# lightest/cellularautomatons3d

Measured on AMD Instinct MI355X. Metric: Gcells/s CA step at 512^3, higher is better.
Workload: dtype u32

## Files before the change

cellularautomatons3d_amd/_capi.py:

```python
from __future__ import annotations

import ctypes as C
import os

_HERE = os.path.dirname(os.path.abspath(__file__))
LIB_PATH = os.path.join(_HERE, "libca3d.so")

CA3D_OK = 0
LAYOUT_PACKED32 = 0
LAYOUT_UNPACKED = 1
LUT_LEN = 81
COMM_ID_BYTES = 128

SLAB_SEND_LOW, SLAB_SEND_HIGH, SLAB_RECV_LOW, SLAB_RECV_HIGH, SLAB_OWNED = range(5)
SLAB_PHASE_ALL, SLAB_PHASE_EDGES, SLAB_PHASE_INTERIOR = range(3)


class Ca3dError(RuntimeError):
    def __init__(self, code: int, message: str):
        super().__init__(f"ca3d error {code}: {message}")
        self.code = code
        self.message = message


class Info(C.Structure):
    _fields_ = [
        ("grid_size", C.c_uint32), ("layout", C.c_int32), ("z0", C.c_uint32), ("nz", C.c_uint32),
        ("ghost", C.c_uint32), ("step", C.c_uint64), ("state_words", C.c_uint64),
        ("current_buffer", C.c_int32), ("device", C.c_int32), ("kernel_name", C.c_char * 64),
        ("launches_total", C.c_uint64),
    ]


class Stats(C.Structure):
    _fields_ = [
        ("steps", C.c_uint64), ("kernel_launches", C.c_uint64), ("gpu_ms", C.c_double),
        ("cell_steps", C.c_double), ("algorithmic_bytes", C.c_double),
    ]


class RenderStats(C.Structure):
    _fields_ = [
        ("gpu_ms", C.c_double), ("primary_rays", C.c_uint64), ("shadow_rays", C.c_uint64),
        ("primary_cell_visits", C.c_uint64), ("shadow_cell_visits", C.c_uint64),
    ]


class SummaryStruct(C.Structure):
    _fields_ = [
        ("step", C.c_uint64), ("population", C.c_uint64), ("births", C.c_uint64), ("deaths", C.c_uint64), ("digest", C.c_uint64),
        ("has_previous", C.c_uint32), ("box_min", C.c_uint32 * 3), ("box_max", C.c_uint32 * 3),
    ]


class ComponentStruct(C.Structure):
    _fields_ = [
        ("population", C.c_uint32), ("first_cell", C.c_uint32), ("box_min", C.c_uint32), ("box_max", C.c_uint32), ("digest", C.c_uint64),
        ("reserved", C.c_uint32 * 2),
    ]


class IsolateJobStruct(C.Structure):
    _fields_ = [("universe", C.c_uint32), ("cell", C.c_uint32)]


class IsolatedStruct(C.Structure):
    _fields_ = [("population", C.c_uint32), ("shift", C.c_int32 * 3)]


ISOLATE_PLACEMENTS = {"keep": 0, "centre": 1, "origin": 2}
ISOLATE_COPY_RULES = 0x100
CONNECTIVITIES = {"closed": 0, "torus": 1}


class ComposePartStruct(C.Structure):
    _fields_ = [("universe", C.c_uint32), ("orientation", C.c_uint32), ("at", C.c_int32 * 3), ("reserved", C.c_uint32)]


class ComposedStruct(C.Structure):
    _fields_ = [("population", C.c_uint32), ("placed", C.c_uint32), ("overlap", C.c_uint32), ("clipped", C.c_uint32)]


class CanonStruct(C.Structure):
    _fields_ = [("key", C.c_uint64), ("symmetry", C.c_uint64), ("orientation", C.c_uint32), ("population", C.c_uint32),
                ("box_min", C.c_uint32), ("box_max", C.c_uint32)]


class CanonPeriodStruct(C.Structure):
    _fields_ = [("key", C.c_uint64), ("symmetry", C.c_uint64), ("orientation", C.c_uint32), ("phase", C.c_uint32),
                ("population", C.c_uint32), ("flags_shift", C.c_uint32)]


class EnvelopeStruct(C.Structure):
    _fields_ = [("period", C.c_uint32), ("flags", C.c_uint32), ("heat", C.c_uint32), ("population_sum", C.c_uint32),
                ("envelope_population", C.c_uint32), ("stator_population", C.c_uint32), ("envelope_min", C.c_uint8 * 4),
                ("envelope_max", C.c_uint8 * 4), ("rotor_min", C.c_uint8 * 4), ("rotor_max", C.c_uint8 * 4), ("reserved", C.c_uint32 * 2)]


ENVELOPE_COPY_RULES = 0x100
COMPOSE_OVER = 0x1
COMPOSE_COPY_RULES = 0x100
COMPOSE_MAX_PARTS = 1 << 20


class SeedStruct(C.Structure):
    _fields_ = [("seed", C.c_uint32), ("and_rounds", C.c_uint32), ("box_min", C.c_uint32 * 3), ("box_max", C.c_uint32 * 3)]


STOP_EXTINCT, STOP_STILL = 1, 2
STOP_PERIODIC = 4
STOP_MOVING = 8
ENSEMBLE_ALL = 0xFFFFFFFF
ENSEMBLE_WORDS = 8192


class CommInfo(C.Structure):
    _fields_ = [("device", C.c_int32), ("comm_ranks", C.c_int32), ("comm_rank", C.c_int32), ("comm_device", C.c_int32),
                ("pci_bus_id", C.c_char * 32)]


class JitStats(C.Structure):
    _fields_ = [
        ("programs_compiled", C.c_uint64), ("programs_from_disk", C.c_uint64), ("programs_from_memory", C.c_uint64),
        ("compile_ms", C.c_double), ("disk_read_ms", C.c_double), ("load_ms", C.c_double), ("cache_dir", C.c_char * 256),
    ]


def jit_stats() -> dict:
    st = JitStats()
    check(load().ca3d_get_jit_stats(C.byref(st)))
    return {"programs_compiled": int(st.programs_compiled), "programs_from_disk": int(st.programs_from_disk),
            "programs_from_memory": int(st.programs_from_memory), "compile_ms": round(st.compile_ms, 2),
            "disk_read_ms": round(st.disk_read_ms, 2), "load_ms": round(st.load_ms, 2), "cache_dir": st.cache_dir.decode()}


_u32p = C.POINTER(C.c_uint32)
_i32p = C.POINTER(C.c_int32)
_H = C.c_void_p
SYMBOLS = [
    ("ca3d_abi_version", C.c_int, []),
    ("ca3d_last_error", C.c_char_p, []),
    ("ca3d_selftest_exception", C.c_int, [C.c_int]),
    ("ca3d_get_jit_stats", C.c_int, [C.c_void_p]),
    ("ca3d_device_count", C.c_int, [C.POINTER(C.c_int)]),
    ("ca3d_create", C.c_int, [C.c_int, C.POINTER(_H)]),
    ("ca3d_destroy", C.c_int, [_H]),
    ("ca3d_configure", C.c_int, [_H, C.c_uint32, C.c_uint32, C.c_uint32, C.c_int]),
    ("ca3d_configure_slab", C.c_int, [_H, C.c_uint32, C.c_int, C.c_uint32, C.c_uint32, C.c_uint32]),
    ("ca3d_set_rules", C.c_int, [_H, _i32p, C.c_uint32, _i32p, C.c_uint32, _i32p, C.c_uint32, _u32p, _u32p]),
    ("ca3d_upload_state", C.c_int, [_H, _u32p, C.c_size_t]),
    ("ca3d_read_state", C.c_int, [_H, _u32p, C.c_size_t]),
    ("ca3d_step", C.c_int, [_H, C.c_uint32]),
    ("ca3d_flush", C.c_int, [_H]),
    ("ca3d_slab_step", C.c_int, [_H, C.c_uint32]),
    ("ca3d_slab_step_phase", C.c_int, [_H, C.c_uint32, C.c_int]),
    ("ca3d_slab_region", C.c_int, [_H, C.c_int, C.POINTER(C.c_void_p), C.POINTER(C.c_size_t)]),
    ("ca3d_comm_unique_id", C.c_int, [C.c_void_p]),
    ("ca3d_slab_comm_init", C.c_int, [_H, C.c_void_p, C.c_int, C.c_int]),
    ("ca3d_slab_run", C.c_int, [_H, C.c_uint32, C.c_int]),
    ("ca3d_slab_exchange", C.c_int, [_H]),
    ("ca3d_slab_comm_info", C.c_int, [_H, C.c_void_p]),
    ("ca3d_slab_gather", C.c_int, [_H, _H]),
    ("ca3d_group_create", C.c_int, [C.POINTER(C.c_int), C.c_int, C.POINTER(_H)]),
    ("ca3d_group_destroy", C.c_int, [_H]),
    ("ca3d_group_size", C.c_int, [_H, C.POINTER(C.c_int)]),
    ("ca3d_group_engine", C.c_int, [_H, C.c_int, C.POINTER(_H)]),
    ("ca3d_group_configure", C.c_int, [_H, C.c_uint32, C.c_int, C.c_uint32]),
    ("ca3d_group_set_rules", C.c_int, [_H, _i32p, C.c_uint32, _i32p, C.c_uint32, _i32p, C.c_uint32, _u32p, _u32p]),
    ("ca3d_group_upload_state", C.c_int, [_H, _u32p, C.c_size_t]),
    ("ca3d_group_read_state", C.c_int, [_H, _u32p, C.c_size_t]),
    ("ca3d_group_step", C.c_int, [_H, C.c_uint32]),
    ("ca3d_group_synchronize", C.c_int, [_H]),
    ("ca3d_group_set_option", C.c_int, [_H, C.c_char_p, C.c_int64]),
    ("ca3d_group_render", C.c_int, [_H, C.POINTER(C.c_float), C.c_uint32, C.c_uint32, C.c_uint32, C.c_void_p, C.c_void_p, C.c_void_p]),
    ("ca3d_group_summarize", C.c_int, [_H, C.POINTER(SummaryStruct), _u32p]),
    ("ca3d_summarize", C.c_int, [_H, C.POINTER(SummaryStruct), _u32p]),
    ("ca3d_get_summary_time", C.c_int, [_H, C.POINTER(C.c_double)]),
    ("ca3d_step_until", C.c_int, [_H, C.c_uint32, C.c_uint32, C.c_uint32, C.POINTER(SummaryStruct), _u32p, _u32p]),
    ("ca3d_step_until_cycle", C.c_int, [_H, C.c_uint32, C.c_uint32, C.c_uint32, C.POINTER(SummaryStruct), _u32p, _u32p, _u32p]),
    ("ca3d_ensemble_create", C.c_int, [C.c_int, C.POINTER(_H)]),
    ("ca3d_ensemble_destroy", C.c_int, [_H]),
    ("ca3d_ensemble_configure", C.c_int, [_H, C.c_uint32, C.c_uint32]),
    ("ca3d_ensemble_configure_neighbourhood", C.c_int, [_H, C.c_uint32, C.c_uint32, C.c_int]),
    ("ca3d_ensemble_get_neighbourhood", C.c_int, [_H, C.POINTER(C.c_int)]),
    ("ca3d_ensemble_configure_clustered", C.c_int, [_H, C.c_uint32, C.c_uint32]),
    ("ca3d_ensemble_get_clustered", C.c_int, [_H, C.POINTER(C.c_int)]),
    ("ca3d_ensemble_set_boundary", C.c_int, [_H, C.c_int]),
    ("ca3d_ensemble_get_boundary", C.c_int, [_H, C.POINTER(C.c_int)]),
    ("ca3d_ensemble_set_rule_tables_clustered", C.c_int, [_H, C.c_uint32, C.c_uint32, _u32p, _u32p, C.c_uint32]),
    ("ca3d_ensemble_set_rules", C.c_int, [_H, C.c_uint32, _i32p, C.c_uint32, _i32p, C.c_uint32, _i32p, C.c_uint32, _u32p, _u32p]),
    ("ca3d_ensemble_upload_state", C.c_int, [_H, C.c_uint32, C.c_uint32, _u32p, C.c_size_t]),
    ("ca3d_ensemble_read_state", C.c_int, [_H, C.c_uint32, C.c_uint32, _u32p, C.c_size_t]),
    ("ca3d_seed_state", C.c_int, [_H, C.POINTER(SeedStruct)]),
    ("ca3d_group_seed_state", C.c_int, [_H, C.POINTER(SeedStruct)]),
    ("ca3d_ensemble_seed_state", C.c_int, [_H, C.c_uint32, C.c_uint32, C.POINTER(SeedStruct), C.c_uint32]),
    ("ca3d_ensemble_set_rule_tables", C.c_int, [_H, C.c_uint32, C.c_uint32, _u32p, _u32p, C.c_uint32]),
    ("ca3d_ensemble_step", C.c_int, [_H, C.c_uint32]),
    ("ca3d_ensemble_step_until", C.c_int, [_H, C.c_uint32, C.c_uint32, C.c_uint32, _u32p, _u32p]),
    ("ca3d_ensemble_step_until_cycle", C.c_int, [_H, C.c_uint32, C.c_uint32, C.c_uint32, _u32p, _u32p, _u32p]),
    ("ca3d_ensemble_step_until_moving", C.c_int, [_H, C.c_uint32, C.c_uint32, C.c_uint32, _u32p, _u32p, _u32p, _i32p]),
    ("ca3d_ensemble_step_until_trace", C.c_int, [_H, C.c_uint32, C.c_uint32, C.c_uint32, _u32p, _u32p, _u32p, C.c_uint32, _u32p]),
    ("ca3d_ensemble_summarize", C.c_int, [_H, C.c_uint32, C.c_uint32, C.POINTER(SummaryStruct)]),
    ("ca3d_ensemble_census", C.c_int, [_H, C.c_uint32, C.c_uint32, C.c_uint32, C.POINTER(ComponentStruct), _u32p, _u32p, C.POINTER(C.c_float)]),
    ("ca3d_ensemble_isolate", C.c_int, [_H, C.c_uint32, _H, C.c_uint32, C.POINTER(IsolateJobStruct), C.c_uint32, C.POINTER(IsolatedStruct),
                                        C.POINTER(C.c_float)]),
    ("ca3d_ensemble_census_connected", C.c_int, [_H, C.c_uint32, C.c_uint32, C.c_uint32, C.c_uint32, C.POINTER(ComponentStruct), _u32p, _u32p,
                                                 C.POINTER(C.c_float)]),
    ("ca3d_ensemble_isolate_connected", C.c_int, [_H, C.c_uint32, _H, C.c_uint32, C.POINTER(IsolateJobStruct), C.c_uint32, C.c_uint32,
                                                  C.POINTER(IsolatedStruct), C.POINTER(C.c_float)]),
    ("ca3d_ensemble_compose", C.c_int, [_H, C.c_uint32, C.c_uint32, _H, C.POINTER(ComposePartStruct), _u32p, C.c_uint32,
                                        C.POINTER(ComposedStruct), C.POINTER(C.c_float)]),
    ("ca3d_ensemble_canon", C.c_int, [_H, C.c_uint32, C.c_uint32, C.POINTER(CanonStruct), C.POINTER(C.c_uint64), C.POINTER(C.c_float)]),
    ("ca3d_ensemble_canon_period", C.c_int, [_H, C.c_uint32, C.c_uint32, _u32p, C.POINTER(CanonPeriodStruct), C.POINTER(C.c_uint64), C.c_uint32,
                                             C.POINTER(C.c_float)]),
    ("ca3d_ensemble_envelope", C.c_int, [_H, C.c_uint32, C.c_uint32, _u32p, _H, C.c_uint32, C.c_uint32, C.POINTER(EnvelopeStruct),
                                         C.POINTER(C.c_float)]),
    ("ca3d_ensemble_synchronize", C.c_int, [_H]),
    ("ca3d_ensemble_get_stats", C.c_int, [_H, C.POINTER(Stats)]),
    ("ca3d_ensemble_render_sheet", C.c_int, [_H, C.c_uint32, C.c_uint32, C.POINTER(C.c_float), C.c_uint32, C.c_uint32, C.c_uint32, C.c_uint32,
                                             C.c_void_p, C.c_void_p, C.c_void_p]),
    ("ca3d_ensemble_get_sheet_stats", C.c_int, [_H, C.POINTER(RenderStats)]),
    ("ca3d_render_target", C.c_int, [_H, C.c_int, C.POINTER(C.c_void_p), C.POINTER(C.c_size_t)]),
    ("ca3d_synchronize", C.c_int, [_H]),
    ("ca3d_recovered_launches", C.c_int, [_H, C.POINTER(C.c_uint32)]),
    ("ca3d_measure_copy", C.c_int, [_H, C.c_size_t, C.c_uint32, C.POINTER(C.c_double)]),
    ("ca3d_set_stream", C.c_int, [_H, C.c_void_p]),
    ("ca3d_use_own_stream", C.c_int, [_H]),
    ("ca3d_device_buffer", C.c_int, [_H, C.c_int, C.POINTER(C.c_void_p), C.POINTER(C.c_size_t)]),
    ("ca3d_get_info", C.c_int, [_H, C.POINTER(Info)]),
    ("ca3d_get_jit_log", C.c_int, [_H, C.c_char_p, C.c_size_t, C.POINTER(C.c_size_t)]),
    ("ca3d_get_kernel_variant", C.c_int, [_H, C.c_char_p, C.c_size_t, C.POINTER(C.c_size_t)]),
    ("ca3d_get_stats", C.c_int, [_H, C.POINTER(Stats)]),
    ("ca3d_set_option", C.c_int, [_H, C.c_char_p, C.c_int64]),
    ("ca3d_render", C.c_int, [_H, C.POINTER(C.c_float), C.c_uint32, C.c_uint32, C.c_uint32, C.c_void_p, C.c_void_p, C.c_void_p]),
    ("ca3d_get_render_pipeline", C.c_int, [_H, C.POINTER(C.c_int32)]),
    ("ca3d_get_render_stats", C.c_int, [_H, C.POINTER(RenderStats)]),
]

_lib = None


def _pin_hip_runtime() -> None:
    if os.environ.get("CA3D_NO_TORCH_PRELOAD"):
        return
    try:
        import torch
    except ImportError:
        pass


def load() -> C.CDLL:
    global _lib
    if _lib is None:
        if not os.path.exists(LIB_PATH):
            raise ImportError(
                f"{LIB_PATH} is missing: build the HIP library first (python -c 'import __graft_entry__ as g; g.build()'). "
                "cellularautomatons3d_amd has no CPU fallback.")
        _pin_hip_runtime()
        lib = C.CDLL(LIB_PATH)
        for name, restype, argtypes in SYMBOLS:
            fn = getattr(lib, name)
            fn.restype = restype
            fn.argtypes = argtypes
        _lib = lib
    return _lib


def check(rc: int) -> None:
    if rc != CA3D_OK:
        raise Ca3dError(rc, load().ca3d_last_error().decode("utf-8", "replace"))
```

cellularautomatons3d_amd/csrc/ca3d_api.cpp:

```cpp
#include <cstdarg>
#include <cstdio>
#include <cstring>
#include <cstdlib>
#include <new>
#include <stdexcept>

#include "ca3d_engine.h"

namespace
{
thread_local char g_last_error[1024] = "";
}

namespace ca3d
{
void set_last_error(const char *msg) noexcept
{
	if (!msg) msg = "";
	size_t n = strlen(msg);
	if (n >= sizeof g_last_error) n = sizeof g_last_error - 1;
	memmove(g_last_error, msg, n);
	g_last_error[n] = 0;
}

// ... 118 lines not shown
	if (!h->has_state) return fail(CA3D_ERR_NOT_CONFIGURED, "ca3d_upload_state has not been called");
	return CA3D_OK;
}

static int state_replaced(ca3d_engine *h)
{
	h->step = 0;
	h->cur = 0;
	h->prev_ok = false;
	h->state_serial++;
	h->buffers_exposed = false;
	h->pending_edges = 0;
	h->ghosts_valid = false;
	h->res_pending.clear();
	if (h->res_status_host && *h->res_status_host)
	{
		HIP_TRY(hipMemsetAsync(h->res_mail, 0, h->res_mail_bytes, h->stream));
		HIP_TRY(hipMemsetAsync(h->res_status, 0, kResStatusBytes, h->stream));
		h->res_status_host[0] = h->res_status_host[1] = 0;
		h->res_epoch = 0;
		h->res_check = false;
		h->res_failed = true;
	}
	h->has_state = true;
	return CA3D_OK;
}

const char *seed_spec_error(const ca3d_seed &s, uint32_t G)
{
	if (s.and_rounds > 31u) return "and_rounds must be in [0, 31]";
	for (int i = 0; i < 3; i++)
	{
		if (s.box_min[i] > s.box_max[i]) return "box_min exceeds box_max";
		if (s.box_max[i] >= G) return "box_max lies outside the grid";
	}
	return nullptr;
}

static int switch_stream(ca3d_engine *h, hipStream_t s)
{
	if (!h) return fail(CA3D_ERR_INVALID_ARGUMENT, "NULL engine handle");
	FLUSH_QUEUED(h);
	int rc = bind_device(h);
	if (rc) return rc;
	HIP_TRY(hipStreamSynchronize(h->stream));
	rc = check_resident(h);
	if (rc) return rc;
	resident_stream_retired(h->stream);
	drop_graph(h);
	h->stream = s;
	h->ev_valid = false;
	refresh_kernels(h);
	return CA3D_OK;
}
}

using namespace ca3d;

extern "C"
{

int ca3d_abi_version(void) { return CA3D_ABI_VERSION; }

const char *ca3d_last_error(void) { return g_last_error; }

int ca3d_selftest_exception(int kind) CA3D_API_TRY
{
	if (kind == 0) throw std::bad_alloc();
	if (kind == 1) throw std::runtime_error("selftest");
	if (kind == 2) throw 42;
	if (kind == 3)
	{
		std::vector<char> v;
		v.resize(v.max_size() / 2u);
		return fail(CA3D_ERR_DEVICE, "selftest: the allocation of %zu bytes succeeded", v.size());
	}
	return CA3D_OK;
}
CA3D_API_CATCH

int ca3d_device_count(int *out_count) CA3D_API_TRY
{
	if (!out_count) return fail(CA3D_ERR_INVALID_ARGUMENT, "out_count is NULL");
	int n = 0;
	hipError_t e = hipGetDeviceCount(&n);
	if (e != hipSuccess) { *out_count = 0; return fail(CA3D_ERR_DEVICE, "hipGetDeviceCount: %s", hipGetErrorString(e)); }
	*out_count = n;
	return CA3D_OK;
}
CA3D_API_CATCH

int ca3d_create(int device, ca3d_t **out) CA3D_API_TRY
{
	if (!out) return fail(CA3D_ERR_INVALID_ARGUMENT, "out is NULL");
	*out = nullptr;
	int n = 0;
	hipError_t e = hipGetDeviceCount(&n);
	if (e != hipSuccess || n <= 0)
		return fail(CA3D_ERR_DEVICE, "no HIP device available (%s); this engine has no CPU fallback",
		            e != hipSuccess ? hipGetErrorString(e) : "device count is 0");
	if (device < 0 || device >= n) return fail(CA3D_ERR_INVALID_ARGUMENT, "device %d out of range [0,%d)", device, n);
	HIP_TRY(hipSetDevice(device));
	hipDeviceProp_t prop;
	HIP_TRY(hipGetDeviceProperties(&prop, device));
	if (strncmp(prop.gcnArchName, "gfx950", 6) != 0)
		return fail(CA3D_ERR_UNSUPPORTED, "device %d is %s; this library carries gfx950 (MI355X) code objects only", device, prop.gcnArchName);
	ca3d_engine *h = new (std::nothrow) ca3d_engine();
	if (!h) return fail(CA3D_ERR_OUT_OF_MEMORY, "out of host memory");
	h->device = device;
	hipError_t err = hipStreamCreateWithFlags(&h->own_stream, hipStreamNonBlocking);
	if (err == hipSuccess) err = hipEventCreate(&h->ev_start);
	if (err == hipSuccess) err = hipEventCreate(&h->ev_stop);
	if (err == hipSuccess) err = hipEventCreate(&h->rev_start);
	if (err == hipSuccess) err = hipEventCreate(&h->rev_stop);
	if (err != hipSuccess)
	{
		ca3d_destroy(h);
		return fail(CA3D_ERR_DEVICE, "engine set-up failed: %s", hipGetErrorString(err));
	}
	h->stream = h->own_stream;
	*out = h;
	return CA3D_OK;
}
CA3D_API_CATCH

int ca3d_destroy(ca3d_t *h) CA3D_API_TRY
{
	if (!h) return CA3D_OK;
	hipSetDevice(h->device);
	h->queued = 0;
	if (h->stream || h->own_stream) hipStreamSynchronize(h->stream);
	for (auto &L : h->lanes)
		if (L.s) hipStreamSynchronize(L.s);
	resident_stream_retired(h->stream);
	free_buffers(h);
	free_render_targets(h);
	free_slab_comm(h);
	if (h->r_counters) hipFree(h->r_counters);
	if (h->r_occ) hipFree(h->r_occ);
	if (h->r_stream) hipFree(h->r_stream);
	if (h->r_bricks) hipFree(h->r_bricks);
	for (auto &L : h->lanes)
	{
		if (L.s) { hipStreamSynchronize(L.s); hipStreamDestroy(L.s); }
		for (hipEvent_t e : {L.start, L.stop, L.done})
			if (e) hipEventDestroy(e);
		if (L.scratch) hipFree(L.scratch);
		if (L.counters) hipFree(L.counters);
	}
	for (hipStream_t sp : h->lane_spares) hipStreamDestroy(sp);
	if (h->ev_state) hipEventDestroy(h->ev_state);
	if (h->r_aux) hipStreamDestroy(h->r_aux);
	if (h->r_fork) hipEventDestroy(h->r_fork);
	if (h->r_join) hipEventDestroy(h->r_join);
	if (h->rev_start) hipEventDestroy(h->rev_start);
	if (h->rev_stop) hipEventDestroy(h->rev_stop);
	if (h->ev_start) hipEventDestroy(h->ev_start);
	if (h->ev_stop) hipEventDestroy(h->ev_stop);
	if (h->sum_ev0) hipEventDestroy(h->sum_ev0);
	if (h->sum_ev1) hipEventDestroy(h->sum_ev1);
	if (h->own_stream) hipStreamDestroy(h->own_stream);
	delete h;
	return CA3D_OK;
}
CA3D_API_CATCH

static int configure_common(ca3d_t *h, uint32_t g, int layout)
{
	if (!h) return fail(CA3D_ERR_INVALID_ARGUMENT, "NULL engine handle");
	if (layout != CA3D_LAYOUT_PACKED32 && layout != CA3D_LAYOUT_UNPACKED) return fail(CA3D_ERR_INVALID_ARGUMENT, "unknown layout %d", layout);
	if (g == 0) return fail(CA3D_ERR_INVALID_ARGUMENT, "grid size must be positive");
	if (layout == CA3D_LAYOUT_PACKED32 && (g % 32u)) return fail(CA3D_ERR_INVALID_ARGUMENT, "packed layout needs a grid size that is a multiple of 32 (got %u)", g);
	if (layout == CA3D_LAYOUT_UNPACKED && (g % 4u)) return fail(CA3D_ERR_INVALID_ARGUMENT, "unpacked layout needs a grid size that is a multiple of 4 (got %u)", g);
	if (g > 8192u) return fail(CA3D_ERR_UNSUPPORTED, "grid size %u exceeds the supported maximum 8192", g);
	int rc = bind_device(h);
	if (rc) return rc;
	HIP_TRY(hipStreamSynchronize(h->stream));
	free_buffers(h);
	h->buffers_exposed = false;
	h->G = g;
	h->layout = layout;
	h->plane_words = layout == CA3D_LAYOUT_PACKED32 ? (size_t)(g / 32u) * g : (size_t)g * g;
	return CA3D_OK;
}

int ca3d_configure(ca3d_t *h, uint32_t gx, uint32_t gy, uint32_t gz, int layout) CA3D_API_TRY
{
	if (gx != gy || gy != gz) return fail(CA3D_ERR_UNSUPPORTED, "only cubic grids exist in the reference (got %ux%ux%u)", gx, gy, gz);
	if (h) h->queued = 0;
	int rc = configure_common(h, gx, layout);
	if (rc) return rc;
	h->slab = false;
	h->z0 = 0;
	h->nz = gx;
	h->ghost = 0;
	h->nplanes = gx;
	rc = allocate(h);
	if (rc == CA3D_OK) refresh_kernels(h);
	return rc;
}
CA3D_API_CATCH

int ca3d_configure_slab(ca3d_t *h, uint32_t g, int layout, uint32_t z0, uint32_t nz, uint32_t ghost) CA3D_API_TRY
{
	if (h) h->queued = 0;
	int rc = configure_common(h, g, layout);
	if (rc) return rc;
	if (nz == 0 || z0 + nz > g) return fail(CA3D_ERR_INVALID_ARGUMENT, "slab [%u, %u) is outside the grid of %u planes", z0, z0 + nz, g);
	if (ghost == 0 || ghost > nz) return fail(CA3D_ERR_INVALID_ARGUMENT, "ghost depth must be in [1, nz] (got %u, nz %u)", ghost, nz);
	if (layout == CA3D_LAYOUT_UNPACKED && (g & (g - 1u))) return fail(CA3D_ERR_UNSUPPORTED, "unpacked slabs need a power-of-two grid size: the legacy kernel's -1 wrap is a torus only then");
	h->slab = true;
	h->z0 = z0;
	h->nz = nz;
	h->ghost = ghost;
	h->nplanes = nz + 2u * ghost;
	rc = allocate(h);
	if (rc == CA3D_OK) refresh_kernels(h);
	return rc;
}
CA3D_API_CATCH

int ca3d_set_rules(ca3d_t *h, const int32_t *main_offsets, uint32_t n_main, const int32_t *edges_offsets, uint32_t n_edges,
                   const int32_t *corners_offsets, uint32_t n_corners, const uint32_t survive[CA3D_LUT_LEN],
                   const uint32_t born[CA3D_LUT_LEN]) CA3D_API_TRY
{
	if (!h) return fail(CA3D_ERR_INVALID_ARGUMENT, "NULL engine handle");
	FLUSH_QUEUED(h);
	if (int rcs = settle_resident(h)) return rcs;
	CanonRules r;
	std::string err;
	int rc = canonicalize_rules(main_offsets, n_main, edges_offsets, n_edges, corners_offsets, n_corners, survive, born, &r, &err);
	if (rc) return fail(rc, "%s", err.c_str());
	rc = bind_device(h);
	if (rc) return rc;
	drop_graph(h);
	h->rules = r;
	refresh_kernels(h);
	return CA3D_OK;
}
CA3D_API_CATCH

int ca3d_upload_state(ca3d_t *h, const uint32_t *words, size_t n_words) CA3D_API_TRY
{
	if (!h) return fail(CA3D_ERR_INVALID_ARGUMENT, "NULL engine handle");
	if (!h->configured) return fail(CA3D_ERR_NOT_CONFIGURED, "ca3d_configure has not been called");
	if (!words) return fail(CA3D_ERR_INVALID_ARGUMENT, "words is NULL");
	h->queued = 0;
	if (n_words != h->state_words()) return fail(CA3D_ERR_INVALID_ARGUMENT, "state has %zu words, expected %zu", n_words, h->state_words());
	int rc = bind_device(h);
	if (rc) return rc;
	const size_t off = h->slab ? (size_t)h->ghost * h->plane_words : 0;
	const size_t bytes = n_words * sizeof(uint32_t);
	if (h->slab)
	{
		HIP_TRY(hipMemsetAsync(h->buf[0], 0, h->buffer_words() * sizeof(uint32_t), h->stream));
		HIP_TRY(hipMemsetAsync(h->buf[1], 0, h->buffer_words() * sizeof(uint32_t), h->stream));
	}
	HIP_TRY(hipMemcpyAsync(h->buf[0] + off, words, bytes, hipMemcpyHostToDevice, h->stream));
	HIP_TRY(hipMemcpyAsync(h->buf[1] + off, h->buf[0] + off, bytes, hipMemcpyDeviceToDevice, h->stream));
	HIP_TRY(hipStreamSynchronize(h->stream));
	rc = state_replaced(h);
	if (rc) return rc;
	h->binary_state = false;
	if (h->layout == CA3D_LAYOUT_UNPACKED)
	{
		bool bin = true;
		for (size_t i = 0; i < n_words && bin; i++) bin = words[i] <= 1u;
		h->binary_state = bin;
	}
	return CA3D_OK;
}
CA3D_API_CATCH

int ca3d_seed_state(ca3d_t *h, const ca3d_seed *spec) CA3D_API_TRY
{
	if (!h) return fail(CA3D_ERR_INVALID_ARGUMENT, "NULL engine handle");
	if (!spec) return fail(CA3D_ERR_INVALID_ARGUMENT, "spec is NULL");
	if (!h->configured) return fail(CA3D_ERR_NOT_CONFIGURED, "ca3d_configure has not been called");
	if (const char *why = seed_spec_error(*spec, h->G))
		return fail(CA3D_ERR_INVALID_ARGUMENT, "seed spec for a grid of %u: %s (box (%u, %u, %u) .. (%u, %u, %u), and_rounds %u)", h->G, why, spec->box_min[0],
		            spec->box_min[1], spec->box_min[2], spec->box_max[0], spec->box_max[1], spec->box_max[2], spec->and_rounds);
	h->queued = 0;
	int rc = bind_device(h);
	if (rc) return rc;
	if (!h->res_pending.empty() || h->res_check) HIP_TRY(hipStreamSynchronize(h->stream));
	SeedLaunch l;
	l.buf0 = h->buf[0]; l.buf1 = h->buf[1];
	l.G = h->G;
	l.layout = h->layout;
	l.z0 = h->z0; l.nz = h->nz; l.ghost = h->slab ? h->ghost : 0u;
	l.spec = *spec;
	hipError_t e = launch_seed(l, h->stream);
	if (e != hipSuccess) return fail(CA3D_ERR_DEVICE, "seed kernel launch failed: %s", hipGetErrorString(e));
	rc = state_replaced(h);
	if (rc) return rc;
	h->binary_state = true;
	return CA3D_OK;
}
CA3D_API_CATCH

int ca3d_read_state(ca3d_t *h, uint32_t *words, size_t n_words) CA3D_API_TRY
{
	if (!h) return fail(CA3D_ERR_INVALID_ARGUMENT, "NULL engine handle");
	if (!h->configured || !h->has_state) return fail(CA3D_ERR_NOT_CONFIGURED, "no state to read: configure and upload first");
	if (!words) return fail(CA3D_ERR_INVALID_ARGUMENT, "words is NULL");
	FLUSH_QUEUED(h);
// ... 299 lines not shown
	out->current_buffer = (int32_t)h->cur;
	out->device = h->device;
	out->launches_total = h->launches_total;
	reported_kernel_name(h, out->kernel_name, sizeof out->kernel_name);
	return CA3D_OK;
}
CA3D_API_CATCH

int ca3d_get_jit_log(ca3d_t *h, char *buf, size_t n_bytes, size_t *needed) CA3D_API_TRY
{
	if (!h) return fail(CA3D_ERR_INVALID_ARGUMENT, "NULL engine handle");
	if (needed) *needed = h->jit_log.size() + 1;
	if (buf && n_bytes)
	{
		const size_t n = h->jit_log.size() < n_bytes - 1 ? h->jit_log.size() : n_bytes - 1;
		memcpy(buf, h->jit_log.data(), n);
		buf[n] = '\0';
	}
	return CA3D_OK;
}
CA3D_API_CATCH

int ca3d_get_jit_stats(ca3d_jit_stats *out) CA3D_API_TRY
{
	if (!out) return fail(CA3D_ERR_INVALID_ARGUMENT, "NULL argument");
	jit_stats(out);
	return CA3D_OK;
}
CA3D_API_CATCH

int ca3d_get_kernel_variant(ca3d_t *h, char *buf, size_t n_bytes, size_t *needed) CA3D_API_TRY
{
	if (!h) return fail(CA3D_ERR_INVALID_ARGUMENT, "NULL engine handle");
	ca3d_info info;
	int rc = ca3d_get_info(h, &info);
	if (rc) return rc;
	uint64_t rh = 1469598103934665603ull;
	auto mix = [&](const void *p, size_t n) { for (size_t i = 0; i < n; i++) { rh ^= static_cast<const unsigned char *>(p)[i]; rh *= 1099511628211ull; } };
	if (h->rules.valid)
	{
		mix(&h->rules.lists, sizeof h->rules.lists);
		mix(h->rules.survive_raw, sizeof h->rules.survive_raw);
		mix(h->rules.born_raw, sizeof h->rules.born_raw);
	}
	const char *zs = getenv("CA3D_RC256_ZS");
	char text[320];
	const bool res = !strncmp(info.kernel_name, "ca_resident", 11);
	const ResidentShape shape = resident_shape(h);
	if (res)
		snprintf(text, sizeof text, "%s;G=%u;rule=%016llx;rows=%u;zsplit=%u;pair=%d;rc256zs=%s;src=%016llx", info.kernel_name, h->G, (unsigned long long)rh,
		         shape.rows, shape.zsplit, shape.pair, zs ? zs : "-", (unsigned long long)jit_sources_hash());
	else
		snprintf(text, sizeof text, "%s;G=%u;rule=%016llx;variant=%d;src=%016llx", info.kernel_name, h->G, (unsigned long long)rh, h->variant, (unsigned long long)jit_sources_hash());
	const size_t len = strlen(text);
	if (needed) *needed = len + 1;
	if (buf && n_bytes)
	{
		const size_t n = len < n_bytes - 1 ? len : n_bytes - 1;
		memcpy(buf, text, n);
		buf[n] = '\0';
	}
	return CA3D_OK;
}
CA3D_API_CATCH

int ca3d_get_stats(ca3d_t *h, ca3d_stats *out) CA3D_API_TRY
{
	if (!h || !out) return fail(CA3D_ERR_INVALID_ARGUMENT, "NULL argument");
	FLUSH_QUEUED(h);
	if (!h->ev_valid) return fail(CA3D_ERR_NOT_CONFIGURED, "no step batch has been timed yet (or option \"stats\" is 0)");
	int rc = bind_device(h);
	if (rc) return rc;
	HIP_TRY(hipEventSynchronize(h->ev_stop));
	float ms = 0.f;
	HIP_TRY(hipEventElapsedTime(&ms, h->ev_start, h->ev_stop));
	h->stats.gpu_ms = ms;
	*out = h->stats;
	HIP_TRY(hipStreamSynchronize(h->stream));
	return check_resident(h);
}
CA3D_API_CATCH

int ca3d_set_option(ca3d_t *h, const char *name, int64_t value) CA3D_API_TRY
{
	if (!h || !name) return fail(CA3D_ERR_INVALID_ARGUMENT, "NULL argument");
	FLUSH_QUEUED(h);
	if (strcmp(name, "queue") && strcmp(name, "stats"))
		if (int rcs = settle_resident(h)) return rcs;
	if (!strcmp(name, "resident_fault_tile"))
	{
		if (value < 0 || value > 1024) return fail(CA3D_ERR_INVALID_ARGUMENT, "resident_fault_tile must be in [0, 1024]");
		h->res_fault_tile = (uint32_t)value;
		return CA3D_OK;
	}
	if (!strcmp(name, "queue"))
	{
		if (value < 0 || value > 1000000) return fail(CA3D_ERR_INVALID_ARGUMENT, "queue must be in [0, 1000000] steps");
		h->queue_max = (uint32_t)value;
		return CA3D_OK;
	}
	if (!strcmp(name, "graph")) { h->use_graph = value ? 1 : 0; return CA3D_OK; }
	if (!strcmp(name, "graph_prepare"))
	{
		int rc = check_ready(h);
		if (rc) return rc;
		rc = bind_device(h);
		if (rc) return rc;
		if (!graphs_allowed(h) || h->slab || value <= 0) return CA3D_OK;
		uint64_t left = (uint64_t)value;
		uint32_t cur = h->cur;
		for (int pass = 0; pass < 2; pass++)
		{
			for (uint64_t l = left; l;)
			{
				const uint32_t n = l > kMaxGraphSteps ? kMaxGraphSteps : (uint32_t)l;
				if (n >= h->graph_min)
				{
					ca3d_engine::StepGraph *g = nullptr;
					rc = step_graph(h, n, cur, &g);
					if (rc) return rc;
				}
				cur = (cur + n) & 1u;
				l -= n;
			}
			if (cur == h->cur) break;
		}
		return CA3D_OK;
	}
	if (!strcmp(name, "stats")) { h->want_stats = value ? 1 : 0; if (!value) h->ev_valid = false; return CA3D_OK; }
	if (!strcmp(name, "graph_min"))
	{
		if (value < 1 || value > kMaxGraphSteps) return fail(CA3D_ERR_INVALID_ARGUMENT, "graph_min must be in [1, %u]", kMaxGraphSteps);
		h->graph_min = (uint32_t)value;
		return CA3D_OK;
	}
	if (!strcmp(name, "render_indirect")) { h->render_indirect = value ? 1 : 0; return CA3D_OK; }
	if (!strcmp(name, "render_sched")) { h->render_sched = value ? 1 : 0; return CA3D_OK; }
	if (!strcmp(name, "render_skip")) { h->render_skip = value ? 1 : 0; return CA3D_OK; }
	if (!strcmp(name, "rows"))
	{
		h->use_rows = value ? 1 : 0;
		refresh_kernels(h);
		return CA3D_OK;
	}
	if (!strcmp(name, "render_frame_bricks")) { h->render_frame_bricks = value ? 1 : 0; return CA3D_OK; }
	if (!strcmp(name, "render_stream")) { h->render_stream = value ? 1 : 0; return CA3D_OK; }
	if (!strcmp(name, "render_pipeline"))
	{
		if (value < 0 || value > ca3d_engine::kMaxLanes) return fail(CA3D_ERR_INVALID_ARGUMENT, "render_pipeline must be 0 (off), 1 (default depth) or 2 .. %d frames in flight", ca3d_engine::kMaxLanes);
		h->render_pipeline = (int)value;
		return CA3D_OK;
	}
	if (!strcmp(name, "render_stream_check")) { h->render_stream_check = value ? 1 : 0; return CA3D_OK; }
	if (!strcmp(name, "render_row_begin") || !strcmp(name, "render_row_end"))
	{
		if (value < 0 || value > 16384) return fail(CA3D_ERR_INVALID_ARGUMENT, "row %lld is outside any target", (long long)value);
		if (name[11] == 'b')
		{
			if (value % 16) return fail(CA3D_ERR_INVALID_ARGUMENT, "render_row_begin must be a multiple of 16 (the renderer's tile height)");
			h->render_row0 = (uint32_t)value;
		}
		else h->render_row1 = (uint32_t)value;
		return CA3D_OK;
	}
	if (!strcmp(name, "render_mode"))
	{
		if (value != 0 && value != 1) return fail(CA3D_ERR_INVALID_ARGUMENT, "render_mode must be 0 (converged frame) or 1 (one literal reference frame)");
		h->render_mode = (int)value;
		return CA3D_OK;
	}
	if (!strcmp(name, "render_reset_history"))
	{
		int rc2 = bind_device(h);
		if (rc2) return rc2;
		return clear_render_history(h);
	}
	if (!strcmp(name, "fused")) { drop_graph(h); h->use_fused = value ? 1 : 0; return CA3D_OK; }
	if (!strcmp(name, "variant"))
	{
		if (value != 0 && value != 1) return fail(CA3D_ERR_INVALID_ARGUMENT, "variant must be 0 (auto) or 1 (generic kernel)");
		drop_graph(h);
		h->variant = (int)value;
		refresh_kernels(h);
		return CA3D_OK;
	}
	if (!strcmp(name, "resident"))
	{
		h->use_resident = value ? 1 : 0;
		if (value) h->res_failed = false;
		refresh_kernels(h);
		return CA3D_OK;
	}
	if (!strcmp(name, "resident_rows"))
	{
		if (value != 16 && value != 32) return fail(CA3D_ERR_INVALID_ARGUMENT, "resident_rows must be 16 or 32");
		if ((uint32_t)value != h->res_rows)
		{
			int rc2 = bind_device(h);
			if (rc2) return rc2;
			HIP_TRY(hipStreamSynchronize(h->stream));
			free_resident(h);
			h->res_rows = (uint32_t)value;
			refresh_kernels(h);
		}
		return CA3D_OK;
	}
	if (!strcmp(name, "resident_pair"))
	{
		if (value != 0 && value != 1) return fail(CA3D_ERR_INVALID_ARGUMENT, "resident_pair must be 0 or 1");
		if ((value != 0) != h->res_pair)
		{
			int rc2 = bind_device(h);
			if (rc2) return rc2;
			HIP_TRY(hipStreamSynchronize(h->stream));
			free_resident(h);
			h->res_pair = value != 0;
			refresh_kernels(h);
		}
		return CA3D_OK;
	}
	if (!strcmp(name, "resident_zsplit"))
	{
		if (value != 1 && value != 2) return fail(CA3D_ERR_INVALID_ARGUMENT, "resident_zsplit must be 1 or 2");
		h->res_zsplit = (uint32_t)value;
		refresh_kernels(h);
		return CA3D_OK;
	}
	if (!strcmp(name, "resident_min"))
	{
		if (value < 1) return fail(CA3D_ERR_INVALID_ARGUMENT, "resident_min must be >= 1");
		h->res_min = (uint32_t)value;
		return CA3D_OK;
	}
	if (!strcmp(name, "resident_timeout_us"))
	{
		if (value < 1 || value > 40000000) return fail(CA3D_ERR_INVALID_ARGUMENT, "resident_timeout_us must be in [1, 40000000]");
		h->res_timeout_ticks = (uint32_t)(value * 100);
		return CA3D_OK;
	}
	if (!strcmp(name, "roll_z"))
	{
		if (value != 0 && value != 2 && value != 4 && value != 8 && value != 16 && value != 15 && value != 30) return fail(CA3D_ERR_INVALID_ARGUMENT, "roll_z must be 0 (automatic), 2, 4, 8, 16 (tile form only), or 15 / 30 (looped forms)");
		drop_graph(h);
		h->roll_z = (int)value;
		return CA3D_OK;
	}
	if (!strcmp(name, "roll_tile"))
	{
		drop_graph(h);
		if (value < 0 || value > 3) return fail(CA3D_ERR_INVALID_ARGUMENT, "roll_tile must be 0 (every thread shifts its rows), 1 (256-thread tiles), 2 (wave tiles) or 3 (two words per thread)");
		h->roll_tile = (int)value;
		return CA3D_OK;
	}
	if (!strcmp(name, "roll"))
	{
		drop_graph(h);
		h->use_roll = value ? 1 : 0;
		refresh_kernels(h);
		return CA3D_OK;
	}
	if (!strcmp(name, "jit"))
	{
		drop_graph(h);
		h->use_jit = value ? 1 : 0;
		refresh_kernels(h);
		return CA3D_OK;
	}
	return fail(CA3D_ERR_INVALID_ARGUMENT, "unknown option '%s'", name);
}
CA3D_API_CATCH

}

namespace ca3d
{
int engine_mark_state(ca3d_engine *h)
{
	if (!h || !h->configured || h->slab) return fail(CA3D_ERR_NOT_CONFIGURED, "engine_mark_state: a configured full-grid engine is needed");
	int rc = bind_device(h);
	if (rc) return rc;
	HIP_TRY(hipMemsetAsync(h->buf[0], 0, h->buffer_words() * sizeof(uint32_t), h->stream));
	HIP_TRY(hipMemsetAsync(h->buf[1], 0, h->buffer_words() * sizeof(uint32_t), h->stream));
	h->step = 0;
	h->cur = 0;
	h->prev_ok = false;
	h->has_state = true;
	h->binary_state = true;
	h->state_serial++;
	h->buffers_exposed = false;
	return CA3D_OK;
}
int engine_state_buffer(ca3d_engine *h, int which, void **device_ptr, size_t *n_bytes)
{
	const bool was = h ? h->buffers_exposed : false;
	const int rc = ca3d_device_buffer(h, which, device_ptr, n_bytes);
	if (h) h->buffers_exposed = was;
	return rc;
}
}
```

cellularautomatons3d_amd/csrc/ca3d_engine.h:

```cpp
#pragma once

#include <map>
#include <string>
#include <vector>

#include "ca3d_internal.h"

struct ca3d_engine
{
	int device = 0;
	hipStream_t own_stream = nullptr;
	hipStream_t stream = nullptr;
	hipEvent_t ev_start = nullptr, ev_stop = nullptr;
	bool ev_valid = false;

	bool configured = false;
	uint32_t G = 0;
	int layout = CA3D_LAYOUT_PACKED32;
	bool slab = false;
	uint32_t z0 = 0, nz = 0, ghost = 0;
	uint32_t nplanes = 0;
	size_t plane_words = 0;
	uint32_t *buf[2] = {nullptr, nullptr};
	bool has_state = false;
	bool binary_state = false;
	uint64_t step = 0;
	uint32_t cur = 0;

	ca3d::CanonRules rules;
	int variant = 0;
	int use_graph = 1;
	int render_mode = 0;
	int render_indirect = 0;
	int render_sched = 1;
	uint32_t render_row0 = 0, render_row1 = 0;
	int use_fused = 0;

	struct StepGraph { hipGraphExec_t exec = nullptr; uint32_t launches = 0; };
	std::map<uint64_t, StepGraph> step_graphs;
	uint32_t graph_min = 128;
	int want_stats = 1;
	std::map<uint64_t, hipGraphExec_t> slab_graphs;
	uint32_t pending_edges = 0;
	bool pending_binary = true;
	bool pending_resident = false;
	int roll_z = 0;
	int roll_tile = 1;
	int use_roll = 1;
	int use_jit = 1;
	ca3d::VnJit vn_jit;
	ca3d::ClassJit class_jit;
	ca3d::RowsJit rows_jit;
	int use_rows = 1;
	ca3d::RollJit roll_jit;
	std::string jit_log;

	int use_resident = 1;
	bool res_ready = false;
	bool res_class = false;
	bool res_failed = false;
	bool res_check = false;
	void *res_jit_fn = nullptr;
	void *res_slab_fn = nullptr;
	size_t res_mail_bytes = 0;
	unsigned long long *res_mail = nullptr;
	uint32_t *res_status = nullptr, *res_status_host = nullptr;
	uint32_t res_epoch = 0;
	uint32_t res_min = 8;
	uint32_t queue_max = 0;
	uint32_t queued = 0;
	uint64_t launches_total = 0;
	bool res_pair = true;
	uint32_t res_rows = 32;
	uint32_t res_zsplit = 1;
	uint32_t res_timeout_ticks = 20000000;
	uint32_t *spare = nullptr;
	struct ResPending { uint32_t epoch0, n, cur_before; uint64_t step_before; uint32_t *in, *other, *spare; };
	std::vector<ResPending> res_pending;
	uint32_t res_fault_tile = 0;
	uint32_t res_recovered = 0;
	std::string res_note;

	void *comm = nullptr;
	int comm_rank = 0, comm_world = 0;
	hipStream_t comm_stream = nullptr;
	hipEvent_t ev_edges = nullptr, ev_comm = nullptr, ev_gather = nullptr;
	bool ghosts_valid = false;

	ca3d_stats stats{};
	const char *unpacked_kernel = "";

	uint32_t *sum_dev = nullptr, *sum_host = nullptr;
	size_t sum_words = 0;
	hipEvent_t sum_ev0 = nullptr, sum_ev1 = nullptr;
	bool sum_ev_valid = false;
	uint32_t *cycle_anchor = nullptr;
	bool prev_ok = false;

	uint32_t rw = 0, rh = 0;
	uint32_t *r_present = nullptr;
	void *r_light[2] = {nullptr, nullptr};
	uint32_t *r_depth[2] = {nullptr, nullptr};
	unsigned long long *r_counters = nullptr;
	size_t r_counter_words = 0;
	unsigned long long *r_occ = nullptr;
	size_t r_occ_words = 0;
	int render_skip = 1;
	int render_stream = 1;
	int render_stream_check = 0;
	int render_frame_bricks = 1;
	uint32_t *r_bricks = nullptr;
	size_t r_bricks_bytes = 0;
	uint64_t state_serial = 1, r_occ_key[3] = {0, 0, 0}, r_bricks_key[3] = {0, 0, 0};
	bool buffers_exposed = false;
	void *r_stream = nullptr;
	size_t r_stream_bytes = 0;
	int r_swap = 0;
	hipEvent_t rev_start = nullptr, rev_stop = nullptr;
	hipStream_t r_aux = nullptr;
	hipEvent_t r_fork = nullptr, r_join = nullptr;
	bool rev_valid = false;
	ca3d_render_stats rstats{};
	static constexpr int kMaxLanes = 4;
	struct FrameLane
	{
		hipStream_t s = nullptr;
		hipEvent_t start = nullptr, stop = nullptr, done = nullptr;
		bool need_state = true;
		void *scratch = nullptr;
		size_t scratch_bytes = 0;
		unsigned long long *counters = nullptr;
		bool pending = false;
		bool used = false;
	} lanes[kMaxLanes];
	int n_lanes = 0;
	hipEvent_t ev_state = nullptr;
	bool main_touched = true;
	bool state_touched = true;
	std::vector<hipStream_t> lane_spares;
	int render_pipeline = 1;
	int lane_next = 0;
	int lanes_in_use = 0;
	bool lanes_exhausted = false;
	int last_lane = -1;

	size_t buffer_words() const { return plane_words * nplanes; }
	size_t state_words() const { return plane_words * (slab ? nz : G); }
	double cells_per_plane() const { return (double)G * G; }
	double bytes_per_cell_step() const { return layout == CA3D_LAYOUT_PACKED32 ? 0.25 : 8.0; }
};

namespace ca3d
{

void set_last_error(const char *msg) noexcept;
int fail(int code, const char *fmt, ...);

#define HIP_TRY(expr)                                                                                          \
	do                                                                                                         \
	{                                                                                                          \
		hipError_t e_ = (expr);                                                                                \
		if (e_ != hipSuccess)                                                                                  \
			return ca3d::fail(e_ == hipErrorOutOfMemory ? CA3D_ERR_OUT_OF_MEMORY : CA3D_ERR_DEVICE, "%s: %s", #expr, \
			                  hipGetErrorString(e_));                                                          \
	} while (0)

int bind_device(ca3d_engine *h, bool join = true);
int check_ready(ca3d_engine *h);
void drop_graph(ca3d_engine *h);
int engine_mark_state(ca3d_engine *h);
int engine_state_buffer(ca3d_engine *h, int which, void **device_ptr, size_t *n_bytes);

constexpr uint32_t kMaxGraphSteps = 1024;
constexpr size_t kResStatusBytes = (4 + 1024) * sizeof(uint32_t);
struct ResidentShape { uint32_t rows, zsplit; int pair; };
ResidentShape resident_shape(const ca3d_engine *h);
bool resident_wanted(const ca3d_engine *h, uint32_t n);
void reported_kernel_name(const ca3d_engine *h, char *out, size_t n_bytes);
void refresh_kernels(ca3d_engine *h);
int enqueue_step(ca3d_engine *h, int src, uint32_t lo, uint32_t hi, hipStream_t s, bool fused = false, uint32_t lo2 = 0, uint32_t hi2 = 0);
bool graphs_allowed(const ca3d_engine *h);
int step_graph(ca3d_engine *h, uint32_t n, uint32_t start, ca3d_engine::StepGraph **out);
int resident_slab_steps(ca3d_engine *h, uint32_t n);
int check_resident(ca3d_engine *h);
int settle_resident(ca3d_engine *h);
int record_batch_stats(ca3d_engine *h, uint32_t steps, uint64_t launches, uint32_t planes);
int flush_queued(ca3d_engine *h);

#define FLUSH_QUEUED(h)                   \
	do                                    \
	{                                     \
		int rcq_ = ca3d::flush_queued(h); \
		if (rcq_) return rcq_;            \
	} while (0)

template <class Enqueue> int capture_graph(ca3d_engine *h, Enqueue &&enqueue, hipGraphExec_t *exec)
{
	hipGraph_t graph = nullptr;
	HIP_TRY(hipStreamBeginCapture(h->stream, hipStreamCaptureModeThreadLocal));
	int rc = enqueue();
	hipError_t e = hipStreamEndCapture(h->stream, &graph);
	if (rc != CA3D_OK) { if (graph) hipGraphDestroy(graph); return rc; }
	if (e != hipSuccess) return fail(CA3D_ERR_DEVICE, "hipStreamEndCapture: %s", hipGetErrorString(e));
	e = hipGraphInstantiate(exec, graph, nullptr, nullptr, 0);
	hipGraphDestroy(graph);
	if (e != hipSuccess) return fail(CA3D_ERR_DEVICE, "hipGraphInstantiate: %s", hipGetErrorString(e));
	return CA3D_OK;
}

void free_slab_comm(ca3d_engine *h);
int engines_rccl_init_all(ca3d_engine **engines, int n);
int engines_rccl_exchange_all(ca3d_engine **engines, int n);

void free_render_targets(ca3d_engine *h);
int join_frames(ca3d_engine *h);
int clear_render_history(ca3d_engine *h);

}
```

cellularautomatons3d_amd/csrc/ca3d_internal.h:

```cpp
#pragma once

#include <hip/hip_runtime.h>
#include <stdint.h>
#include <string>

#include "ca3d.h"
#include "ca_device_types.h"

namespace ca3d
{

constexpr int kMaxOffsets = 26;

struct OffsetLists
{
	uint32_t n[3];
	uint8_t code[3][32];
};

struct CanonRules
{
	bool valid = false;
	MainKind main = MAIN_GENERIC;
	bool need[3] = {false, false, false};
	bool fast = false;
	OffsetLists lists{};
	PackedRuleArgs prog{};
	uint32_t onset_survive[3]{}, onset_born[3]{};
	uint32_t unpacked_survive = 0, unpacked_born = 0;
	RuleSetProg unpacked_prog{};
	bool unpacked_fast = false;
	uint32_t survive_raw[CA3D_LUT_LEN]{}, born_raw[CA3D_LUT_LEN]{};
};

int canonicalize_rules(const int32_t *main_offs, uint32_t n_main, const int32_t *edge_offs, uint32_t n_edge,
                       const int32_t *corner_offs, uint32_t n_corner, const uint32_t *survive,
                       const uint32_t *born, CanonRules *out, std::string *err);
void compile_rule_prog(uint32_t onset_mask, uint32_t max_count, RuleProg *out);


struct VnJit
{
	void *zr1 = nullptr, *zr2 = nullptr, *zr4 = nullptr, *zr8 = nullptr;
	int cvl = -1;
	uint32_t lut_s = 0, lut_b = 0;
};

struct RowsJit
{
	void *deep = nullptr, *flat = nullptr;
	uint32_t G = 0;
	int zrun = 0, main = -1;
	bool e = false, c = false;
};

struct ClassJit
{
	void *deep = nullptr, *deep_za = nullptr, *flat = nullptr;
	void *deep_np2 = nullptr, *flat_np2 = nullptr;
	int main = -1;
	bool e = false, c = false;
};

struct RollJit
{
	void *z[3] = {nullptr, nullptr, nullptr};
	void *tile[4] = {nullptr, nullptr, nullptr, nullptr};
	void *tile_x = nullptr; int zx = 0;
	void *loop[2][2] = {{nullptr, nullptr}, {nullptr, nullptr}};
	void *w2[2] = {nullptr, nullptr};
	void *wtile[2] = {nullptr, nullptr};
	void *np2[3] = {nullptr, nullptr, nullptr};
	int cv_np2 = 0;
	int cvl = -1;
	int main = -1;
	bool e = false, c = false;
};

struct PackedLaunch
{
	const uint32_t *in;
	uint32_t *out;
	PlaneRange pr;
	const CanonRules *rules;
	int variant;
	const VnJit *vn_jit = nullptr;
	const ClassJit *class_jit = nullptr;
	const RollJit *roll_jit = nullptr;
	int roll_z = 0;
	int roll_tile = 1;
	const RowsJit *rows_jit = nullptr;
};

struct ResidentLaunch
{
	const uint32_t *in;
	uint32_t *out_last, *out_prev;
	uint32_t G;
	unsigned long long *mail;
	uint32_t *status;
	uint32_t *host_flag;
	uint32_t steps, epoch0, timeout_ticks;
	uint32_t lut_s, lut_b;
	void *jit_fn = nullptr;
	uint32_t rows = 32;
	uint32_t fault_tile = 0;
	uint32_t zsplit = 1;
	int pair = 0;
};

struct UnpackedLaunch
{
	const uint32_t *in;
	uint32_t *out;
	PlaneRange pr;
	const CanonRules *rules;
	bool binary_state;
};

struct RenderLaunch
{
	const uint32_t *cells;
	uint32_t G, W, H, spp;
	const float *uniforms;
	uint32_t *presentation;
	void *light;
	uint32_t *depth;
	unsigned long long *counters;
	bool legacy;
	int mode;
	const void *prev_light;
	const uint32_t *prev_depth;
	int sched = 1;
	unsigned long long *occ = nullptr;
	uint32_t row0 = 0, row1 = 0;
	bool indirect = false;
	bool trace = false;
	hipStream_t aux = nullptr;
	hipEvent_t ev_fork = nullptr, ev_join = nullptr;
	uint32_t *bricks = nullptr;
	bool occ_valid = false, bricks_valid = false;
	bool *occ_built = nullptr, *bricks_built = nullptr;
	void *stream_scratch = nullptr;
	hipEvent_t after = nullptr;
	int walk_share_pct = 100;
	bool stream_check = false;
};

constexpr uint32_t kSummaryHeaderWords = 16;
struct SummaryLaunch
{
	const uint32_t *cur, *prev;
	uint32_t *result;
	uint32_t G;
	int layout;
	uint32_t z0, nz;
};
hipError_t launch_summary(const SummaryLaunch &l, hipStream_t stream);
hipError_t launch_state_equal(const uint32_t *a, const uint32_t *b, size_t n_words, uint32_t *flag, hipStream_t stream);
constexpr uint32_t kEnsembleWords = 8192;
constexpr uint32_t kEnsembleMaxSteps = 65536;
struct EnsembleLaunch
{
	uint32_t *state, *prev;
	const uint32_t *rules;
	int neighbourhood;
	bool clustered;
	int boundary;
	ca3d_summary *records;
	uint32_t *steps_done;
	uint32_t *reason;
	uint32_t *anchor;
	uint32_t *cycle;
	uint32_t *samples;
	uint32_t sample_stride;
	uint32_t first, count;
	uint32_t steps;
	uint32_t base;
	uint32_t check_every, stop_mask;
	bool final;
	bool reset;
};
hipError_t launch_ensemble(const EnsembleLaunch &l, hipStream_t stream);
const void *ensemble_boundary_kernel(int boundary, int kind, int form);
int ensemble_workgroups_per_cu(int neighbourhood, bool clustered = false);
constexpr uint32_t ensemble_rule_words(int neighbourhood, bool clustered = false)
{
	return clustered ? 6u : neighbourhood == CA3D_ENSEMBLE_MOORE ? 2u : 1u;
}
constexpr uint32_t kCensusMaxComponents = 1024;
struct CensusLaunch
{
	const uint32_t *state;
	uint32_t first, count;
	uint32_t max_components;
	ca3d_component *out;
	uint32_t *n_components, *remaining;
	uint32_t connectivity;
};
hipError_t launch_census(const CensusLaunch &l, hipStream_t stream);
hipError_t launch_census_torus(const CensusLaunch &l, hipStream_t stream);
struct IsolateLaunch
{
	const uint32_t *src_state;
	uint32_t *dst_state, *dst_prev;
	const uint32_t *src_rules;
	uint32_t *dst_rules;
	const ca3d_isolate_job *jobs;
	ca3d_isolated *out;
	uint32_t dst_first, n_jobs;
	uint32_t placement;
	uint32_t rule_words;
	uint32_t connectivity;
};
hipError_t launch_isolate(const IsolateLaunch &l, hipStream_t stream);
hipError_t launch_isolate_torus(const IsolateLaunch &l, hipStream_t stream);
struct ComposeLaunch
{
	const uint32_t *src_state;
	uint32_t *dst_state, *dst_prev;
	const uint32_t *src_rules;
	uint32_t *dst_rules;
	const ca3d_compose_part *parts;
	const uint32_t *part_begin;
	ca3d_composed *out;
	uint32_t dst_first, n_dst;
	bool over;
	uint32_t rule_words;
};
hipError_t launch_compose(const ComposeLaunch &l, hipStream_t stream);
struct CanonLaunch
{
	const uint32_t *state;
	uint32_t first, count;
	ca3d_canon *out;
	uint64_t *digests;
};
hipError_t launch_canon(const CanonLaunch &l, hipStream_t stream);
struct CanonPeriodLaunch
{
	const uint32_t *state;
	const uint32_t *rules;
	int neighbourhood;
	bool clustered;
	uint32_t first, count;
	const uint32_t *periods;
	ca3d_canon_period *out;
	uint64_t *keys;
	uint32_t keys_stride;
};
hipError_t launch_canon_period(const CanonPeriodLaunch &l, hipStream_t stream);
struct EnvelopeLaunch
{
	const uint32_t *state;
	const uint32_t *rules;
	int neighbourhood;
	bool clustered;
	int boundary;
	uint32_t first, count;
	const uint32_t *periods;
	ca3d_envelope *out;
	uint32_t images;
	uint32_t *dst_state, *dst_prev;
	uint32_t *dst_rules;
	uint32_t dst_first;
	uint32_t rule_words;
};
hipError_t launch_envelope(const EnvelopeLaunch &l, hipStream_t stream);
struct SheetLaunch
{
	const uint32_t *state;
	uint32_t first, count;
	uint32_t tile_w, tile_h, columns, spp;
	const float *uniforms;
	uint32_t *presentation;
	void *light;
	uint32_t *depth;
	unsigned long long *counters;
};
hipError_t launch_render_sheet(const SheetLaunch &l, hipStream_t stream);
uint32_t sheet_shares(uint32_t count, uint32_t blocks, uint32_t slots);
struct SeedLaunch
{
	uint32_t *buf0, *buf1;
	uint32_t G;
	int layout;
	uint32_t z0, nz, ghost;
	ca3d_seed spec;
};
hipError_t launch_seed(const SeedLaunch &l, hipStream_t stream);
hipError_t launch_seed_ensemble(uint32_t *state, uint32_t *prev, uint32_t first, uint32_t count, const ca3d_seed *specs, const ca3d_seed &one, hipStream_t stream);
const char *seed_spec_error(const ca3d_seed &s, uint32_t G);
hipError_t launch_copy_f4(const void *in, void *out, size_t bytes, hipStream_t stream);
hipError_t streams_concurrent(hipStream_t a, hipStream_t b, bool *out);
hipError_t launch_render(const RenderLaunch &l, hipStream_t stream);
size_t stream_scratch_bytes(uint32_t W, uint32_t H, uint32_t spp, size_t *hit_off, size_t *occl_off, size_t *rays_off);
size_t frame_bricks_bytes(uint32_t G);
bool frame_bricks_applies(uint32_t G);
hipError_t launch_render_frame_bricks(const void *frame_params, uint32_t *bricks, bool bricks_valid, hipStream_t stream, bool *bricks_built = nullptr);
hipError_t launch_brick_volume(const uint32_t *cells, uint32_t *bricks, uint32_t G, hipStream_t stream);
hipError_t launch_render_stream(const void *params, void *scratch, uint32_t W, uint32_t H, bool check, uint32_t *bricks, bool bricks_valid, hipStream_t stream, bool *bricks_built = nullptr, hipEvent_t before_resolve = nullptr, int walk_share_pct = 100,
                                bool *sparse_too = nullptr);

hipError_t launch_packed_step(const PackedLaunch &l, hipStream_t stream);
const char *packed_kernel_name(const CanonRules &r, uint32_t G, int variant);
bool vn_rule_applies(const CanonRules &r, int variant);
bool side_tables_silent(const CanonRules &r);
bool vn_kernel_applies(const CanonRules &r, uint32_t G, int variant);
hipError_t launch_packed_vn(const PackedLaunch &l, hipStream_t stream);
void vn_tables(const CanonRules &r, uint32_t *lut_s, uint32_t *lut_b);
bool vn_tables_prebuilt(uint32_t lut_s, uint32_t lut_b);
int vn_grid_log2(uint32_t G);
uint64_t jit_sources_hash();
int jit_vn_kernels(int device, int cvl, uint32_t lut_s, uint32_t lut_b, VnJit *out, std::string *log);
void class_tables(const CanonRules &r, uint32_t tables[6]);
int class_zrun(const CanonRules &r);
bool use_class_kernel(const CanonRules &r, uint32_t G, int variant);
int jit_class_kernels(int device, const CanonRules &r, ClassJit *out, std::string *log);
int jit_rows_kernels(int device, const CanonRules &r, uint32_t G, RowsJit *out, std::string *log);
bool rows_kernel_applies(const CanonRules &r, uint32_t G, int variant);
int jit_roll_kernels(int device, const CanonRules &r, int cvl, RollJit *out, std::string *log);
int jit_roll_np2_kernels(int device, const CanonRules &r, int cv, RollJit *out, std::string *log);
bool roll_np2_applies(const CanonRules &r, uint32_t G, int variant);
bool roll_kernel_applies(const CanonRules &r, uint32_t G, int variant);
std::string synthesize_rule_source(const CanonRules &r, int *ops_out);
std::string rule_function_source(const CanonRules &r);
bool resident_kernel_applies(const CanonRules &r, uint32_t G, int variant);
size_t resident_mail_bytes(uint32_t G, uint32_t rows);
hipError_t launch_resident(const ResidentLaunch &l, hipStream_t stream);
bool resident_capacity(uint32_t G, uint32_t rows, uint32_t zsplit, int pair, void *jit_fn, hipStream_t stream, uint32_t *tiles, uint32_t *capacity);
bool resident_slab_capacity(void *fn, hipStream_t stream, uint32_t *tiles, uint32_t *capacity);
int jit_resident_kernel(int device, uint32_t lut_s, uint32_t lut_b, uint32_t rows, uint32_t zsplit, int pair, void **fn, std::string *log);
bool resident_class_applies(const CanonRules &r, uint32_t G, int variant);
int jit_resident_class_kernel(int device, const CanonRules &r, uint32_t G, uint32_t zsplit, void **fn, std::string *log);
uint32_t resident_class_zsplit(uint32_t G);
struct ResidentSlabLaunch
{
	const uint32_t *in;
	uint32_t *out;
	unsigned long long *mail;
	uint32_t *status, *host_flag;
	uint32_t steps, epoch0, timeout_ticks;
	int dead_plane;
	void *fn;
};
int resident_slab_planes(const CanonRules &r, uint32_t G, uint32_t nplanes, int variant);
size_t resident_slab_mail_bytes();
hipError_t launch_resident_slab(const ResidentSlabLaunch &l, hipStream_t stream);
void resident_stream_retired(hipStream_t stream);
int jit_resident_slab_kernel(int device, uint32_t lut_s, uint32_t lut_b, int pz, void **fn, std::string *log);
int packed_fused_steps(const CanonRules &r, uint32_t G, int variant);
hipError_t launch_packed_fused(const PackedLaunch &l, hipStream_t stream);
hipError_t launch_unpacked_step(const UnpackedLaunch &l, hipStream_t stream, const char **kernel_name);


int exception_to_status() noexcept;
void jit_stats(ca3d_jit_stats *out);
#define CA3D_API_TRY try
#define CA3D_API_CATCH                          \
	catch (...)                                 \
	{                                           \
		return ca3d::exception_to_status();     \
	}

}
```

cellularautomatons3d_amd/csrc/ca3d_render.cpp:

```cpp
#include <cstdio>
#include <cstdlib>
#include <cstring>
#include <vector>

#include "ca3d_engine.h"

namespace ca3d
{

void free_render_targets(ca3d_engine *h)
{
	if (h->r_present) hipFree(h->r_present);
	for (int i = 0; i < 2; i++)
	{
		if (h->r_light[i]) hipFree(h->r_light[i]);
		if (h->r_depth[i]) hipFree(h->r_depth[i]);
		h->r_light[i] = nullptr;
		h->r_depth[i] = nullptr;
	}
	h->r_present = nullptr;
	h->rw = h->rh = 0;
}

static int render_default_lanes(size_t samples)
{
	static const int env = getenv("CA3D_RENDER_LANES") ? atoi(getenv("CA3D_RENDER_LANES")) : 0;
	if (env >= 2 && env <= ca3d_engine::kMaxLanes) return env;
	return samples <= (24u << 20) ? 4 : 3;
}
static int render_walk_share(size_t samples, int lanes) { return lanes < 2 ? 100 : (samples <= (24u << 20) ? 100 / lanes : 67); }

int join_frames(ca3d_engine *h)
{
	for (auto &L : h->lanes)
		if (L.pending)
		{
			HIP_TRY(hipStreamWaitEvent(h->stream, L.done, 0));
			L.pending = false;
		}
	return CA3D_OK;
}

int clear_render_history(ca3d_engine *h)
{
	const size_t px = (size_t)h->rw * h->rh;
	for (int i = 0; i < 2 && px && h->r_light[i] && h->r_depth[i]; i++)
	{
		HIP_TRY(hipMemsetAsync(h->r_light[i], 0, px * 8, h->stream));
		HIP_TRY(hipMemsetAsync(h->r_depth[i], 0, px * 4, h->stream));
	}
	return CA3D_OK;
}

static const char *render_trace_path()
{
	static const char *path = getenv("CA3D_RENDER_TRACE");
	return path;
}
static bool render_aux_off()
{
	static const bool off = getenv("CA3D_RENDER_AUX") && atoi(getenv("CA3D_RENDER_AUX")) == 0;
	return off;
}

struct Frame
{
	uint32_t width, height, spp;
	bool to_host;
	const char *trace_path;
	size_t counter_words = 0;
	ca3d_engine::FrameLane *L = nullptr;
	int active_lanes = 0;
	hipStream_t rs = nullptr;
	unsigned long long *counters = nullptr;
	uint64_t state_key[3] = {0, 0, 0};
	bool occ_built = false, bricks_built = false;
	RenderLaunch l;
};

static bool frame_pipelined(const ca3d_engine *h, const Frame &f)
{
	const bool first_after_touch = h->state_touched;
	return !first_after_touch && h->render_pipeline && h->render_mode == 0 && !f.to_host && h->stream == h->own_stream &&
	       h->layout == CA3D_LAYOUT_PACKED32 && h->render_stream && h->render_sched && !h->render_indirect && !h->render_stream_check && !f.trace_path &&
	       !render_aux_off() && !h->render_row0 && !h->render_row1 && f.width == h->rw && f.height == h->rh;
}

static int size_render_targets(ca3d_engine *h, const Frame &f)
{
	if (f.width == h->rw && f.height == h->rh) return CA3D_OK;
	const size_t px = (size_t)f.width * f.height;
	HIP_TRY(hipStreamSynchronize(h->stream));
	free_render_targets(h);
	HIP_TRY(hipMalloc((void **)&h->r_present, px * 4));
	for (int i = 0; i < 2; i++)
	{
		HIP_TRY(hipMalloc(&h->r_light[i], px * 8));
		HIP_TRY(hipMalloc((void **)&h->r_depth[i], px * 4));
		HIP_TRY(hipMemsetAsync(h->r_light[i], 0, px * 8, h->stream));
		HIP_TRY(hipMemsetAsync(h->r_depth[i], 0, px * 4, h->stream));
	}
	h->rw = f.width;
	h->rh = f.height;
	h->r_swap = 0;
	return CA3D_OK;
}

static int size_render_counters(ca3d_engine *h, Frame &f)
{
	const size_t trace_waves = f.trace_path ? ((size_t)(f.width + 31u) / 32u * 2u) * ((f.height + 15u) / 16u * 4u) : 0u;
	f.counter_words = 8u + 4u * trace_waves;
	if (h->r_counters && h->r_counter_words < f.counter_words) { HIP_TRY(hipFree(h->r_counters)); h->r_counters = nullptr; }
	if (!h->r_counters)
	{
		HIP_TRY(hipMalloc((void **)&h->r_counters, f.counter_words * sizeof(unsigned long long)));
		h->r_counter_words = f.counter_words;
	}
	return CA3D_OK;
}

static int create_lanes(ca3d_engine *h, int want_lanes)
{
	for (auto &fl : h->lanes)
		if (fl.s && fl.pending) HIP_TRY(hipStreamSynchronize(fl.s));
	if (!h->lanes[0].s) { HIP_TRY(hipStreamCreateWithFlags(&h->lanes[0].s, hipStreamNonBlocking)); h->n_lanes = 1; }
	for (int tries = 0; tries < 10 && h->n_lanes < want_lanes; tries++)
	{
		hipStream_t cand = nullptr;
		HIP_TRY(hipStreamCreateWithFlags(&cand, hipStreamNonBlocking));
		bool side_by_side = true;
		for (int i = 0; i < h->n_lanes && side_by_side; i++) HIP_TRY(streams_concurrent(h->lanes[i].s, cand, &side_by_side));
		if (side_by_side) h->lanes[h->n_lanes++].s = cand;
		else h->lane_spares.push_back(cand);
	}
	if (h->n_lanes < want_lanes) h->lanes_exhausted = true;
	if (h->n_lanes < 2) h->render_pipeline = 0;
	else
		for (int i = 0; i < h->n_lanes; i++)
		{
			ca3d_engine::FrameLane &fl = h->lanes[i];
			if (fl.done) continue;
			HIP_TRY(hipEventCreateWithFlags(&fl.done, hipEventDisableTiming));
			HIP_TRY(hipEventCreate(&fl.start));
			HIP_TRY(hipEventCreate(&fl.stop));
			HIP_TRY(hipMalloc((void **)&fl.counters, 8u * sizeof(unsigned long long)));
		}
	if (!h->ev_state) HIP_TRY(hipEventCreateWithFlags(&h->ev_state, hipEventDisableTiming));
	return CA3D_OK;
}

static int pick_lane(ca3d_engine *h, Frame &f, bool pipelined)
{
	f.l.walk_share_pct = 100;
	f.rs = h->stream;
	f.counters = h->r_counters;
	const size_t frame_samples = (size_t)f.width * f.height * f.spp;
	const int want_lanes = h->render_pipeline >= 2 ? (h->render_pipeline < ca3d_engine::kMaxLanes ? h->render_pipeline : ca3d_engine::kMaxLanes) : render_default_lanes(frame_samples);
	if (pipelined && h->n_lanes < want_lanes && !h->lanes_exhausted)
		if (int rc = create_lanes(h, want_lanes)) return rc;
	f.active_lanes = h->n_lanes < want_lanes ? h->n_lanes : want_lanes;
	if (!(pipelined && h->render_pipeline && f.active_lanes >= 2)) return CA3D_OK;
	if (h->lane_next >= f.active_lanes) h->lane_next = 0;
	ca3d_engine::FrameLane *L = f.L = &h->lanes[h->lane_next];
	h->lanes_in_use = f.active_lanes;
	bool beside = false;
	for (int i = 0; i < f.active_lanes && !beside && !h->main_touched; i++)
		if (&h->lanes[i] != L && h->lanes[i].used)
		{
			const hipError_t q = hipEventQuery(h->lanes[i].done);
			if (q == hipErrorNotReady) { beside = true; (void)hipGetLastError(); }
			else if (q != hipSuccess) HIP_TRY(q);
		}
	f.l.walk_share_pct = beside ? render_walk_share(frame_samples, f.active_lanes) : 100;
	if (h->main_touched)
	{
		HIP_TRY(hipEventRecord(h->ev_state, h->stream));
		h->main_touched = false;
		for (auto &fl : h->lanes) fl.need_state = true;
	}
	if (L->need_state)
	{
		HIP_TRY(hipStreamWaitEvent(L->s, h->ev_state, 0));
		L->need_state = false;
	}
	f.rs = L->s;
	f.counters = L->counters;
	return CA3D_OK;
}

static int begin_launch(ca3d_engine *h, Frame &f, const float *uniforms)
{
	HIP_TRY(hipMemsetAsync(f.counters, 0, (f.trace_path ? f.counter_words : 8u) * sizeof(unsigned long long), f.rs));
	RenderLaunch &l = f.l;
	l.trace = f.trace_path != nullptr;
	l.cells = h->buf[h->cur];
	l.G = h->G;
	l.W = f.width;
	l.H = f.height;
	l.spp = f.spp;
	l.uniforms = uniforms;
	l.presentation = h->r_present;
	l.light = h->r_light[h->r_swap];
	l.depth = h->r_depth[h->r_swap];
	l.counters = f.counters;
	if (h->buffers_exposed) h->state_serial++;
	f.state_key[0] = h->state_serial;
	f.state_key[1] = h->step;
	f.state_key[2] = (uint64_t)(uintptr_t)l.cells;
	return CA3D_OK;
}

static int prepare_occupancy(ca3d_engine *h, Frame &f)
{
	if (!(h->render_skip && h->layout == CA3D_LAYOUT_PACKED32)) return CA3D_OK;
	const size_t fine = (size_t)(h->G / 32u) * (h->G / 8u) * (h->G / 8u);
	const size_t words = (fine + 63u) / 64u + 1u + (fine / 64u + 63u) / 64u + 3u;
	if (words != h->r_occ_words)
	{
		h->r_occ_key[0] = 0;
		for (auto &fl : h->lanes)
			if (fl.s) HIP_TRY(hipStreamSynchronize(fl.s));
		if (h->r_occ) HIP_TRY(hipFree(h->r_occ));
		h->r_occ = nullptr;
		h->r_occ_words = 0;
		HIP_TRY(hipMalloc((void **)&h->r_occ, words * sizeof(unsigned long long)));
		h->r_occ_words = words;
	}
	f.l.occ = h->r_occ;
	f.l.occ_valid = !memcmp(f.state_key, h->r_occ_key, sizeof f.state_key);
	f.l.occ_built = &f.occ_built;
	return CA3D_OK;
}

static int apply_render_options(const ca3d_engine *h, Frame &f)
{
	RenderLaunch &l = f.l;
	l.mode = h->render_mode;
	l.sched = h->render_sched;
	l.indirect = h->render_indirect != 0;
	if (l.indirect && (h->render_mode != 0 || h->layout != CA3D_LAYOUT_PACKED32)) return fail(CA3D_ERR_UNSUPPORTED, "render_indirect is implemented for the converged-frame mode over the packed layout");
	l.row0 = h->render_row0;
	l.row1 = h->render_row1 > f.height ? f.height : h->render_row1;
	if (l.row1 && l.row0 >= l.row1) return fail(CA3D_ERR_INVALID_ARGUMENT, "render rows [%u, %u) are empty for a target of %u rows", l.row0, h->render_row1, f.height);
	if ((l.row0 || l.row1) && h->render_mode != 0) return fail(CA3D_ERR_UNSUPPORTED, "row bands are implemented for the converged-frame mode only");
	l.legacy = h->layout == CA3D_LAYOUT_UNPACKED;
	l.prev_light = h->r_light[h->r_swap ^ 1];
	l.prev_depth = h->r_depth[h->r_swap ^ 1];
	return CA3D_OK;
}

static int prepare_aux_stream(ca3d_engine *h, Frame &f)
{
	if (f.L) return CA3D_OK;
	if (render_aux_off() || h->render_mode != 0 || !h->render_sched || f.trace_path) return CA3D_OK;
	if (!h->r_aux)
	{
		HIP_TRY(hipStreamCreateWithFlags(&h->r_aux, hipStreamNonBlocking));
		HIP_TRY(hipEventCreateWithFlags(&h->r_fork, hipEventDisableTiming));
		HIP_TRY(hipEventCreateWithFlags(&h->r_join, hipEventDisableTiming));
	}
	f.l.aux = h->r_aux;
	f.l.ev_fork = h->r_fork;
	f.l.ev_join = h->r_join;
	return CA3D_OK;
}

static int prepare_stream_scratch(ca3d_engine *h, Frame &f)
{
	RenderLaunch &l = f.l;
	if (!(h->render_stream && h->render_mode == 0 && h->render_sched && !l.legacy && !l.indirect && !f.trace_path)) return CA3D_OK;
	size_t o0, o1, o2;
	const size_t need = stream_scratch_bytes(f.width, f.height, f.spp, &o0, &o1, &o2);
	void *&scratch = f.L ? f.L->scratch : h->r_stream;
	size_t &scratch_bytes = f.L ? f.L->scratch_bytes : h->r_stream_bytes;
	if (scratch_bytes < need)
	{
		HIP_TRY(hipStreamSynchronize(f.rs));
		if (scratch) HIP_TRY(hipFree(scratch));
		scratch = nullptr;
		scratch_bytes = 0;
		HIP_TRY(hipMalloc(&scratch, need));
		scratch_bytes = need;
	}
	l.stream_scratch = scratch;
	l.stream_check = h->render_stream_check != 0;
	if (l.stream_check) HIP_TRY(hipMemsetAsync(scratch, 0, 4096, f.rs));
	return CA3D_OK;
}

static int prepare_bricks(ca3d_engine *h, Frame &f)
{
	if (!(h->render_frame_bricks && frame_bricks_applies(h->G) && (h->render_mode == 1 || f.l.stream_scratch))) return CA3D_OK;
	const size_t need = frame_bricks_bytes(h->G);
	if (h->r_bricks_bytes != need)
	{
		HIP_TRY(hipStreamSynchronize(h->stream));
		for (auto &fl : h->lanes)
			if (fl.s) HIP_TRY(hipStreamSynchronize(fl.s));
		if (h->r_bricks) HIP_TRY(hipFree(h->r_bricks));
		h->r_bricks = nullptr;
		h->r_bricks_bytes = 0;
		HIP_TRY(hipMalloc((void **)&h->r_bricks, need));
		h->r_bricks_bytes = need;
		h->r_bricks_key[0] = 0;
	}
	f.l.bricks = h->r_bricks;
	f.l.bricks_valid = !memcmp(f.state_key, h->r_bricks_key, sizeof f.state_key);
	f.l.bricks_built = &f.bricks_built;
	return CA3D_OK;
}

static int cross_lane_waits(ca3d_engine *h, Frame &f)
{
	if (!f.L) return CA3D_OK;
	RenderLaunch &l = f.l;
	if (h->last_lane >= 0 && h->last_lane != h->lane_next && h->lanes[h->last_lane].used) l.after = h->lanes[h->last_lane].done;
	const bool occ_rebuild = l.occ && !l.occ_valid, bricks_rebuild = l.bricks && !l.bricks_valid;
	if (occ_rebuild || bricks_rebuild)
		for (auto &fl : h->lanes)
			if (&fl != f.L && fl.used) HIP_TRY(hipStreamWaitEvent(f.rs, fl.done, 0));
	return CA3D_OK;
}

static int launch_frame(ca3d_engine *h, Frame &f)
{
	ca3d_engine::FrameLane *L = f.L;
	HIP_TRY(hipEventRecord(L ? L->start : h->rev_start, f.rs));
	hipError_t e = launch_render(f.l, f.rs);
	if (e != hipSuccess)
	{
		h->r_occ_key[0] = h->r_bricks_key[0] = 0;
		return fail(CA3D_ERR_DEVICE, "render launch failed: %s", hipGetErrorString(e));
	}
	if (f.occ_built) memcpy(h->r_occ_key, f.state_key, sizeof f.state_key);
	if (f.bricks_built) memcpy(h->r_bricks_key, f.state_key, sizeof f.state_key);
	HIP_TRY(hipEventRecord(L ? L->stop : h->rev_stop, f.rs));
	h->rev_valid = true;
	h->last_lane = L ? h->lane_next : -1;
	if (L)
	{
		HIP_TRY(hipEventRecord(L->done, f.rs));
		L->pending = L->used = true;
		h->lane_next = (h->lane_next + 1) % f.active_lanes;
	}
	return CA3D_OK;
}

static int read_back_diagnostics(ca3d_engine *h, const Frame &f)
{
	if (f.trace_path)
	{
		std::vector<unsigned long long> t(f.counter_words);
		HIP_TRY(hipStreamSynchronize(h->stream));
		HIP_TRY(hipMemcpy(t.data(), h->r_counters, f.counter_words * sizeof(unsigned long long), hipMemcpyDeviceToHost));
		if (FILE *file = fopen(f.trace_path, "wb"))
		{
			fwrite(t.data(), sizeof(unsigned long long), f.counter_words, file);
			fclose(file);
		}
	}
	if (f.l.stream_scratch && f.l.stream_check)
	{
		uint32_t bad[4] = {0, 0, 0, 0};
		HIP_TRY(hipStreamSynchronize(h->stream));
		HIP_TRY(hipMemcpy(bad, static_cast<const uint32_t *>(f.l.stream_scratch) + 2, sizeof bad, hipMemcpyDeviceToHost));
		if (bad[0]) return fail(CA3D_ERR_DEVICE, "render_stream_check: the interval filter contradicted the slab test at %u live cells", bad[0]);
		if (bad[1]) return fail(CA3D_ERR_DEVICE, "render_stream_check: %u looked-up answers had not been given in this frame (jobs lost by the queues; jobs %u .. %u)", bad[1], ~bad[2], bad[3]);
	}
	return CA3D_OK;
}
}

using namespace ca3d;

extern "C"
{

int ca3d_render_target(ca3d_t *h, int which, void **device_ptr, size_t *n_bytes) CA3D_API_TRY
{
	if (!h || !device_ptr || !n_bytes) return fail(CA3D_ERR_INVALID_ARGUMENT, "NULL argument");
	if (!h->r_present) return fail(CA3D_ERR_NOT_CONFIGURED, "ca3d_render has not been called yet");
	if (int rcb = bind_device(h)) return rcb;
	const size_t px = (size_t)h->rw * h->rh;
	switch (which)
	{
	case 0: *device_ptr = h->r_present; *n_bytes = px * 4; break;
	case 1: *device_ptr = h->r_light[h->r_swap ^ 1]; *n_bytes = px * 8; break;
	case 2: *device_ptr = h->r_depth[h->r_swap ^ 1]; *n_bytes = px * 4; break;
	default: return fail(CA3D_ERR_INVALID_ARGUMENT, "target must be 0 (presentation), 1 (light) or 2 (depth)");
	}
	return CA3D_OK;
}
CA3D_API_CATCH

int ca3d_render(ca3d_t *h, const float uniforms[128], uint32_t width, uint32_t height, uint32_t spp,
                uint8_t *presentation_rgba8, uint16_t *light_rgba16f, uint16_t *depth_rg16f) CA3D_API_TRY
{
	if (!h) return fail(CA3D_ERR_INVALID_ARGUMENT, "NULL engine handle");
	if (!h->configured || !h->has_state) return fail(CA3D_ERR_NOT_CONFIGURED, "no state to render: configure and upload first");
	FLUSH_QUEUED(h);
	if (h->slab) return fail(CA3D_ERR_UNSUPPORTED, "the renderer reads a full grid, not a slab");
	if (h->layout == CA3D_LAYOUT_UNPACKED && h->render_mode != 0) return fail(CA3D_ERR_UNSUPPORTED, "the literal frame mode is implemented for the packed layout only");
	if (!uniforms) return fail(CA3D_ERR_INVALID_ARGUMENT, "uniforms is NULL");
	if (width == 0 || height == 0 || width > 16384u || height > 16384u) return fail(CA3D_ERR_INVALID_ARGUMENT, "bad target size %ux%u", width, height);
	if (spp != 1 && spp != 4) return fail(CA3D_ERR_INVALID_ARGUMENT, "spp must be 1 or 4");
	if (h->render_mode == 1 && spp != 1) return fail(CA3D_ERR_INVALID_ARGUMENT, "the literal frame mode takes one jittered sample per pixel (spp = 1)");
	Frame f;
	f.width = width;
	f.height = height;
	f.spp = spp;
	f.to_host = presentation_rgba8 || light_rgba16f || depth_rg16f;
	f.trace_path = render_trace_path();
	const bool pipelined = frame_pipelined(h, f);
	int rc = bind_device(h, !pipelined);
	if (rc) return rc;
	if (f.to_host || (h->res_status_host && *h->res_status_host)) rc = settle_resident(h);
	if (rc) return rc;
	if ((rc = size_render_targets(h, f))) return rc;
	if ((rc = size_render_counters(h, f))) return rc;
	if ((rc = pick_lane(h, f, pipelined))) return rc;
	if ((rc = begin_launch(h, f, uniforms))) return rc;
	if ((rc = prepare_occupancy(h, f))) return rc;
	if ((rc = apply_render_options(h, f))) return rc;
	if ((rc = prepare_aux_stream(h, f))) return rc;
	if ((rc = prepare_stream_scratch(h, f))) return rc;
	if ((rc = prepare_bricks(h, f))) return rc;
	if ((rc = cross_lane_waits(h, f))) return rc;
	if ((rc = launch_frame(h, f))) return rc;
	if ((rc = read_back_diagnostics(h, f))) return rc;
	const size_t px = (size_t)width * height;
	h->rstats.primary_rays = (uint64_t)width * ((f.l.row1 ? f.l.row1 : height) - f.l.row0) * spp;
	if (presentation_rgba8) HIP_TRY(hipMemcpyAsync(presentation_rgba8, h->r_present, px * 4, hipMemcpyDeviceToHost, h->stream));
	if (light_rgba16f) HIP_TRY(hipMemcpyAsync(light_rgba16f, h->r_light[h->r_swap], px * 8, hipMemcpyDeviceToHost, h->stream));
	if (depth_rg16f) HIP_TRY(hipMemcpyAsync(depth_rg16f, h->r_depth[h->r_swap], px * 4, hipMemcpyDeviceToHost, h->stream));
	if (f.to_host) HIP_TRY(hipStreamSynchronize(h->stream));
	h->r_swap ^= 1;
	h->state_touched = false;
	return CA3D_OK;
}
CA3D_API_CATCH

int ca3d_get_render_stats(ca3d_t *h, ca3d_render_stats *out) CA3D_API_TRY
{
	if (!h || !out) return fail(CA3D_ERR_INVALID_ARGUMENT, "NULL argument");
	if (!h->rev_valid) return fail(CA3D_ERR_NOT_CONFIGURED, "ca3d_render has not been called yet");
	int rc = bind_device(h);
	if (rc) return rc;
	const ca3d_engine::FrameLane *L = h->last_lane >= 0 ? &h->lanes[h->last_lane] : nullptr;
	HIP_TRY(hipEventSynchronize(L ? L->stop : h->rev_stop));
	float ms = 0.f;
	HIP_TRY(hipEventElapsedTime(&ms, L ? L->start : h->rev_start, L ? L->stop : h->rev_stop));
	unsigned long long c[3] = {0, 0, 0};
	HIP_TRY(hipMemcpy(c, L ? L->counters : h->r_counters, sizeof c, hipMemcpyDeviceToHost));
	h->rstats.gpu_ms = ms;
	h->rstats.shadow_rays = c[0];
	h->rstats.primary_cell_visits = c[1];
	h->rstats.shadow_cell_visits = c[2];
	*out = h->rstats;
	return CA3D_OK;
}
CA3D_API_CATCH

int ca3d_get_render_pipeline(ca3d_t *h, int32_t *frames_in_flight) CA3D_API_TRY
{
	if (!h || !frames_in_flight) return fail(CA3D_ERR_INVALID_ARGUMENT, "ca3d_get_render_pipeline: NULL argument");
	*frames_in_flight = h->render_pipeline && h->n_lanes >= 2 ? h->lanes_in_use : 0;
	return CA3D_OK;
}
CA3D_API_CATCH

}
```

cellularautomatons3d_amd/csrc/render.hip:

```cpp
#include <hip/hip_fp16.h>

#include "ca3d_internal.h"

namespace ca3d
{
namespace
{

#include "render_device.inc"


template <bool SKIP>
__global__ __launch_bounds__(256, 4) void ca_render_packed(RenderParams P)
{
	if ((!P.legacy && occ_skip_enabled(P)) != SKIP) return;
	const bool whole_frame = SKIP && live_box_small(P);
	if (whole_frame && P.spread) return;
	if (P.outside_only && !whole_frame && blockIdx.x * 16u >= P.rx0 && blockIdx.x * 16u < P.rx1 && P.row0 + blockIdx.y * 16u >= P.ry0 && P.row0 + blockIdx.y * 16u < P.ry1) return;
	const u32 px = blockIdx.x * 16u + (threadIdx.x & 15u);
	const u32 py = P.row0 + blockIdx.y * 16u + (threadIdx.x >> 4);
	if (px >= P.W || py >= P.row1) return;
	float r = 0.0f, g = 0.0f, b = 0.0f, a = 0.0f, d0 = 0.0f;
	u32 shadow = 0, pvis = 0, svis = 0;
	for (u32 k = 0; k < P.spp; k++)
// ... 805 lines not shown
		const v3 p = cam + ray * mixed_depth;
		reprojected_uv(P, p, uvx, uvy);
		float col[3] = {0.0f, 0.0f, 0.0f};
		{
			const CellU cell = cell_u(P, p);
			const u32 st = cell_state(P, cell.x, cell.y, cell.z);
			const float dist = sd_box(p - cell.origin, vhalf);
			if (st == 1u && !(dist > 0.001f))
			{
				const v3 light_pos = V(u[U_LIGHT], u[U_LIGHT + 1], u[U_LIGHT + 2]);
				const v3 ldir = norm3(light_pos - p);
				const float rnd = n1rand(P, vu, vv);
				float vn, vf;
				ray_cube(p, ldir, V(0.0f, 0.0f, 0.0f), half, vn, vf);
				const v3 vexit = p + ldir * vf;
				float occ = 1.0f;
				{
					const v3 seg = vexit - p;
					const v3 dir = norm3(seg);
					const float march = len3(seg);
					const float step = fmaxf(cs * u[U_CELLSIZE], march / u[U_SHADOWSAMPLES]);
					float depth = step * rnd + 0.0025f;
					for (int guard = 0; depth < march && guard < 100000; guard++)
					{
						svis++;
						const v3 sp = p + dir * depth;
						const v3 cc = V(floorf(to_cells(P, sp.x)), floorf(to_cells(P, sp.y)), floorf(to_cells(P, sp.z)));
						const u32 ux = f2u(cc.x), uy = f2u(cc.y), uz = f2u(cc.z);
						const u32 st2 = cell_state(P, ux, uy, uz);
						const v3 origin = V(cc.x * cs + cs * 0.5f - kHalf, cc.y * cs + cs * 0.5f - kHalf, cc.z * cs + cs * 0.5f - kHalf);
						if ((ux != cell.x || uy != cell.y || uz != cell.z) && st2 == 1u)
						{
							float a, b;
							ray_cube(p, dir, origin, vhalf, a, b);
							if (a <= b && a >= 0.0f) { occ = kOcclusion; break; }
						}
						depth += step;
					}
				}
				shadow = 1u;
				const v3 N = face_normal(p, cell.origin);
				const float Gf = (float)P.G;
				const float cxn = (float)cell.x / Gf, cyn = (float)cell.y / Gf;
				v3 albedo = V(cxn, cyn, 1.0f - cxn);
				if (u[U_MATERIALCOLOR] != 0.0f || u[U_MATERIALCOLOR + 1] != 0.0f || u[U_MATERIALCOLOR + 2] != 0.0f)
					albedo = V(u[U_MATERIALCOLOR], u[U_MATERIALCOLOR + 1], u[U_MATERIALCOLOR + 2]);
				const v3 Vd = norm3(cam - p);
				const v3 L = norm3(light_pos - p);
				const v3 F0 = V(u[U_REFLECTIVITY], u[U_REFLECTIVITY + 1], u[U_REFLECTIVITY + 2]);
				const v3 brdf = surface_brdf(L, Vd, N, u[U_ROUGHNESS], albedo, F0);
				const float mag = u[U_LIGHT + 3];
				const float LoN = dot3(L, N);
				col[0] = occ * fmaxf(0.0f, brdf.x * mag * LoN);
				col[1] = occ * fmaxf(0.0f, brdf.y * mag * LoN);
				col[2] = occ * fmaxf(0.0f, brdf.z * mag * LoN);
			}
		}
		{
			float pc[4] = {0.0f, 0.0f, 0.0f, 0.0f};
			size_t ti;
			if (F.prev_light && texel_xy(P, uvx * u[U_WINDOW], uvy * u[U_WINDOW + 1], ti))
			{
				const uint2 raw = F.prev_light[ti];
				pc[0] = __half2float(__ushort_as_half((unsigned short)(raw.x & 0xFFFFu)));
				pc[1] = __half2float(__ushort_as_half((unsigned short)(raw.x >> 16)));
				pc[2] = __half2float(__ushort_as_half((unsigned short)(raw.y & 0xFFFFu)));
				pc[3] = __half2float(__ushort_as_half((unsigned short)(raw.y >> 16)));
			}
			const v3 rdir = norm3(p - pcam);
			const v3 rpoint = pcam + rdir * pdr;
			const CellU rcell = cell_u(P, rpoint), ccell = cell_u(P, p);
			const bool outside = uvx < 0.0f || uvx > 1.0f || uvy < 0.0f || uvy > 1.0f;
			if (outside || ccell.idx != rcell.idx) { out[0] = col[0]; out[1] = col[1]; out[2] = col[2]; out[3] = 1.0f; }
			else
			{
				const float a = u[U_TEMPORALALPHA];
				const float cur[4] = {col[0], col[1], col[2], 1.0f};
				for (int k = 0; k < 4; k++) out[k] = fminf(fmaxf(pc[k] * (1.0f - a) + cur[k] * a, 0.0f), 1.0f);
			}
		}
	}
	{
		const v3 light_pos = V(u[U_LIGHT], u[U_LIGHT + 1], u[U_LIGHT + 2]);
		float ln, lf;
		ray_cube(cam, ray, light_pos, V(0.005f, 0.005f, 0.005f), ln, lf);
		if (ln <= lf && lf >= 0.0f && out[0] == 0.0f && out[1] == 0.0f && out[2] == 0.0f) { out[0] = out[1] = out[2] = out[3] = 1.0f; }
	}
	if (u[U_SHOWDEPTH] == 1.0f && vu < 0.5f) { out[0] = mixed_depth; out[1] = 0.0f; out[2] = 0.0f; out[3] = 1.0f; }
	const size_t i = (size_t)py * P.W + px;
	if (P.light)
	{
		const __half2 rg = __floats2half2_rn(out[0], out[1]), ba = __floats2half2_rn(out[2], 1.0f);
		uint2 v;
		v.x = *reinterpret_cast<const u32 *>(&rg);
		v.y = *reinterpret_cast<const u32 *>(&ba);
		P.light[i] = v;
	}
	if (P.depth)
	{
		const __half2 d = __floats2half2_rn(mixed_depth, 1.0f);
		P.depth[i] = *reinterpret_cast<const u32 *>(&d);
	}
	if (P.presentation)
	{
		const float ig = 1.0f / u[U_GAMMA];
		P.presentation[i] = unorm8(powf(out[0], ig)) | (unorm8(powf(out[1], ig)) << 8) | (unorm8(powf(out[2], ig)) << 16) | (unorm8(out[3]) << 24);
	}
	if (P.counters)
	{
		atomicAdd(&P.counters[0], (unsigned long long)shadow);
		atomicAdd(&P.counters[1], (unsigned long long)pvis);
		atomicAdd(&P.counters[2], (unsigned long long)svis);
	}
}

}

static void volume_rect(RenderParams &P)
{
	const float *v = P.u + U_VIEW;
	const double m[3][3] = {{v[0], v[4], v[8]}, {v[1], v[5], v[9]}, {v[2], v[6], v[10]}};
	const double det = m[0][0] * (m[1][1] * m[2][2] - m[1][2] * m[2][1]) - m[0][1] * (m[1][0] * m[2][2] - m[1][2] * m[2][0]) +
	                   m[0][2] * (m[1][0] * m[2][1] - m[1][1] * m[2][0]);
	const double aspect = (double)P.u[U_WINDOW] / (double)P.u[U_WINDOW + 1];
	double lo_x = 1e30, hi_x = -1e30, lo_y = 1e30, hi_y = -1e30;
	bool whole = !(fabs(det) > 1e-12) || !(aspect > 0.0);
	for (int c = 0; c < 8 && !whole; c++)
	{
		const double d[3] = {(c & 1 ? 0.5 : -0.5) - v[12], (c & 2 ? 0.5 : -0.5) - v[13], (c & 4 ? 0.5 : -0.5) - v[14]};
		double q[3];
		for (int k = 0; k < 3; k++)
		{
			double t[3][3];
			for (int i = 0; i < 3; i++)
				for (int j = 0; j < 3; j++) t[i][j] = j == k ? d[i] : m[i][j];
			q[k] = (t[0][0] * (t[1][1] * t[2][2] - t[1][2] * t[2][1]) - t[0][1] * (t[1][0] * t[2][2] - t[1][2] * t[2][0]) +
			        t[0][2] * (t[1][0] * t[2][1] - t[1][1] * t[2][0])) / det;
		}
		if (!(q[2] < -1e-3)) { whole = true; break; }
		const double vu = 0.5 - 0.5 * P.cot_half_fov * (q[0] / q[2]) / aspect, vv = 0.5 - 0.5 * P.cot_half_fov * (q[1] / q[2]);
		const double x = vu * P.W, y = (1.0 - vv) * P.H;
		lo_x = fmin(lo_x, x); hi_x = fmax(hi_x, x); lo_y = fmin(lo_y, y); hi_y = fmax(hi_y, y);
	}
	if (whole) { lo_x = 0; hi_x = P.W; lo_y = 0; hi_y = P.H; }
	const double x0 = fmax(0.0, floor(lo_x) - 2.0), x1 = fmin((double)P.W, ceil(hi_x) + 2.0);
	const double y0 = fmax((double)P.row0, floor(lo_y) - 2.0), y1 = fmin((double)P.row1, ceil(hi_y) + 2.0);
	if (!(x1 > x0) || !(y1 > y0)) return;
	P.rx0 = ((u32)x0 / 32u) * 32u;
	P.rx1 = (((u32)x1 + 31u) / 32u) * 32u;
	P.ry0 = P.row0 + (((u32)y0 - P.row0) / 16u) * 16u;
	P.ry1 = P.row0 + (((u32)y1 - P.row0 + 15u) / 16u) * 16u;
}

hipError_t launch_render(const RenderLaunch &l, hipStream_t stream)
{
	RenderParams P;
	P.cells = l.cells;
	P.G = l.G;
	P.cols = l.G / 32u;
	P.W = l.W;
	P.H = l.H;
	P.spp = l.spp;
	P.cot_half_fov = (float)(1.0 / tan(37.5 * 3.14159265359 / 180.0));
	for (int i = 0; i < U_LIVE; i++) P.u[i] = l.uniforms[i];
	P.presentation = l.presentation;
	P.light = reinterpret_cast<uint2 *>(l.light);
	P.depth = l.depth;
	P.counters = l.counters;
	P.legacy = l.legacy ? 1u : 0u;
	P.indirect = l.indirect && !l.legacy ? 1u : 0u;
	P.trace = l.trace ? 1u : 0u;
	P.occ = nullptr;
	P.live_box = nullptr;
	P.spread = 0;
	static const int park_env = getenv("CA3D_RENDER_PARK") ? atoi(getenv("CA3D_RENDER_PARK")) : 0;
	P.park = (u32)(park_env > 0 ? park_env : 0);
	P.occ_words = 0;
	P.occ_coarse = 0;
	if (!l.legacy && l.mode != 1 && l.occ)
	{
		const u32 nblocks = P.cols * (l.G >> 3) * (l.G >> 3);
		P.occ_words = (nblocks + 63u) / 64u;
		P.occ_coarse = l.G % 128u == 0 ? 1u : 0u;
		const size_t coarse_words = (nblocks / 64u + 63u) / 64u;
		u32 *box = reinterpret_cast<u32 *>(l.occ + P.occ_words + 1u + coarse_words);
		if (!l.occ_valid)
		{
			hipError_t e = hipMemsetAsync(l.occ + P.occ_words, 0, sizeof(unsigned long long), stream);
			if (e == hipSuccess) e = hipMemsetAsync(box, 0, 6u * sizeof(u32), stream);
			if (e != hipSuccess) return e;
			hipLaunchKernelGGL(ca_occupancy, dim3((nblocks + 255u) / 256u), dim3(256), 0, stream, l.cells, l.occ, l.G, P.cols, nblocks, P.occ_words, box);
			if (l.occ_built) *l.occ_built = true;
			if (P.occ_coarse)
				hipLaunchKernelGGL(ca_occupancy_coarse, dim3((nblocks / 64u + 255u) / 256u), dim3(256), 0, stream, l.occ, l.G, P.cols, nblocks / 64u, P.occ_words);
		}
		P.live_box = box;
		P.occ = l.occ;
	}
	P.row0 = l.row0;
	P.row1 = l.row1 ? l.row1 : l.H;
	P.rx0 = P.rx1 = P.ry0 = P.ry1 = P.outside_only = 0;
	P.bg = P.gx0 = P.gx1 = P.gy0 = P.gy1 = 0;
	const dim3 grid((l.W + 15u) / 16u, (l.mode == 1 ? l.H + 15u : P.row1 - P.row0 + 15u) / 16u);
	if (l.mode == 1)
	{
		FrameParams F;
		F.base = P;
		F.prev_light = reinterpret_cast<const uint2 *>(l.prev_light);
		F.prev_depth = l.prev_depth;
		if (l.bricks && frame_bricks_applies(l.G))
		{
			hipError_t e = launch_render_frame_bricks(&F, l.bricks, l.bricks_valid, stream, l.bricks_built);
			if (e != hipSuccess) return e;
		}
		else hipLaunchKernelGGL(ca_render_frame_packed, grid, dim3(256), 0, stream, F);
	}
	else if (l.sched && !P.indirect && l.counters)
	{
		volume_rect(P);
		const bool one = l.spp == 1;
		const u32 tiles = ((P.rx1 - P.rx0) / (one ? 32u : 16u)) * ((P.ry1 - P.ry0) / (one ? 8u : 4u));
		const bool around = tiles == 0 || P.rx0 > 0 || P.rx1 < l.W || P.ry0 > P.row0 || P.ry1 < P.row1;
		static const bool bg_off = getenv("CA3D_RENDER_BG") && atoi(getenv("CA3D_RENDER_BG")) == 0;
		if (!bg_off && !P.legacy && !(P.u[U_SHOWDEPTH] == 1.0f))
		{
			const double lo[3] = {(double)P.u[U_LIGHT] - 0.005, (double)P.u[U_LIGHT + 1] - 0.005, (double)P.u[U_LIGHT + 2] - 0.005};
			const double hi[3] = {(double)P.u[U_LIGHT] + 0.005, (double)P.u[U_LIGHT + 1] + 0.005, (double)P.u[U_LIGHT + 2] + 0.005};
			PixRect gr;
			if (box_pix_rect(P.u, P.cot_half_fov, P.W, P.H, P.row0, P.row1, lo, hi, gr))
			{
				P.bg = 1u;
				P.gx0 = gr.x0; P.gx1 = gr.x1; P.gy0 = gr.y0; P.gy1 = gr.y1;
			}
		}
		if (P.bg && P.occ && P.live_box) hipLaunchKernelGGL(ca_live_rect, dim3(1), dim3(64), 0, stream, P);
		const bool beside = tiles && l.aux && l.ev_fork && l.ev_join;
		hipStream_t side = beside ? l.aux : stream;
		if (beside)
		{
			hipError_t e = hipEventRecord(l.ev_fork, stream);
			if (e == hipSuccess) e = hipStreamWaitEvent(l.aux, l.ev_fork, 0);
			if (e == hipSuccess && l.after) e = hipStreamWaitEvent(l.aux, l.after, 0);
			if (e != hipSuccess) return e;
		}

		if (tiles)
		{
			int dev = 0, cus = 256;
			if (hipGetDevice(&dev) == hipSuccess) hipDeviceGetAttribute(&cus, hipDeviceAttributeMultiprocessorCount, dev);
			const u32 wgs = min((tiles + 3u) / 4u, (u32)cus * (u32)kSchedWaves);
			const bool streamed = l.stream_scratch && !P.legacy && !P.trace;
			bool stream_sparse = false;
			if (streamed)
			{
				hipError_t e = launch_render_stream(&P, l.stream_scratch, l.W, l.H, l.stream_check, l.bricks, l.bricks_valid, stream, l.bricks_built, l.after, l.walk_share_pct, &stream_sparse);
				if (e != hipSuccess) return e;
			}
			if (one)
			{
				if (!streamed) hipLaunchKernelGGL((ca_render_packed_sched<false, 256, 1, kSchedWaves>), dim3(wgs), dim3(256), 0, stream, P);
				if (P.occ && !stream_sparse) hipLaunchKernelGGL((ca_render_packed_sched<true, 256, 1, kSchedWaves>), dim3(wgs), dim3(256), 0, side, P);
			}
			else
			{
				if (!streamed) hipLaunchKernelGGL((ca_render_packed_sched<false, 64, kSchedChunk, kSchedWaves>), dim3(wgs), dim3(256), 0, stream, P);
				if (P.occ && !stream_sparse) hipLaunchKernelGGL((ca_render_packed_sched<true, 64, kSchedChunk, kSchedWaves>), dim3(wgs), dim3(256), 0, side, P);
			}
		}
		if (!beside && l.after)
		{
			hipError_t e = hipStreamWaitEvent(stream, l.after, 0);
			if (e != hipSuccess) return e;
		}
		P.outside_only = tiles ? 1u : 0u;
		if (P.bg) hipLaunchKernelGGL(ca_render_background, grid, dim3(256), 0, side, P);
		else if (around) hipLaunchKernelGGL(ca_render_packed<false>, grid, dim3(256), 0, side, P);
		if (P.occ && P.live_box)
		{
			int dev = 0, cus = 256;
			if (hipGetDevice(&dev) == hipSuccess) hipDeviceGetAttribute(&cus, hipDeviceAttributeMultiprocessorCount, dev);
			P.spread = 1u;
			hipLaunchKernelGGL(ca_render_packed_spread<true>, dim3((u32)cus * 4u), dim3(256), 0, side, P);
		}
		if (P.occ && around && !P.bg) hipLaunchKernelGGL(ca_render_packed<true>, grid, dim3(256), 0, side, P);
		if (beside)
		{
			hipError_t e = hipEventRecord(l.ev_join, l.aux);
			if (e == hipSuccess) e = hipStreamWaitEvent(stream, l.ev_join, 0);
			if (e != hipSuccess) return e;
		}
	}
	else
	{
		hipLaunchKernelGGL(ca_render_packed<false>, grid, dim3(256), 0, stream, P);
		if (P.occ) hipLaunchKernelGGL(ca_render_packed<true>, grid, dim3(256), 0, stream, P);
	}
	return hipGetLastError();
}

}
```

cellularautomatons3d_amd/csrc/render_device.inc:

```
using u32 = uint32_t;

struct v3
{
	float x, y, z;
};
__device__ __forceinline__ v3 V(float x, float y, float z) { return v3{x, y, z}; }
__device__ __forceinline__ v3 operator+(v3 a, v3 b) { return V(a.x + b.x, a.y + b.y, a.z + b.z); }
__device__ __forceinline__ v3 operator-(v3 a, v3 b) { return V(a.x - b.x, a.y - b.y, a.z - b.z); }
__device__ __forceinline__ v3 operator*(v3 a, v3 b) { return V(a.x * b.x, a.y * b.y, a.z * b.z); }
__device__ __forceinline__ v3 operator*(v3 a, float s) { return V(a.x * s, a.y * s, a.z * s); }
__device__ __forceinline__ float dot3(v3 a, v3 b) { return a.x * b.x + a.y * b.y + a.z * b.z; }
__device__ __forceinline__ float len3(v3 a) { return sqrtf(dot3(a, a)); }
__device__ __forceinline__ v3 norm3(v3 a) { const float l = len3(a); return V(a.x / l, a.y / l, a.z / l); }

enum
{
	U_LIGHT = 0, U_VIEW = 4, U_PROJVIEWINV = 20, U_PREVVIEW = 36, U_PREVPROJVIEWINV = 52, U_WINDOW = 68, U_TIME = 70,
	U_DEPTHSAMPLES = 71, U_SHADOWSAMPLES = 72, U_CELLSIZE = 73, U_SHOWDEPTH = 74, U_TEMPORALALPHA = 75,
	U_REFLECTIVITY = 76, U_ROUGHNESS = 79, U_MATERIALCOLOR = 80, U_GAMMA = 83, U_LIVE = 84
};

struct RenderParams
{
	const u32 *cells;
	u32 G, cols;
	u32 W, H, spp;
	float cot_half_fov;
	float u[U_LIVE];
	u32 *presentation;
	uint2 *light;
	u32 *depth;
	unsigned long long *counters;
	u32 legacy;
	const unsigned long long *occ;
	u32 occ_words;
	u32 occ_coarse;
	u32 row0, row1;
	u32 indirect;
	u32 trace;
	u32 rx0, rx1, ry0, ry1, outside_only;
	const u32 *live_box;
	u32 bg, gx0, gx1, gy0, gy1;
	u32 spread;
	u32 park;
};

constexpr float kPi = 3.14159265359f;
constexpr float kHalf = 0.5f;
constexpr float kOcclusion = 0.0095f;

__device__ __forceinline__ float to_cells(const RenderParams &P, float v)
{
	const float cs = 1.0f / (float)P.G;
	return (P.G & (P.G - 1u)) == 0u ? (v + kHalf) * (float)P.G : (v + kHalf) / cs;
}

__device__ __forceinline__ u32 cell_state(const RenderParams &P, u32 x, u32 y, u32 z)
{
	if (P.legacy)
	{
		if (x >= P.G || y >= P.G || z >= P.G) return 0u;
		return P.cells[(size_t)x + (size_t)y * P.G + (size_t)z * P.G * P.G] == 1u ? 1u : 0u;
	}
	if ((P.G & (P.G - 1u)) == 0u)
	{
		const u32 idx = ((x >> 5) & (P.cols - 1u)) + (y & (P.G - 1u)) * P.cols + (z & (P.G - 1u)) * P.cols * P.G;
		return (P.cells[idx] >> (x & 31u)) & 1u;
	}
	const u32 idx = ((x >> 5) % P.cols) + (y % P.G) * P.cols + (z % P.G) * P.cols * P.G;
	return (P.cells[idx] >> (x & 31u)) & 1u;
}

__device__ __forceinline__ void ray_cube(v3 o, v3 d, v3 center, v3 half, float &tnear, float &tfar)
{
	const v3 inv = V(1.0f / d.x, 1.0f / d.y, 1.0f / d.z);
	const v3 tmin = ((center - half) - o) * inv;
	const v3 tmax = ((center + half) - o) * inv;
	const v3 t1 = V(fminf(tmin.x, tmax.x), fminf(tmin.y, tmax.y), fminf(tmin.z, tmax.z));
	const v3 t2 = V(fmaxf(tmin.x, tmax.x), fmaxf(tmin.y, tmax.y), fmaxf(tmin.z, tmax.z));
	tnear = fmaxf(fmaxf(t1.x, t1.y), t1.z);
	tfar = fminf(fminf(t2.x, t2.y), t2.z);
}

__device__ __forceinline__ void ray_cube_inv(v3 o, v3 inv, v3 center, v3 half, float &tnear, float &tfar)
{
	const v3 tmin = ((center - half) - o) * inv;
	const v3 tmax = ((center + half) - o) * inv;
	const v3 t1 = V(fminf(tmin.x, tmax.x), fminf(tmin.y, tmax.y), fminf(tmin.z, tmax.z));
	const v3 t2 = V(fmaxf(tmin.x, tmax.x), fmaxf(tmin.y, tmax.y), fmaxf(tmin.z, tmax.z));
	tnear = fmaxf(fmaxf(t1.x, t1.y), t1.z);
	tfar = fminf(fminf(t2.x, t2.y), t2.z);
}

__device__ __forceinline__ float sd_box(v3 p, v3 b)
{
	const v3 q = V(fabsf(p.x) - b.x, fabsf(p.y) - b.y, fabsf(p.z) - b.z);
	const v3 m = V(fmaxf(q.x, 0.0f), fmaxf(q.y, 0.0f), fmaxf(q.z, 0.0f));
	return len3(m) + fminf(fmaxf(q.x, fmaxf(q.y, q.z)), 0.0f);
}

__device__ __forceinline__ v3 face_normal(v3 p, v3 origin)
{
	const v3 d = p - origin;
	const v3 a = V(fabsf(d.x), fabsf(d.y), fabsf(d.z));
	const float m = fmaxf(fmaxf(a.x, a.y), a.z);
	v3 n;
	if (a.x == m) n = V(d.x, 0.0f, 0.0f);
	else if (a.y == m) n = V(0.0f, d.y, 0.0f);
	else n = V(0.0f, 0.0f, d.z);
	return norm3(n);
}

__device__ __forceinline__ v3 cell_origin(float cs, int x, int y, int z)
{
	return V((float)x * cs + cs * 0.5f - kHalf, (float)y * cs + cs * 0.5f - kHalf, (float)z * cs + cs * 0.5f - kHalf);
}

__device__ v3 surface_brdf(v3 L, v3 Vd, v3 N, float roughness, v3 albedo, v3 F0)
{
	const v3 Hh = norm3(L + Vd);
	const v3 fL = V(albedo.x / kPi, albedo.y / kPi, albedo.z / kPi);
	const float a2 = roughness * roughness;
	const float NoH = dot3(N, Hh);
	const float NoH2 = NoH * NoH;
	const float f = NoH2 * (a2 - 1.0f) + 1.0f;
	const float D = a2 / (kPi * f * f);
	const float n = roughness + 1.0f;
	const float k = (n * n) / 8.0f;
	const float NoV = fmaxf(0.0f, dot3(N, Vd));
	const float gv = NoV / (NoV * (1.0f - k) + k);
	const float NoL = fmaxf(0.0f, dot3(N, L));
	const float gl = NoL / (NoL * (1.0f - k) + k);
	const float Gm = gv * gl;
	const float p = powf(1.0f - dot3(Hh, Vd), 5.0f);
	const v3 F = V(F0.x + (1.0f - F0.x) * p, F0.y + (1.0f - F0.y) * p, F0.z + (1.0f - F0.z) * p);
	const float denom = 4.0f * dot3(Vd, N) * dot3(L, N);
	return V(fL.x + (D * Gm * F.x) / denom, fL.y + (D * Gm * F.y) / denom, fL.z + (D * Gm * F.z) / denom);
}

__device__ v3 lighting_from(const RenderParams &P, v3 p, v3 origin, u32 cx, u32 cy, v3 eye, v3 incident, v3 light_pos)
{
	const float *u = P.u;
	const v3 N = face_normal(p, origin);
	const float Gf = (float)P.G;
	const float cxn = (float)cx / Gf, cyn = (float)cy / Gf;
	v3 albedo = V(cxn, cyn, 1.0f - cxn);
	if (u[U_MATERIALCOLOR] != 0.0f || u[U_MATERIALCOLOR + 1] != 0.0f || u[U_MATERIALCOLOR + 2] != 0.0f)
		albedo = V(u[U_MATERIALCOLOR], u[U_MATERIALCOLOR + 1], u[U_MATERIALCOLOR + 2]);
	const v3 Vd = norm3(eye - p);
	const v3 L = norm3(light_pos - p);
	const v3 F0 = V(u[U_REFLECTIVITY], u[U_REFLECTIVITY + 1], u[U_REFLECTIVITY + 2]);
	const v3 brdf = surface_brdf(L, Vd, N, u[U_ROUGHNESS], albedo, F0);
	const float LoN = dot3(L, N);
	return V(fmaxf(0.0f, brdf.x * incident.x * LoN), fmaxf(0.0f, brdf.y * incident.y * LoN), fmaxf(0.0f, brdf.z * incident.z * LoN));
}

__device__ __forceinline__ bool occ_skip_enabled(const RenderParams &P)
{
	if (!P.occ) return false;
	const unsigned long long set = P.occ[P.occ_words];
	return set * 4ull < (unsigned long long)P.cols * (P.G >> 3) * (P.G >> 3);
}

__device__ __forceinline__ bool misses_live_box(const RenderParams &P, v3 o, v3 d)
{
	if (!P.live_box) return false;
	const u32 x1 = P.live_box[0], x0 = ~P.live_box[1], y1 = P.live_box[2], y0 = ~P.live_box[3], z1 = P.live_box[4], z0 = ~P.live_box[5];
	if (x0 >= x1) return true;
	const float cs = 1.0f / (float)P.G;
	const v3 lo = V((float)x0 * cs - kHalf - cs, (float)y0 * cs - kHalf - cs, (float)z0 * cs - kHalf - cs);
	const v3 hi = V((float)x1 * cs - kHalf + cs, (float)y1 * cs - kHalf + cs, (float)z1 * cs - kHalf + cs);
	float tn, tf;
	ray_cube(o, d, V(0.5f * (lo.x + hi.x), 0.5f * (lo.y + hi.y), 0.5f * (lo.z + hi.z)), V(0.5f * (hi.x - lo.x), 0.5f * (hi.y - lo.y), 0.5f * (hi.z - lo.z)), tn, tf);
	return tn > tf || tf < 0.0f;
}

__device__ __forceinline__ bool live_box_small(const RenderParams &P)
{
	if (!P.live_box) return false;
	const u32 x1 = P.live_box[0], x0 = ~P.live_box[1], y1 = P.live_box[2], y0 = ~P.live_box[3], z1 = P.live_box[4], z0 = ~P.live_box[5];
	if (x0 >= x1) return true;
	return (unsigned long long)(x1 - x0) * (y1 - y0) * (z1 - z0) * 8ull < (unsigned long long)P.G * P.G * P.G;
}

__device__ __forceinline__ bool block_occupied(const RenderParams &P, int ix, int iy, int iz)
{
	const int bk = (ix >> 5) + ((iy >> 3) + (iz >> 3) * ((int)P.G >> 3)) * (int)P.cols;
	return (P.occ[bk >> 6] >> (bk & 63)) & 1ull;
}

__device__ __forceinline__ bool coarse_occupied(const RenderParams &P, int ix, int iy, int iz)
{
	const int ck = (ix >> 7) + ((iy >> 5) + (iz >> 5) * ((int)P.G >> 5)) * ((int)P.cols >> 2);
	return (P.occ[P.occ_words + 1u + (u32)(ck >> 6)] >> (ck & 63)) & 1ull;
}

template <int LX, int LY, int LZ>
__device__ __forceinline__ bool block_jump(const RenderParams &P, v3 start, v3 dir, v3 inv, float tmax, int &ix, int &iy, int &iz, float &t,
                                           float &tx, float &ty, float &tz)
{
	constexpr int BX = 1 << LX, BY = 1 << LY, BZ = 1 << LZ;
	const int G = (int)P.G;
	const float cs = 1.0f / (float)P.G, big = 3.0e38f;
	const int sx = dir.x > 0.0f ? 1 : -1, sy = dir.y > 0.0f ? 1 : -1, sz = dir.z > 0.0f ? 1 : -1;
	const int bx0 = ix & ~(BX - 1), by0 = iy & ~(BY - 1), bz0 = iz & ~(BZ - 1);
	const float tex = dir.x != 0.0f ? (((float)(sx > 0 ? bx0 + BX : bx0) * cs - kHalf) - start.x) * inv.x : big;
	const float tey = dir.y != 0.0f ? (((float)(sy > 0 ? by0 + BY : by0) * cs - kHalf) - start.y) * inv.y : big;
	const float tez = dir.z != 0.0f ? (((float)(sz > 0 ? bz0 + BZ : bz0) * cs - kHalf) - start.z) * inv.z : big;
	const bool mx = tex <= tey && tex <= tez, my = !mx && tey <= tez;
	const float te = mx ? tex : (my ? tey : tez);
	if (te >= tmax) return false;
	const v3 p = start + dir * te;
	int nx = min(max((int)floorf(to_cells(P, p.x)), bx0), bx0 + BX - 1);
	int ny = min(max((int)floorf(to_cells(P, p.y)), by0), by0 + BY - 1);
	int nz = min(max((int)floorf(to_cells(P, p.z)), bz0), bz0 + BZ - 1);
	if (mx) nx = sx > 0 ? bx0 + BX : bx0 - 1;
	else if (my) ny = sy > 0 ? by0 + BY : by0 - 1;
	else nz = sz > 0 ? bz0 + BZ : bz0 - 1;
	if ((u32)nx >= (u32)G || (u32)ny >= (u32)G || (u32)nz >= (u32)G) return false;
	ix = nx; iy = ny; iz = nz;
	t = te;
	tx = dir.x != 0.0f ? (((float)(ix + (sx > 0 ? 1 : 0)) * cs - kHalf) - start.x) * inv.x : big;
	ty = dir.y != 0.0f ? (((float)(iy + (sy > 0 ? 1 : 0)) * cs - kHalf) - start.y) * inv.y : big;
	tz = dir.z != 0.0f ? (((float)(iz + (sz > 0 ? 1 : 0)) * cs - kHalf) - start.z) * inv.z : big;
	return true;
}

__device__ __forceinline__ bool live_box_clip(const RenderParams &P, v3 start, v3 dir, v3 inv, float t0, float &tmax, int &ix, int &iy, int &iz,
                                              float &t, float &tx, float &ty, float &tz)
{
	const int G = (int)P.G;
	const float cs = 1.0f / (float)P.G, big = 3.0e38f;
	const u32 bx1 = P.live_box[0], bx0 = ~P.live_box[1], by1 = P.live_box[2], by0 = ~P.live_box[3], bz1 = P.live_box[4], bz0 = ~P.live_box[5];
	if (bx0 >= bx1) return false;
	const v3 lo = V((float)bx0 * cs - kHalf - cs, (float)by0 * cs - kHalf - cs, (float)bz0 * cs - kHalf - cs);
	const v3 hi = V((float)bx1 * cs - kHalf + cs, (float)by1 * cs - kHalf + cs, (float)bz1 * cs - kHalf + cs);
	float bn, bf;
	ray_cube_inv(start, inv, V(0.5f * (lo.x + hi.x), 0.5f * (lo.y + hi.y), 0.5f * (lo.z + hi.z)), V(0.5f * (hi.x - lo.x), 0.5f * (hi.y - lo.y), 0.5f * (hi.z - lo.z)), bn, bf);
	if (bn > bf || bf < t0) return false;
	if (bf < tmax) tmax = bf;
	if (bn > t0 + cs)
	{
		if (bn >= tmax) return false;
		const int sx = dir.x > 0.0f ? 1 : -1, sy = dir.y > 0.0f ? 1 : -1, sz = dir.z > 0.0f ? 1 : -1;
		const v3 q = start + dir * bn;
		ix = min(max((int)floorf(to_cells(P, q.x)), 0), G - 1);
		iy = min(max((int)floorf(to_cells(P, q.y)), 0), G - 1);
		iz = min(max((int)floorf(to_cells(P, q.z)), 0), G - 1);
		t = bn;
		tx = dir.x != 0.0f ? (((float)(ix + (sx > 0 ? 1 : 0)) * cs - kHalf) - start.x) / dir.x : big;
		ty = dir.y != 0.0f ? (((float)(iy + (sy > 0 ? 1 : 0)) * cs - kHalf) - start.y) / dir.y : big;
		tz = dir.z != 0.0f ? (((float)(iz + (sz > 0 ? 1 : 0)) * cs - kHalf) - start.z) / dir.z : big;
	}
	return true;
}

struct GlobalWords
{
	__device__ __forceinline__ u32 operator()(const RenderParams &P, int key) const { return P.cells[key]; }
};

template <bool SHADOW, bool SKIP, class Fetch>
__device__ __forceinline__ bool walk_from(const RenderParams &P, v3 start, v3 dir, float t0, float tmax, v3 half, int sx0, int sy0, int sz0,
                                          float &tnear_out, u32 &visits, const Fetch &fetch)
{
	const int G = (int)P.G;
	const float cs = 1.0f / (float)P.G;
	const v3 p = start + dir * t0;
	int ix = (int)floorf(to_cells(P, p.x)), iy = (int)floorf(to_cells(P, p.y)), iz = (int)floorf(to_cells(P, p.z));
	ix = min(max(ix, 0), G - 1);
	iy = min(max(iy, 0), G - 1);
	iz = min(max(iz, 0), G - 1);
	const int sx = dir.x > 0.0f ? 1 : -1, sy = dir.y > 0.0f ? 1 : -1, sz = dir.z > 0.0f ? 1 : -1;
	const float big = 3.0e38f;
	float tx = dir.x != 0.0f ? (((float)(ix + (sx > 0 ? 1 : 0)) * cs - kHalf) - start.x) / dir.x : big;
	float ty = dir.y != 0.0f ? (((float)(iy + (sy > 0 ? 1 : 0)) * cs - kHalf) - start.y) / dir.y : big;
	float tz = dir.z != 0.0f ? (((float)(iz + (sz > 0 ? 1 : 0)) * cs - kHalf) - start.z) / dir.z : big;
	const float dx = dir.x != 0.0f ? cs / fabsf(dir.x) : big, dy = dir.y != 0.0f ? cs / fabsf(dir.y) : big,
	            dz = dir.z != 0.0f ? cs / fabsf(dir.z) : big;
	float t = t0;
	const v3 inv = V(1.0f / dir.x, 1.0f / dir.y, 1.0f / dir.z);
	if (SKIP && P.live_box && !live_box_clip(P, start, dir, inv, t0, tmax, ix, iy, iz, t, tx, ty, tz)) return false;
	u32 word = 0;
	int wkey = -1, okey = -1;
	for (int guard = 0; guard < 3 * G + 3; guard++)
	{
		if (t >= tmax) return false;
		visits++;
		if (SKIP)
		{
			const int bk = (ix >> 5) + ((iy >> 3) + (iz >> 3) * (G >> 3)) * (int)P.cols;
			if (bk != okey)
			{
				if (P.occ_coarse && !coarse_occupied(P, ix, iy, iz))
				{
					if (!block_jump<7, 5, 5>(P, start, dir, inv, tmax, ix, iy, iz, t, tx, ty, tz)) return false;
					continue;
				}
				if (!block_occupied(P, ix, iy, iz))
				{
					if (!block_jump<5, 3, 3>(P, start, dir, inv, tmax, ix, iy, iz, t, tx, ty, tz)) return false;
					continue;
				}
				okey = bk;
			}
		}
		bool alive;
		if (P.legacy) alive = P.cells[(size_t)ix + ((size_t)iy + (size_t)iz * G) * G] == 1u;
		else
		{
			const int key = (ix >> 5) + (iy + iz * G) * (int)P.cols;
			if (key != wkey) { word = fetch(P, key); wkey = key; }
			alive = (word >> (ix & 31)) & 1u;
		}
		if (alive)
		{
			if (!(SHADOW && ix == sx0 && iy == sy0 && iz == sz0))
			{
				float tn, tf;
				ray_cube_inv(start, inv, cell_origin(cs, ix, iy, iz), half, tn, tf);
				if (SHADOW ? (tn <= tf && tn >= 0.0f)  : (tf >= 0.0f && tn <= tf) )
				{
					tnear_out = tn;
					return true;
				}
			}
		}
		const bool mx = tx <= ty && tx <= tz, my = !mx && ty <= tz, mz = !mx && !my;
		t = mx ? tx : (my ? ty : tz);
		tx += mx ? dx : 0.0f;
		ty += my ? dy : 0.0f;
		tz += mz ? dz : 0.0f;
		ix += mx ? sx : 0;
		iy += my ? sy : 0;
		iz += mz ? sz : 0;
// ... 69 lines not shown
		const v3 final_point = hit ? enter + dir * tnear : exitp;
		s.depth = len3(final_point - cam);
		if (TracerKnowsMiss<Tracer>::value) return s;
		const v3 p = cam + ray * s.depth;
		const v3 f = V(floorf(to_cells(P, p.x)), floorf(to_cells(P, p.y)), floorf(to_cells(P, p.z)));
		const v3 origin = V(f.x * cs + cs * 0.5f - kHalf, f.y * cs + cs * 0.5f - kHalf, f.z * cs + cs * 0.5f - kHalf);
		const int cx = (int)f.x, cy = (int)f.y, cz = (int)f.z;
		const u32 st = cell_state(P, (u32)cx, (u32)cy, (u32)cz);
		const float dist = sd_box(p - origin, vhalf);
		if (st == 1u && !(dist > 0.001f))
		{
			const v3 light_pos = V(u[U_LIGHT], u[U_LIGHT + 1], u[U_LIGHT + 2]);
			const v3 ldir = norm3(light_pos - p);
			float vn, vf;
			ray_cube(p, ldir, V(0.0f, 0.0f, 0.0f), half, vn, vf);
			const v3 vexit = p + ldir * vf;
			const v3 sseg = vexit - p;
			const v3 sdir = norm3(sseg);
			const float slen = len3(sseg);
			const bool occluded = tr.shadow(P, p, sdir, slen, vhalf, cx, cy, cz);
			if (Tracer::kStopAfterShadow) return s;
			const float occ = occluded ? (P.legacy ? 0.095f : kOcclusion) : 1.0f;
			if (P.legacy)
			{
				const v3 N = face_normal(p, origin);
				const float Gf = (float)P.G;
				const v3 colr = V(f.x / Gf, f.y / Gf, 1.0f - f.x / Gf);
				const v3 view_dir = norm3(p - cam);
				const float dl = len3(light_pos - p), dc = len3(cam - p);
				const float fl = fmaxf(1.0f, powf(dl, 2.0f)), fc = fmaxf(1.0f, powf(dc, 2.0f));
				const float incident = u[U_LIGHT + 3] / fl;
				const v3 inc_dir = norm3(p - light_pos);
				const float ndi = dot3(N, inc_dir);
				const v3 refl = V(inc_dir.x - 2.0f * ndi * N.x, inc_dir.y - 2.0f * ndi * N.y, inc_dir.z - 2.0f * ndi * N.z);
				const float reflected = incident * dot3(refl, V(-view_dir.x, -view_dir.y, -view_dir.z));
				s.r = occ * ((colr.x * reflected + incident * colr.x) / fc);
				s.g = occ * ((colr.y * reflected + incident * colr.y) / fc);
				s.b = occ * ((colr.z * reflected + incident * colr.z) / fc);
				s.a = occ;
				s.shadow_ray = 1u;
			}
			else
			{
			const v3 N = face_normal(p, origin);
			const float Gf = (float)P.G;
			const float cxn = (float)(u32)cx / Gf, cyn = (float)(u32)cy / Gf;
			v3 albedo = V(cxn, cyn, 1.0f - cxn);
			if (u[U_MATERIALCOLOR] != 0.0f || u[U_MATERIALCOLOR + 1] != 0.0f || u[U_MATERIALCOLOR + 2] != 0.0f)
				albedo = V(u[U_MATERIALCOLOR], u[U_MATERIALCOLOR + 1], u[U_MATERIALCOLOR + 2]);
			const v3 Vd = norm3(cam - p);
			const v3 L = norm3(light_pos - p);
			const v3 F0 = V(u[U_REFLECTIVITY], u[U_REFLECTIVITY + 1], u[U_REFLECTIVITY + 2]);
			const v3 brdf = surface_brdf(L, Vd, N, u[U_ROUGHNESS], albedo, F0);
			const float mag = u[U_LIGHT + 3];
			const float LoN = dot3(L, N);
			s.r = occ * fmaxf(0.0f, brdf.x * mag * LoN);
			s.g = occ * fmaxf(0.0f, brdf.y * mag * LoN);
			s.b = occ * fmaxf(0.0f, brdf.z * mag * LoN);
			s.shadow_ray = 1u;
			if (P.indirect)
			{
				int ox[4], oy[4], oz[4];
				if (N.x != 0.0f) { const int sx = N.x < 0.0f ? -1 : 1; ox[0] = ox[1] = ox[2] = ox[3] = sx; oy[0] = 1; oy[1] = -1; oy[2] = oy[3] = 0; oz[0] = oz[1] = 0; oz[2] = 1; oz[3] = -1; }
				else if (N.y != 0.0f) { const int sy = N.y < 0.0f ? -1 : 1; oy[0] = oy[1] = oy[2] = oy[3] = sy; ox[0] = -1; ox[1] = 1; ox[2] = ox[3] = 0; oz[0] = oz[1] = 0; oz[2] = 1; oz[3] = -1; }
				else { const int sz = N.z < 0.0f ? -1 : 1; oz[0] = oz[1] = oz[2] = oz[3] = sz; ox[0] = ox[1] = 0; ox[2] = -1; ox[3] = 1; oy[0] = 1; oy[1] = -1; oy[2] = oy[3] = 0; }
				for (int i = 0; i < 4; i++)
				{
					const u32 nx = (u32)(cx + ox[i]), ny = (u32)(cy + oy[i]), nz = (u32)(cz + oz[i]);
					if (!cell_state(P, nx, ny, nz)) continue;
					const v3 norigin = V((float)nx * cs + cs * 0.5f - kHalf, (float)ny * cs + cs * 0.5f - kHalf, (float)nz * cs + cs * 0.5f - kHalf);
					const v3 ndir = V((float)ox[i], (float)oy[i], (float)oz[i]);
					float qn, qf;
					ray_cube(p, ndir, norigin, vhalf, qn, qf);
					if (!(qn <= qf && qf >= 0.0f)) continue;
					const v3 np = p + ndir * qn;
					const v3 nl = norm3(light_pos - np);
					float wn, wf;
					ray_cube(np, nl, V(0.0f, 0.0f, 0.0f), half, wn, wf);
					const v3 nseg = (np + nl * wf) - np;
					const bool nocc = tr.shadow(P, np, norm3(nseg), len3(nseg), vhalf, (int)nx, (int)ny, (int)nz);
					const v3 refl = lighting_from(P, np, norigin, nx, ny, p, V(mag, mag, mag), light_pos) * (nocc ? kOcclusion : 1.0f);
					const v3 ind = lighting_from(P, p, origin, (u32)cx, (u32)cy, cam, refl, np);
					s.r += ind.x; s.g += ind.y; s.b += ind.z;
				}
			}
			}
		}
		s.r = fminf(fmaxf(s.r, 0.0f), 1.0f);
		s.g = fminf(fmaxf(s.g, 0.0f), 1.0f);
		s.b = fminf(fmaxf(s.b, 0.0f), 1.0f);
		s.a = fminf(fmaxf(s.a, 0.0f), 1.0f);
	}
	{
		const v3 light_pos = V(u[U_LIGHT], u[U_LIGHT + 1], u[U_LIGHT + 2]);
		float ln, lf;
		ray_cube(cam, ray, light_pos, V(0.005f, 0.005f, 0.005f), ln, lf);
		if (ln <= lf && lf >= 0.0f && s.r == 0.0f && s.g == 0.0f && s.b == 0.0f) { s.r = s.g = s.b = 1.0f; s.a = 1.0f; }
	}
	if (u[U_SHOWDEPTH] == 1.0f && vu < 0.5f) { s.r = s.depth; s.g = 0.0f; s.b = 0.0f; s.a = 1.0f; }
	return s;
}

struct MissTracer
{
	static constexpr bool kSkipBox = false, kStopAfterPrimary = false, kStopAfterShadow = false;
	__device__ __forceinline__ bool primary(const RenderParams &, v3, v3, v3, v3, float, v3, float &) { return false; }
	__device__ __forceinline__ bool shadow(const RenderParams &, v3, v3, float, v3, int, int, int) { return false; }
};
template <>
struct TracerKnowsMiss<MissTracer>
{
	static constexpr bool value = true;
};

struct PixRect
{
	u32 x0, x1, y0, y1;
};
__host__ __device__ inline bool box_pix_rect(const float *u, float cot_half_fov, u32 W, u32 H, u32 row0, u32 row1, const double lo[3], const double hi[3], PixRect &r)
{
	const float *v = u + U_VIEW;
	const double m[3][3] = {{v[0], v[4], v[8]}, {v[1], v[5], v[9]}, {v[2], v[6], v[10]}};
	const double det = m[0][0] * (m[1][1] * m[2][2] - m[1][2] * m[2][1]) - m[0][1] * (m[1][0] * m[2][2] - m[1][2] * m[2][0]) +
	                   m[0][2] * (m[1][0] * m[2][1] - m[1][1] * m[2][0]);
	const double aspect = (double)u[U_WINDOW] / (double)u[U_WINDOW + 1];
	r.x0 = r.x1 = r.y0 = r.y1 = 0u;
	if (!(fabs(det) > 1e-12) || !(aspect > 0.0)) return false;
	double lo_x = 1e30, hi_x = -1e30, lo_y = 1e30, hi_y = -1e30;
	int behind = 0;
	for (int c = 0; c < 8; c++)
	{
		const double d[3] = {(c & 1 ? hi[0] : lo[0]) - v[12], (c & 2 ? hi[1] : lo[1]) - v[13], (c & 4 ? hi[2] : lo[2]) - v[14]};
		const double q0 = (d[0] * (m[1][1] * m[2][2] - m[1][2] * m[2][1]) - m[0][1] * (d[1] * m[2][2] - m[1][2] * d[2]) + m[0][2] * (d[1] * m[2][1] - m[1][1] * d[2])) / det;
		const double q1 = (m[0][0] * (d[1] * m[2][2] - m[1][2] * d[2]) - d[0] * (m[1][0] * m[2][2] - m[1][2] * m[2][0]) + m[0][2] * (m[1][0] * d[2] - d[1] * m[2][0])) / det;
		const double q2 = (m[0][0] * (m[1][1] * d[2] - d[1] * m[2][1]) - m[0][1] * (m[1][0] * d[2] - d[1] * m[2][0]) + d[0] * (m[1][0] * m[2][1] - m[1][1] * m[2][0])) / det;
		if (q2 > 1e-3) { behind++; continue; }
		if (!(q2 < -1e-3)) return false;
		const double vu = 0.5 - 0.5 * cot_half_fov * (q0 / q2) / aspect, vv = 0.5 - 0.5 * cot_half_fov * (q1 / q2);
		const double x = vu * W, y = (1.0 - vv) * H;
		lo_x = fmin(lo_x, x); hi_x = fmax(hi_x, x); lo_y = fmin(lo_y, y); hi_y = fmax(hi_y, y);
	}
	if (behind == 8) return true;
	if (behind) return false;
	const double x0 = fmax(0.0, floor(lo_x) - 2.0), x1 = fmin((double)W, ceil(hi_x) + 2.0);
	const double y0 = fmax((double)row0, floor(lo_y) - 2.0), y1 = fmin((double)row1, ceil(hi_y) + 2.0);
	if (!(x1 > x0) || !(y1 > y0)) return true;
	r.x0 = ((u32)x0 / 16u) * 16u;
	r.x1 = (((u32)x1 + 15u) / 16u) * 16u;
	r.y0 = row0 + (((u32)y0 - row0) / 16u) * 16u;
	r.y1 = row0 + (((u32)y1 - row0 + 15u) / 16u) * 16u;
	return true;
}

__device__ inline bool live_box_pix_rect(const RenderParams &P, PixRect &r)
{
	r.x0 = r.x1 = r.y0 = r.y1 = 0u;
	if (!P.live_box) return false;
	const u32 x1 = P.live_box[0], x0 = ~P.live_box[1], y1 = P.live_box[2], y0 = ~P.live_box[3], z1 = P.live_box[4], z0 = ~P.live_box[5];
	if (x0 >= x1) return true;
	{
		const u32 G = P.G;
		const u32 xa = ((0x7FFFFFFu % P.cols) << 5) + 31u, ya = 0xFFFFFFFFu % G;
		const u32 sx[3] = {0u, G - 1u, xa}, syz[3] = {0u, G - 1u, ya};
		for (int k = 0; k < 3; k++)
			if ((sx[k] >= x0 && sx[k] < x1) || (syz[k] >= y0 && syz[k] < y1) || (syz[k] >= z0 && syz[k] < z1)) return false;
	}
	const double cs = 1.0 / (double)P.G;
	const double lo[3] = {(double)x0 * cs - 0.5 - 2.0 * cs, (double)y0 * cs - 0.5 - 2.0 * cs, (double)z0 * cs - 0.5 - 2.0 * cs};
	const double hi[3] = {(double)x1 * cs - 0.5 + 2.0 * cs, (double)y1 * cs - 0.5 + 2.0 * cs, (double)z1 * cs - 0.5 + 2.0 * cs};
	return box_pix_rect(P.u, P.cot_half_fov, P.W, P.H, P.row0, P.row1, lo, hi, r);
}
__device__ __forceinline__ bool in_pix_rect(const PixRect &r, u32 x, u32 y) { return x >= r.x0 && x < r.x1 && y >= r.y0 && y < r.y1; }
__device__ __forceinline__ bool live_rect_load(const RenderParams &P, PixRect &r)
{
	const u32 *w = reinterpret_cast<const u32 *>(P.counters + 4);
	r.x0 = w[1] & 0xFFFFu; r.x1 = w[1] >> 16; r.y0 = w[2] & 0xFFFFu; r.y1 = w[2] >> 16;
	return w[0] == 1u;
}

template <bool SKIP>
__device__ Sample shade_sample(const RenderParams &P, float vu, float vv, u32 &pvis, u32 &svis)
{
	WalkTracer<SKIP> tr{pvis, svis};
	return shade_sample_with(P, vu, vv, tr);
}

__device__ __forceinline__ u32 unorm8(float x) { return (u32)__float2int_rn(fminf(fmaxf(x, 0.0f), 1.0f) * 255.0f); }

struct FrameParams
{
	RenderParams base;
	const uint2 *prev_light;
	const u32 *prev_depth;
};

__device__ __forceinline__ float fract1(float x) { return x - floorf(x); }

__device__ __attribute__((unused)) float n1rand(const RenderParams &P, float u, float v)
{
	const float t = 0.07f * fract1(P.u[U_TIME]);
	const float d = (t + u) * 12.9898f + (t + v) * 78.233f;
	const float s = (float)sin((double)d);
	return fract1(s * 43758.5453f);
}

__device__ __forceinline__ u32 f2u(float f) { return !(f >= 0.0f) ? 0u : (f >= 4294967296.0f ? 0xFFFFFFFFu : (u32)f); }

__device__ __attribute__((unused)) void reprojected_uv(const RenderParams &P, v3 p, float &ux, float &uy)
{
	const float *m = P.u + U_PREVPROJVIEWINV;
	const float q0 = m[0] * p.x + m[4] * p.y + m[8] * p.z + m[12];
	const float q1 = m[1] * p.x + m[5] * p.y + m[9] * p.z + m[13];
	const float q3 = m[3] * p.x + m[7] * p.y + m[11] * p.z + m[15];
	const float cx = q0 / q3, cy = q1 / q3;
	ux = cx * 0.5f + 0.5f;
	uy = -cy * 0.5f + 0.5f;
}

__device__ __attribute__((unused)) bool texel_xy(const RenderParams &P, float fx, float fy, size_t &idx)
{
	if (!(fx == fx) || !(fy == fy)) return false;
	if (fx <= -1.0f || fy <= -1.0f || fx >= (float)P.W || fy >= (float)P.H) return false;
	const int x = (int)fx, y = (int)fy;
	if (x < 0 || y < 0 || x >= (int)P.W || y >= (int)P.H) return false;
	idx = (size_t)y * P.W + (size_t)x;
	return true;
}

struct CellU
{
	v3 origin;
	u32 x, y, z, idx;
};

__device__ __attribute__((unused)) CellU cell_u(const RenderParams &P, v3 p)
{
	const float cs = 1.0f / (float)P.G;
	const v3 f = V(floorf(to_cells(P, p.x)), floorf(to_cells(P, p.y)), floorf(to_cells(P, p.z)));
	CellU r;
	r.origin = V(f.x * cs + cs * 0.5f - kHalf, f.y * cs + cs * 0.5f - kHalf, f.z * cs + cs * 0.5f - kHalf);
	r.x = f2u(f.x); r.y = f2u(f.y); r.z = f2u(f.z);
	r.idx = r.x + r.y * P.G + r.z * (u32)((float)P.G * (float)P.G);
	return r;
}
```

cellularautomatons3d_amd/csrc/render_stream.hip:

```cpp
#include <hip/hip_fp16.h>

#include <cstdio>
#include <vector>

#include "ca3d_internal.h"

namespace ca3d
{
namespace
{

#include "render_device.inc"

constexpr u32 kNoHit = 0xFFFFFFFFu;
constexpr u32 kUnanswered = 0x5A5A5A5Au;
enum : unsigned char { kOcclNone = 0, kOcclHit = 1, kOcclPending = 2 };

constexpr int kStatSlots = 64;

struct StreamParams
{
	RenderParams R;
	u32 *hit;
	unsigned char *occl;
// ... 809 lines not shown
					w.tx += mx ? w.dx : 0.0f;
					w.ty += my ? w.dy : 0.0f;
					w.tz += mz ? w.dz : 0.0f;
					w.pos = npos;
					cur = nxt;
					st = hit ? 1 : ((leaving || tmin >= w.tmax) ? 2 : 0);
				}
				walking = __builtin_popcountll(__builtin_amdgcn_ballot_w64(st == 0));
			} while (walking > leave_at);
			if (st != 3) term = st;
		}
		else if (SKIP)
		{
			do
			{
				visits += (u32)walking;
				if (job >= 0 && term == 0)
				{
					int empty = 0;
					const int bk = (w.ix >> 5) + ((w.iy >> 3) + (w.iz >> 3) * ((int)P.G >> 3)) * (int)P.cols;
					const int key = word_key<LAYOUT>(S, w.ix, w.iy, w.iz);
					const u32 cur = *reinterpret_cast<const u32 *>(reinterpret_cast<const char *>(S.volume) + ((u32)key << 2));
					if (bk != okey)
					{
						const int ck = (w.ix >> 7) + ((w.iy >> 5) + (w.iz >> 5) * ((int)P.G >> 5)) * ((int)P.cols >> 2);
						const unsigned long long fw = P.occ[bk >> 6];
						const unsigned long long cw = P.occ_coarse ? P.occ[P.occ_words + 1u + (u32)(ck >> 6)] : ~0ull;
						if (!((cw >> (ck & 63)) & 1ull)) empty = 1;
						else if (!((fw >> (bk & 63)) & 1ull)) empty = 2;
						else okey = bk;
					}
					if (empty)
					{
						const v3 start = V(ctx[0 * stride], ctx[1 * stride], ctx[2 * stride]), inv = V(ctx[3 * stride], ctx[4 * stride], ctx[5 * stride]), dir = V(ctx[6 * stride], ctx[7 * stride], ctx[8 * stride]);
						const bool on = empty == 1 ? block_jump<7, 5, 5>(P, start, dir, inv, w.tmax, w.ix, w.iy, w.iz, w.t, w.tx, w.ty, w.tz)
						                           : block_jump<5, 3, 3>(P, start, dir, inv, w.tmax, w.ix, w.iy, w.iz, w.t, w.tx, w.ty, w.tz);
						if (!on) term = 2;
						exempt = false;
					}
					else term = walk_cell_word<SHADOW, LAYOUT, CHECK>(S, w, cur, exempt, vhalf, k0, k1, eps_a, ctx, stride);
				}
				walking = __builtin_amdgcn_readfirstlane(__popcll(__ballot(job >= 0 && term == 0)));
			} while (walking > leave_at);
		}
		else
		{
			do
			{
				const int key = word_key<LAYOUT>(S, w.ix, w.iy, w.iz);
				visits += (u32)walking;
				if (job >= 0 && term == 0) term = walk_cell<SHADOW, LAYOUT, CHECK>(S, w, key, exempt, vhalf, k0, k1, eps_a, ctx, stride);
				walking = __builtin_amdgcn_readfirstlane(__popcll(__ballot(job >= 0 && term == 0)));
			} while (walking > leave_at);
		}
	}
	if (S.trace && lane == 0)
	{
		unsigned long long *t = S.trace + 8ull * ((SHADOW ? gridDim.x * (u32)kW2Waves : 0u) + blockIdx.x * (u32)kW2Waves + (u32)wave);
		t[0] = tr_t0; t[1] = __builtin_amdgcn_s_memrealtime(); t[2] = tr_rounds; t[3] = 0; t[4] = 0; t[5] = tr_refill; t[6] = tr_jobs; t[7] = 0;
	}
	if (lane == 0 && visits) atomicAdd(&S.ctl[16 + 4 * ((blockIdx.x * (u32)kW2Waves + (u32)wave) % kStatSlots) + (SHADOW ? 2 : 1)], visits);
}

__global__ __launch_bounds__(256) void ca_stream_shadow_rays(StreamParams S)
{
	const RenderParams &P = S.R;
	if (!stream_owns_frame(S)) return;
	const u32 j = blockIdx.x * 256u + threadIdx.x;
	const u32 lj = 2u * S.lb + job_shift(P);
	const u32 c = j >> lj;
	bool lit = false;
	if (c < S.chunks)
	{
		u32 px, py, k;
		job_pixel(S, c, j & ((1u << lj) - 1u), px, py, k);
		unsigned char flag = kOcclNone;
		if (px < P.W && py < P.row1)
		{
			float vu, vv;
			sample_uv(P, px, py, k, vu, vv);
			LookupPrimaryRecordShadow tr;
			tr.answer = S.hit[j];
			shade_sample_with(P, vu, vv, tr);
			if (S.check && tr.unanswered) { atomicAdd(&S.ctl[3], 1u); atomicMax(&S.ctl[4], ~j); atomicMax(&S.ctl[5], j); }
			if (tr.lit)
			{
				S.rays[j] = make_float4(tr.p.x, tr.p.y, tr.p.z, 0.0f);
				flag = kOcclPending;
				lit = true;
			}
		}
		S.occl[j] = flag;
	}
	const u32 n = (u32)__popcll(__ballot(lit));
	if ((threadIdx.x & 63u) == 0u && n) atomicAdd(&S.ctl[16 + 4 * (blockIdx.x % kStatSlots) + 0], n);
}

__global__ __launch_bounds__(256) void ca_stream_resolve(StreamParams S)
{
	const RenderParams &P = S.R;
	if (!stream_owns_frame(S)) return;
	if (blockIdx.x == 0 && threadIdx.x < 3u && P.counters)
	{
		unsigned long long sum = 0;
		for (int s = 0; s < kStatSlots; s++) sum += S.ctl[16 + 4 * s + threadIdx.x];
		if (sum) atomicAdd(&P.counters[threadIdx.x], sum);
	}
	const u32 sh = job_shift(P);
	const u32 n = blockIdx.x * 256u + threadIdx.x;
	const u32 lj = 2u * S.lb + sh;
	const u32 c = (n << sh) >> lj;
	if (c >= S.chunks) return;
	u32 px, py, k0;
	job_pixel(S, c, (n << sh) & ((1u << lj) - 1u), px, py, k0);
	if (px >= P.W || py >= P.row1) return;
	float r = 0.0f, g = 0.0f, b = 0.0f, a = 0.0f, d0 = 0.0f;
	for (u32 k = 0; k < P.spp; k++)
	{
		const u32 j = (n << sh) + k;
		float vu, vv;
		sample_uv(P, px, py, k, vu, vv);
		LookupBoth tr;
		tr.answer = S.hit[j];
		tr.occl = S.occl + j;
		const Sample s = shade_sample_with(P, vu, vv, tr);
		if (S.check && tr.unanswered) atomicAdd(&S.ctl[3], 1u);
		r += s.r; g += s.g; b += s.b; a += s.a;
		if (k == 0) d0 = s.depth;
	}
	const float inv = 1.0f / (float)P.spp;
	r *= inv; g *= inv; b *= inv; a *= inv;
	const size_t i = (size_t)py * P.W + px;
	if (P.light)
	{
		const __half2 rg = __floats2half2_rn(r, g), ba = __floats2half2_rn(b, 1.0f);
		uint2 v;
		v.x = *reinterpret_cast<const u32 *>(&rg);
		v.y = *reinterpret_cast<const u32 *>(&ba);
		P.light[i] = v;
	}
	if (P.depth)
	{
		const __half2 d = __floats2half2_rn(d0, 1.0f);
		P.depth[i] = *reinterpret_cast<const u32 *>(&d);
	}
	if (P.presentation)
	{
		const float ig = 1.0f / P.u[U_GAMMA];
		P.presentation[i] = unorm8(powf(r, ig)) | (unorm8(powf(g, ig)) << 8) | (unorm8(powf(b, ig)) << 16) | (unorm8(a) << 24);
	}
}

template <int LAYOUT, bool CHECK>
void launch_walks2(const StreamParams &S, u32 wgs2, u32 job_blocks, hipStream_t stream)
{
	constexpr int PS = kBricksReadAny;
	hipLaunchKernelGGL((ca_stream_walk2<false, LAYOUT, CHECK>), dim3(wgs2), dim3(kW2Threads), 0, stream, S);
	if (S.skip_ok) hipLaunchKernelGGL((ca_stream_walk2<false, PS, CHECK, true>), dim3(wgs2), dim3(kW2Threads), 0, stream, S);
	hipLaunchKernelGGL(ca_stream_shadow_rays, dim3(job_blocks), dim3(256), 0, stream, S);
	hipLaunchKernelGGL((ca_stream_walk2<true, LAYOUT, CHECK>), dim3(wgs2), dim3(kW2Threads), 0, stream, S);
	if (S.skip_ok) hipLaunchKernelGGL((ca_stream_walk2<true, PS, CHECK, true>), dim3(wgs2), dim3(kW2Threads), 0, stream, S);
}

}

size_t stream_scratch_bytes(uint32_t W, uint32_t H, uint32_t spp, size_t *hit_off, size_t *occl_off, size_t *rays_off)
{
	const size_t jobs = (size_t)((W + 31u) / 32u * 32u) * ((H + 15u) / 16u * 16u) * spp;
	size_t off = 4096;
	*hit_off = off; off += jobs * 4u;
	*occl_off = off; off += (jobs + 255u) / 256u * 256u;
	*rays_off = off; off += jobs * 16u;
	return off;
}

hipError_t launch_render_stream(const void *params, void *scratch, uint32_t W, uint32_t H, bool check, uint32_t *bricks, bool bricks_valid, hipStream_t stream, bool *bricks_built, hipEvent_t before_resolve, int walk_share_pct, bool *sparse_too)
{
	StreamParams S;
	S.R = *static_cast<const RenderParams *>(params);
	const RenderParams &P = S.R;
	size_t hit_off, occl_off, rays_off;
	stream_scratch_bytes(W, H, P.spp, &hit_off, &occl_off, &rays_off);
	char *base = static_cast<char *>(scratch);
	S.ctl = reinterpret_cast<u32 *>(base);
	S.hit = reinterpret_cast<u32 *>(base + hit_off);
	S.occl = reinterpret_cast<unsigned char *>(base + occl_off);
	S.rays = reinterpret_cast<float4 *>(base + rays_off);
	static const int qmap_env = getenv("CA3D_STREAM_QMAP") ? atoi(getenv("CA3D_STREAM_QMAP")) : 0;
	S.lb = P.spp == 4u ? 3u : 4u;
	S.qmap = qmap_env == 1 || !getenv("CA3D_STREAM_QMAP") ? 1u : 0u;
	const u32 edge = 1u << S.lb;
	S.chunks_x = (P.rx1 - P.rx0) / edge;
	S.chunks = S.chunks_x * ((P.ry1 - P.ry0) / edge);
	const u32 per = P.spp << (2u * S.lb);
	const bool p2 = (P.G & (P.G - 1u)) == 0u;
	S.lg = S.lc = 0;
	S.nb = P.G >> 3;
	S.lnbp = 0;
	while ((1u << S.lnbp) < S.nb) S.lnbp++;
	if (p2)
	{
		while ((1u << S.lg) < P.G) S.lg++;
		S.lc = S.lg - 5u;
	}
	static const char *trace_path = getenv("CA3D_STREAM_TRACE");
	static unsigned long long *trace_buf = nullptr;
	const size_t trace_words = 8u * 2u * 4u * 256u * 8u * 2u;
	if (trace_path && !trace_buf && hipMalloc((void **)&trace_buf, trace_words * 8u) != hipSuccess) trace_buf = nullptr;
	S.trace = trace_path ? trace_buf : nullptr;
	if (S.trace) hipMemsetAsync(S.trace, 0, trace_words * 8u, stream);
	S.check = check ? 1u : 0u;
	if (check)
	{
		hipMemsetAsync(S.hit, 0x5A, (size_t)S.chunks * per * 4u, stream);
		hipMemsetAsync(S.occl, 0x5A, (size_t)S.chunks * per, stream);
	}
	hipError_t e = hipMemsetAsync(S.ctl, 0, 4096, stream);
	if (e != hipSuccess) return e;
	int dev = 0, cus = 256;
	if (hipGetDevice(&dev) == hipSuccess) hipDeviceGetAttribute(&cus, hipDeviceAttributeMultiprocessorCount, dev);
	const u32 job_blocks = (S.chunks * per + 255u) / 256u;
	const bool bricked = bricks && frame_bricks_applies(P.G);
	S.volume = bricked ? bricks : P.cells;
	if (bricked && !bricks_valid)
	{
		hipError_t eb = launch_brick_volume(P.cells, bricks, P.G, stream);
		if (eb != hipSuccess) return eb;
		if (bricks_built) *bricks_built = true;
	}
	static const int pop_env = getenv("CA3D_STREAM_POP") ? atoi(getenv("CA3D_STREAM_POP")) : 0;
	S.pop_at = pop_env >= 1 && pop_env <= 64 ? pop_env : 16;
	static const int tb_env = getenv("CA3D_STREAM_TAIL_BATCH") ? atoi(getenv("CA3D_STREAM_TAIL_BATCH")) : 1;
	S.tail_batch = tb_env == 2 ? 2 : (tb_env ? 1 : 0);
	static const int wgs_env = getenv("CA3D_STREAM_WGS_PCT") ? atoi(getenv("CA3D_STREAM_WGS_PCT")) : 0;
	const u32 pct = (u32)(wgs_env >= 10 && wgs_env <= 100 ? wgs_env : (walk_share_pct >= 10 && walk_share_pct <= 100 ? walk_share_pct : 100));
	const u32 wgs2 = max(8u, min(S.chunks, (u32)cus * (u32)kW2PerSimd * 4u / (u32)kW2Waves * pct / 100u));
	static const int skip_env = getenv("CA3D_STREAM_SKIP") ? atoi(getenv("CA3D_STREAM_SKIP")) : 1;
	S.skip_ok = bricked && skip_env && P.occ ? 1u : 0u;
	if (sparse_too) *sparse_too = S.skip_ok != 0u;
	static const int packed_env = getenv("CA3D_STREAM_PACKED") ? atoi(getenv("CA3D_STREAM_PACKED")) : 1;
	const bool packed = bricked && packed_env && P.G <= 1024u && (unsigned long long)S.chunks * per < (1ull << 28);
	void (*walks)(const StreamParams &, u32, u32, hipStream_t);
	if (packed) walks = check ? launch_walks2<kBricksPacked, true> : launch_walks2<kBricksPacked, false>;
	else if (bricked && p2) walks = check ? launch_walks2<kBricksRead, true> : launch_walks2<kBricksRead, false>;
	else if (bricked) walks = check ? launch_walks2<kBricksReadAny, true> : launch_walks2<kBricksReadAny, false>;
	else if (p2) walks = check ? launch_walks2<kRowsP2, true> : launch_walks2<kRowsP2, false>;
	else walks = check ? launch_walks2<kRowsAny, true> : launch_walks2<kRowsAny, false>;
	walks(S, wgs2, job_blocks, stream);
	const unsigned long long trace_waves = (unsigned long long)wgs2 * (unsigned)kW2Waves;
	if (before_resolve)
	{
		hipError_t ew = hipStreamWaitEvent(stream, before_resolve, 0);
		if (ew != hipSuccess) return ew;
	}
	hipLaunchKernelGGL(ca_stream_resolve, dim3((S.chunks * (per / P.spp) + 255u) / 256u), dim3(256), 0, stream, S);
	if (S.trace)
	{
		std::vector<unsigned long long> t(trace_words);
		if (hipStreamSynchronize(stream) == hipSuccess && hipMemcpy(t.data(), S.trace, trace_words * 8u, hipMemcpyDeviceToHost) == hipSuccess)
			if (FILE *f = fopen(trace_path, "wb"))
			{
				const unsigned long long n = trace_waves;
				fwrite(&n, 8, 1, f);
				fwrite(t.data(), 8, (size_t)n * 16u, f);
				fclose(f);
			}
	}
	return hipGetLastError();
}

}
```

cellularautomatons3d_amd/engine.py:

```python
from __future__ import annotations

import ctypes as C
from dataclasses import dataclass
from typing import Optional, Sequence, Tuple

import numpy as np

from . import _capi, host
from ._capi import Ca3dError, Info, RenderStats, Stats

_u32p = C.POINTER(C.c_uint32)
_i32p = C.POINTER(C.c_int32)


def _as_u32(a) -> np.ndarray:
    return np.ascontiguousarray(a, dtype=np.uint32)


def _as_i32(a) -> np.ndarray:
    return np.ascontiguousarray(a, dtype=np.int32)


@dataclass
class Summary:
# ... 93 lines not shown
        spec = _seed_spec(self.grid_size, seed, and_rounds, box)
        _capi.check(self._lib.ca3d_seed_state(self._h, C.byref(spec)))

    def read_state(self) -> np.ndarray:
        out = np.empty(self.info().state_words, dtype=np.uint32)
        _capi.check(self._lib.ca3d_read_state(self._h, out.ctypes.data_as(_u32p), out.size))
        return out

    def save_checkpoint(self, path) -> None:
        i = self.info()
        host.save_checkpoint(path, self.read_state(), i.grid_size, i.step, i.layout)

    def load_checkpoint(self, path) -> int:
        words, grid_size, step, layout = host.load_checkpoint(path)
        self.configure(grid_size, layout)
        self.upload_state(words)
        return step

    def step(self, n_steps: int = 1) -> None:
        _capi.check(self._lib.ca3d_step(self._h, n_steps))

    compute_pass = step

    def flush(self) -> None:
        _capi.check(self._lib.ca3d_flush(self._h))

    def summary(self, planes: bool = False) -> Summary:
        st = _capi.SummaryStruct()
        pp = np.empty(self.info().nz, dtype=np.uint32) if planes else None
        _capi.check(self._lib.ca3d_summarize(self._h, C.byref(st), pp.ctypes.data_as(_u32p) if planes else None))
        return _summary(st, pp)

    def summary_gpu_ms(self) -> float:
        v = C.c_double()
        _capi.check(self._lib.ca3d_get_summary_time(self._h, C.byref(v)))
        return float(v.value)

    def step_until(self, max_steps: int, check_every: int = 8, extinct: bool = True, still: bool = True):
        st = _capi.SummaryStruct()
        done, reason = C.c_uint32(), C.c_uint32()
        mask = (STOP_EXTINCT if extinct else 0) | (STOP_STILL if still else 0)
        _capi.check(self._lib.ca3d_step_until(self._h, max_steps, check_every, mask, C.byref(st), C.byref(done), C.byref(reason)))
        return int(done.value), int(reason.value), _summary(st, None)

    def step_until_cycle(self, max_steps: int, check_every: int = 8, extinct: bool = True, still: bool = True, periodic: bool = True):
        st = _capi.SummaryStruct()
        done, reason, period = C.c_uint32(), C.c_uint32(), C.c_uint32()
        mask = (STOP_EXTINCT if extinct else 0) | (STOP_STILL if still else 0) | (STOP_PERIODIC if periodic else 0)
        _capi.check(self._lib.ca3d_step_until_cycle(self._h, max_steps, check_every, mask, C.byref(st), C.byref(done), C.byref(reason),
                                                    C.byref(period)))
        return int(done.value), int(reason.value), int(period.value), _summary(st, None)

    def slab_step(self, n_steps: int) -> None:
        _capi.check(self._lib.ca3d_slab_step(self._h, n_steps))

    def slab_step_phase(self, n_steps: int, phase: int) -> None:
        _capi.check(self._lib.ca3d_slab_step_phase(self._h, n_steps, phase))

    def slab_region(self, region: int):
        p, n = C.c_void_p(), C.c_size_t()
        _capi.check(self._lib.ca3d_slab_region(self._h, region, C.byref(p), C.byref(n)))
        return int(p.value), int(n.value)

    @staticmethod
    def comm_unique_id() -> bytes:
        buf = C.create_string_buffer(_capi.COMM_ID_BYTES)
        _capi.check(_capi.load().ca3d_comm_unique_id(buf))
        return buf.raw

    def slab_comm_init(self, unique_id: bytes, rank: int, world: int) -> None:
        if len(unique_id) != _capi.COMM_ID_BYTES:
            raise ValueError("the communicator id holds 128 bytes")
        _capi.check(self._lib.ca3d_slab_comm_init(self._h, C.c_char_p(unique_id), rank, world))

    def slab_run(self, n_steps: int, overlap: bool = False) -> None:
        _capi.check(self._lib.ca3d_slab_run(self._h, n_steps, 1 if overlap else 0))

    def slab_exchange(self) -> None:
        _capi.check(self._lib.ca3d_slab_exchange(self._h))

    def comm_info(self) -> dict:
        ci = _capi.CommInfo()
        _capi.check(self._lib.ca3d_slab_comm_info(self._h, C.byref(ci)))
        return {"device": int(ci.device), "pci_bus_id": ci.pci_bus_id.decode(), "comm_ranks": int(ci.comm_ranks),
                "comm_rank": int(ci.comm_rank), "comm_device": int(ci.comm_device)}

    def slab_gather(self, full: "Engine") -> None:
        _capi.check(self._lib.ca3d_slab_gather(self._h, full._h))

    def render_target(self, which: int = 0):
        p, n = C.c_void_p(), C.c_size_t()
        _capi.check(self._lib.ca3d_render_target(self._h, which, C.byref(p), C.byref(n)))
        return int(p.value), int(n.value)

    def device_buffer(self, which: int):
        p, n = C.c_void_p(), C.c_size_t()
        _capi.check(self._lib.ca3d_device_buffer(self._h, which, C.byref(p), C.byref(n)))
        return int(p.value), int(n.value)

    def synchronize(self) -> None:
        _capi.check(self._lib.ca3d_synchronize(self._h))

    def recovered_launches(self) -> int:
        n = C.c_uint32()
        _capi.check(self._lib.ca3d_recovered_launches(self._h, C.byref(n)))
        return int(n.value)

    def measure_copy(self, n_bytes: int = 1 << 30, reps: int = 8) -> float:
        v = C.c_double()
        _capi.check(self._lib.ca3d_measure_copy(self._h, n_bytes, reps, C.byref(v)))
        return float(v.value)

    def set_stream(self, hip_stream: int) -> None:
        _capi.check(self._lib.ca3d_set_stream(self._h, C.c_void_p(int(hip_stream))))

    def use_own_stream(self) -> None:
        _capi.check(self._lib.ca3d_use_own_stream(self._h))

    def set_option(self, name: str, value: int) -> None:
        _capi.check(self._lib.ca3d_set_option(self._h, name.encode(), int(value)))

    def render(self, uniforms, width: int, height: int, spp: int = 1, readback: bool = True, rows=None):
        u = np.ascontiguousarray(uniforms, dtype=np.float32)
        if u.size != 128:
            raise ValueError("the common uniform block holds 128 floats")
        up = u.ctypes.data_as(C.POINTER(C.c_float))
        self.set_option("render_row_begin", rows[0] if rows else 0)
        self.set_option("render_row_end", rows[1] if rows else 0)
        if not readback:
            _capi.check(self._lib.ca3d_render(self._h, up, width, height, spp, None, None, None))
            return None
        pres = np.empty((height, width, 4), dtype=np.uint8)
        light = np.empty((height, width, 4), dtype=np.float16)
        depth = np.empty((height, width, 2), dtype=np.float16)
        _capi.check(self._lib.ca3d_render(self._h, up, width, height, spp, pres.ctypes.data, light.ctypes.data, depth.ctypes.data))
        return pres, light, depth

    def set_render_mode(self, literal_frame: bool) -> None:
        self.set_option("render_mode", 1 if literal_frame else 0)

    def reset_render_history(self) -> None:
        self.set_option("render_reset_history", 1)

    def render_stats(self) -> RenderStats:
        s = RenderStats()
        _capi.check(self._lib.ca3d_get_render_stats(self._h, C.byref(s)))
        return s

    def render_pipeline(self) -> int:
        n = C.c_int32(0)
        _capi.check(self._lib.ca3d_get_render_pipeline(self._h, C.byref(n)))
        return int(n.value)

    def info(self) -> Info:
        i = Info()
        _capi.check(self._lib.ca3d_get_info(self._h, C.byref(i)))
        return i

    def jit_log(self) -> str:
        need = C.c_size_t()
        _capi.check(self._lib.ca3d_get_jit_log(self._h, None, 0, C.byref(need)))
        buf = C.create_string_buffer(max(1, need.value))
        _capi.check(self._lib.ca3d_get_jit_log(self._h, buf, len(buf), None))
        return buf.value.decode("utf-8", "replace")

    def kernel_variant(self) -> str:
        need = C.c_size_t()
        _capi.check(self._lib.ca3d_get_kernel_variant(self._h, None, 0, C.byref(need)))
        buf = C.create_string_buffer(max(1, need.value))
        _capi.check(self._lib.ca3d_get_kernel_variant(self._h, buf, len(buf), None))
        return buf.value.decode("utf-8", "replace")

    def stats(self) -> Stats:
        s = Stats()
        _capi.check(self._lib.ca3d_get_stats(self._h, C.byref(s)))
        return s


class EngineGroup:

    def __init__(self, devices: Sequence[int]):
        self._lib = _capi.load()
        d = (C.c_int * len(devices))(*[int(x) for x in devices])
        h = C.c_void_p()
        _capi.check(self._lib.ca3d_group_create(d, len(devices), C.byref(h)))
        self._h = h
        self.devices = list(devices)
        self.grid_size = 0

    def close(self) -> None:
        if getattr(self, "_h", None):
            self._lib.ca3d_group_destroy(self._h)
            self._h = None

    def __enter__(self):
        return self

    def __exit__(self, *exc):
        self.close()

    def __del__(self):
        try:
            self.close()
        except Exception:
            pass

    def configure(self, grid_size: int, ghost: int, layout: int = _capi.LAYOUT_PACKED32) -> None:
        _capi.check(self._lib.ca3d_group_configure(self._h, grid_size, layout, ghost))
        self.grid_size = grid_size

    def set_rules(self, main_offsets, edges_offsets, corners_offsets, survive, born) -> None:
        m, e, c = _as_i32(main_offsets), _as_i32(edges_offsets), _as_i32(corners_offsets)
        s, b = _as_u32(survive), _as_u32(born)
        _capi.check(self._lib.ca3d_group_set_rules(self._h, m.ctypes.data_as(_i32p), m.size, e.ctypes.data_as(_i32p), e.size,
                                                   c.ctypes.data_as(_i32p), c.size, s.ctypes.data_as(_u32p), b.ctypes.data_as(_u32p)))

    def set_rule_strings(self, neighbourhood: str = host.DEFAULTS["neighbourhood"], born: str = host.DEFAULTS["bornRulesString"],
                         survive: str = host.DEFAULTS["surviveRulesString"], born_edges: str = "27", survive_edges: str = "27",
                         born_corners: str = "27", survive_corners: str = "27") -> None:
        b, s = host.recalculate_rules_values(born, survive, born_edges, survive_edges, born_corners, survive_corners)
        self.set_rules(host.NEIGHBOURHOOD_MAP[neighbourhood], host.NEIGHBOURHOOD_MAP["edges"], host.NEIGHBOURHOOD_MAP["corners"], s, b)

    def upload_state(self, words) -> None:
        w = _as_u32(words).ravel()
        _capi.check(self._lib.ca3d_group_upload_state(self._h, w.ctypes.data_as(_u32p), w.size))
        self._words = w.size

    def seed_state(self, seed: int, and_rounds: int = 0, box=None) -> None:
        spec = _seed_spec(self.grid_size, seed, and_rounds, box)
        _capi.check(self._lib.ca3d_group_seed_state(self._h, C.byref(spec)))
        e = C.c_void_p()
        _capi.check(self._lib.ca3d_group_engine(self._h, 0, C.byref(e)))
        i = Info()
        _capi.check(self._lib.ca3d_get_info(e, C.byref(i)))
        self._words = int(i.state_words) * len(self.devices)

    def read_state(self) -> np.ndarray:
        out = np.empty(self._words, dtype=np.uint32)
        _capi.check(self._lib.ca3d_group_read_state(self._h, out.ctypes.data_as(_u32p), out.size))
        return out

    def step(self, n_steps: int = 1) -> None:
        _capi.check(self._lib.ca3d_group_step(self._h, n_steps))

    def synchronize(self) -> None:
        _capi.check(self._lib.ca3d_group_synchronize(self._h))

    def summary(self, planes: bool = False) -> Summary:
        st = _capi.SummaryStruct()
        pp = np.empty(self.grid_size, dtype=np.uint32) if planes else None
        _capi.check(self._lib.ca3d_group_summarize(self._h, C.byref(st), pp.ctypes.data_as(_u32p) if planes else None))
        return _summary(st, pp)

    def set_option(self, name: str, value: int) -> None:
        _capi.check(self._lib.ca3d_group_set_option(self._h, name.encode(), int(value)))

    def kernel_name(self, rank: int = 0) -> str:
        e = C.c_void_p()
        _capi.check(self._lib.ca3d_group_engine(self._h, rank, C.byref(e)))
        i = Info()
        _capi.check(self._lib.ca3d_get_info(e, C.byref(i)))
        return i.kernel_name.decode()

    def render(self, uniforms, width: int, height: int, spp: int = 1, readback: bool = True):
        u = np.ascontiguousarray(uniforms, dtype=np.float32)
        up = u.ctypes.data_as(C.POINTER(C.c_float))
        if not readback:
            _capi.check(self._lib.ca3d_group_render(self._h, up, width, height, spp, None, None, None))
            return None
        pres = np.empty((height, width, 4), dtype=np.uint8)
        light = np.empty((height, width, 4), dtype=np.float16)
        depth = np.empty((height, width, 2), dtype=np.float16)
        _capi.check(self._lib.ca3d_group_render(self._h, up, width, height, spp, pres.ctypes.data, light.ctypes.data, depth.ctypes.data))
        return pres, light, depth
```

include/ca3d.h:

```cpp
#ifndef CA3D_H
#define CA3D_H

#include <stddef.h>
#include <stdint.h>

#ifdef __cplusplus
extern "C" {
#endif

#define CA3D_ABI_VERSION 7
#define CA3D_LUT_LEN 81

typedef struct ca3d_engine ca3d_t;

enum ca3d_status
{
	CA3D_OK = 0,
	CA3D_ERR_INVALID_ARGUMENT = -1,
	CA3D_ERR_NOT_CONFIGURED = -2,
	CA3D_ERR_DEVICE = -3,
	CA3D_ERR_OUT_OF_MEMORY = -4,
	CA3D_ERR_UNSUPPORTED = -5
};

// ... 194 lines not shown
};
int ca3d_ensemble_census_connected(ca3d_ensemble_t *e, uint32_t first, uint32_t count, uint32_t max_components, uint32_t connectivity,
                                   ca3d_component *out , uint32_t *n_components ,
                                   uint32_t *remaining , float *gpu_ms );
int ca3d_ensemble_isolate_connected(ca3d_ensemble_t *dst, uint32_t dst_first, ca3d_ensemble_t *src, uint32_t n_jobs, const ca3d_isolate_job *jobs,
                                    uint32_t flags, uint32_t connectivity, ca3d_isolated *out ,
                                    float *gpu_ms );
typedef struct ca3d_compose_part
{
	uint32_t universe;
	uint32_t orientation;
	int32_t at[3];
	uint32_t reserved;
} ca3d_compose_part;
typedef struct ca3d_composed
{
	uint32_t population;
	uint32_t placed;
	uint32_t overlap;
	uint32_t clipped;
} ca3d_composed;
#define CA3D_COMPOSE_OVER 0x1u
#define CA3D_COMPOSE_COPY_RULES 0x100u
#define CA3D_COMPOSE_MAX_PARTS (1u << 20)
int ca3d_ensemble_compose(ca3d_ensemble_t *dst, uint32_t dst_first, uint32_t n_dst, ca3d_ensemble_t *src, const ca3d_compose_part *parts,
                          const uint32_t *part_begin , uint32_t flags, ca3d_composed *out ,
                          float *gpu_ms );
typedef struct ca3d_canon
{
	uint64_t key;
	uint64_t symmetry;
	uint32_t orientation;
	uint32_t population;
	uint32_t box_min, box_max;
} ca3d_canon;
int ca3d_ensemble_canon(ca3d_ensemble_t *e, uint32_t first, uint32_t count, ca3d_canon *out ,
                        uint64_t *digests , float *gpu_ms );
#define CA3D_CANON_CLOSED 1u
#define CA3D_CANON_MAX_PERIOD 4096u
typedef struct ca3d_canon_period
{
	uint64_t key;
	uint64_t symmetry;
	uint32_t orientation;
	uint32_t phase;
	uint32_t population;
	uint32_t flags_shift;
} ca3d_canon_period;
int ca3d_ensemble_canon_period(ca3d_ensemble_t *e, uint32_t first, uint32_t count, const uint32_t *periods ,
                               ca3d_canon_period *out , uint64_t *keys ,
                               uint32_t keys_stride, float *gpu_ms );
#define CA3D_ENVELOPE_RETURNS 1u
#define CA3D_ENVELOPE_IMAGE_ENVELOPE 1u
#define CA3D_ENVELOPE_IMAGE_STATOR 2u
#define CA3D_ENVELOPE_IMAGE_ROTOR 4u
#define CA3D_ENVELOPE_COPY_RULES 0x100u
typedef struct ca3d_envelope
{
	uint32_t period;
	uint32_t flags;
	uint32_t heat;
	uint32_t population_sum;
	uint32_t envelope_population;
	uint32_t stator_population;
	uint8_t envelope_min[4], envelope_max[4];
	uint8_t rotor_min[4], rotor_max[4];
	uint32_t reserved[2];
} ca3d_envelope;
int ca3d_ensemble_envelope(ca3d_ensemble_t *src, uint32_t first, uint32_t count, const uint32_t *periods ,
                           ca3d_ensemble_t *dst , uint32_t dst_first, uint32_t flags,
                           ca3d_envelope *out , float *gpu_ms );
int ca3d_ensemble_synchronize(ca3d_ensemble_t *e);
int ca3d_ensemble_get_stats(ca3d_ensemble_t *e, struct ca3d_stats *out);

typedef struct ca3d_seed
{
	uint32_t seed;
	uint32_t and_rounds;
	uint32_t box_min[3];
	uint32_t box_max[3];
} ca3d_seed;
int ca3d_seed_state(ca3d_t *h, const ca3d_seed *spec);
int ca3d_group_seed_state(ca3d_group_t *g, const ca3d_seed *spec);
int ca3d_ensemble_seed_state(ca3d_ensemble_t *e, uint32_t first, uint32_t count, const ca3d_seed *specs, uint32_t n_specs);
int ca3d_ensemble_set_rule_tables(ca3d_ensemble_t *e, uint32_t first, uint32_t count, const uint32_t *born_masks, const uint32_t *survive_masks,
                                  uint32_t n_masks);

int ca3d_recovered_launches(ca3d_t *h, uint32_t *out_count);

int ca3d_set_stream(ca3d_t *h, void *hip_stream);
int ca3d_use_own_stream(ca3d_t *h);
int ca3d_device_buffer(ca3d_t *h, int which, void **device_ptr, size_t *n_bytes);

typedef struct ca3d_info
{
	uint32_t grid_size;
	int32_t layout;
	uint32_t z0, nz, ghost;
	uint64_t step;
	uint64_t state_words;
	int32_t current_buffer;
	int32_t device;
	char kernel_name[64];
	uint64_t launches_total;
} ca3d_info;
int ca3d_get_info(ca3d_t *h, ca3d_info *out);

int ca3d_get_jit_log(ca3d_t *h, char *buf, size_t n_bytes, size_t *needed);

typedef struct ca3d_jit_stats
{
	uint64_t programs_compiled;
	uint64_t programs_from_disk;
	uint64_t programs_from_memory;
	double compile_ms;
	double disk_read_ms;
	double load_ms;
	char cache_dir[256];
} ca3d_jit_stats;
int ca3d_get_jit_stats(ca3d_jit_stats *out);

int ca3d_get_kernel_variant(ca3d_t *h, char *buf, size_t n_bytes, size_t *needed);

typedef struct ca3d_stats
{
	uint64_t steps;
	uint64_t kernel_launches;
	double gpu_ms;
	double cell_steps;
	double algorithmic_bytes;
} ca3d_stats;
int ca3d_get_stats(ca3d_t *h, ca3d_stats *out);

int ca3d_render(ca3d_t *h, const float uniforms[128], uint32_t width, uint32_t height, uint32_t spp,
                uint8_t *presentation_rgba8, uint16_t *light_rgba16f, uint16_t *depth_rg16f);

int ca3d_measure_copy(ca3d_t *h, size_t n_bytes, uint32_t reps, double *gb_per_s);

typedef struct ca3d_render_stats
{
	double gpu_ms;
	uint64_t primary_rays;
	uint64_t shadow_rays;
	uint64_t primary_cell_visits, shadow_cell_visits;
} ca3d_render_stats;
int ca3d_get_render_stats(ca3d_t *h, ca3d_render_stats *out);

int ca3d_ensemble_render_sheet(ca3d_ensemble_t *e, uint32_t first, uint32_t count, const float uniforms[128], uint32_t tile_w, uint32_t tile_h,
                               uint32_t columns, uint32_t spp, uint8_t *presentation_rgba8, uint16_t *light_rgba16f, uint16_t *depth_rg16f);
int ca3d_ensemble_get_sheet_stats(ca3d_ensemble_t *e, ca3d_render_stats *out);

int ca3d_get_render_pipeline(ca3d_t *h, int32_t *frames_in_flight);

int ca3d_set_option(ca3d_t *h, const char *name, int64_t value);

#ifdef __cplusplus
}
#endif
#endif
```

Before: 60280.

## Classify render frames from cached occupancy facts to skip unneeded launches

After building the occupancy grid, the renderer asynchronously copies the occupied-block count and live bounding box into pinned host memory. On later renders of the same state it reads them back to classify the frame as dense, scattered or small. It then drops kernels that class does not need: dense or sparse walk passes, the live-rect kernel, the side stream, and pipelining for small frames. The change targets rendering only, so the CA step metric should be unaffected, apart from a small risk of wrong output if the cached facts go stale.

Result: slower. 59290 (-1.6%).

```diff
diff --git a/cellularautomatons3d_amd/_capi.py b/cellularautomatons3d_amd/_capi.py
--- a/cellularautomatons3d_amd/_capi.py
+++ b/cellularautomatons3d_amd/_capi.py
@@ -107,6 +107,7 @@
     _fields_ = [("seed", C.c_uint32), ("and_rounds", C.c_uint32), ("box_min", C.c_uint32 * 3), ("box_max", C.c_uint32 * 3)]
 
 
+RENDER_CLASS_UNKNOWN, RENDER_CLASS_DENSE, RENDER_CLASS_SCATTERED, RENDER_CLASS_SMALL = range(4)
 STOP_EXTINCT, STOP_STILL = 1, 2
 STOP_PERIODIC = 4
 STOP_MOVING = 8
@@ -234,6 +235,10 @@
     ("ca3d_set_option", C.c_int, [_H, C.c_char_p, C.c_int64]),
     ("ca3d_render", C.c_int, [_H, C.POINTER(C.c_float), C.c_uint32, C.c_uint32, C.c_uint32, C.c_void_p, C.c_void_p, C.c_void_p]),
     ("ca3d_get_render_pipeline", C.c_int, [_H, C.POINTER(C.c_int32)]),
+    ("ca3d_get_render_class", C.c_int, [_H, C.POINTER(C.c_int32)]),
+    ("ca3d_get_render_launches", C.c_int, [_H, _u32p]),
+    ("ca3d_render_classify", C.c_int, [C.c_uint32, C.c_uint64, _u32p, C.POINTER(C.c_int32)]),
+    ("ca3d_render_facts_usable", C.c_int, [C.POINTER(C.c_uint64), C.POINTER(C.c_uint64), C.c_int, C.c_int, C.POINTER(C.c_int32)]),
     ("ca3d_get_render_stats", C.c_int, [_H, C.POINTER(RenderStats)]),
 ]
 
diff --git a/cellularautomatons3d_amd/csrc/ca3d_api.cpp b/cellularautomatons3d_amd/csrc/ca3d_api.cpp
--- a/cellularautomatons3d_amd/csrc/ca3d_api.cpp
+++ b/cellularautomatons3d_amd/csrc/ca3d_api.cpp
@@ -294,6 +294,8 @@
 	if (h->ev_state) hipEventDestroy(h->ev_state);
 	if (h->r_aux) hipStreamDestroy(h->r_aux);
 	if (h->r_fork) hipEventDestroy(h->r_fork);
+	if (h->r_facts_ev) hipEventDestroy(h->r_facts_ev);
+	if (h->r_facts) hipHostFree(h->r_facts);
 	if (h->r_join) hipEventDestroy(h->r_join);
 	if (h->rev_start) hipEventDestroy(h->rev_start);
 	if (h->rev_stop) hipEventDestroy(h->rev_stop);
@@ -899,6 +901,7 @@
 		return CA3D_OK;
 	}
 	if (!strcmp(name, "render_stream_check")) { h->render_stream_check = value ? 1 : 0; return CA3D_OK; }
+	if (!strcmp(name, "render_class_launch")) { h->render_class_launch = value ? 1 : 0; return CA3D_OK; }
 	if (!strcmp(name, "render_row_begin") || !strcmp(name, "render_row_end"))
 	{
 		if (value < 0 || value > 16384) return fail(CA3D_ERR_INVALID_ARGUMENT, "row %lld is outside any target", (long long)value);
diff --git a/cellularautomatons3d_amd/csrc/ca3d_engine.h b/cellularautomatons3d_amd/csrc/ca3d_engine.h
--- a/cellularautomatons3d_amd/csrc/ca3d_engine.h
+++ b/cellularautomatons3d_amd/csrc/ca3d_engine.h
@@ -112,6 +112,13 @@
 	uint32_t *r_bricks = nullptr;
 	size_t r_bricks_bytes = 0;
 	uint64_t state_serial = 1, r_occ_key[3] = {0, 0, 0}, r_bricks_key[3] = {0, 0, 0};
+	ca3d::RenderFacts *r_facts = nullptr;
+	hipEvent_t r_facts_ev = nullptr;
+	uint64_t r_facts_key[3] = {0, 0, 0};
+	int render_class_launch = 1;
+	int r_last_class = 0;
+	uint32_t r_last_launches = 0;
+	int r_cus = 0;
 	bool buffers_exposed = false;
 	void *r_stream = nullptr;
 	size_t r_stream_bytes = 0;
diff --git a/cellularautomatons3d_amd/csrc/ca3d_internal.h b/cellularautomatons3d_amd/csrc/ca3d_internal.h
--- a/cellularautomatons3d_amd/csrc/ca3d_internal.h
+++ b/cellularautomatons3d_amd/csrc/ca3d_internal.h
@@ -117,6 +117,14 @@
 	const CanonRules *rules;
 	bool binary_state;
 };
+
+enum { kFrameUnknown = 0, kFrameDense = 1, kFrameScattered = 2, kFrameSmall = 3 };
+struct RenderFacts
+{
+	unsigned long long occupied;
+	uint32_t box[6];
+};
+int render_frame_class(uint32_t G, const RenderFacts &facts);
 
 struct RenderLaunch
 {
@@ -145,6 +153,12 @@
 	hipEvent_t after = nullptr;
 	int walk_share_pct = 100;
 	bool stream_check = false;
+	RenderFacts *facts_out = nullptr;
+	hipEvent_t facts_ev = nullptr;
+	const RenderFacts *facts = nullptr;
+	int cus = 0;
+	int *frame_class = nullptr;
+	uint32_t *launches = nullptr;
 };
 
 constexpr uint32_t kSummaryHeaderWords = 16;
@@ -300,7 +314,8 @@
 hipError_t launch_render_frame_bricks(const void *frame_params, uint32_t *bricks, bool bricks_valid, hipStream_t stream, bool *bricks_built = nullptr);
 hipError_t launch_brick_volume(const uint32_t *cells, uint32_t *bricks, uint32_t G, hipStream_t stream);
 hipError_t launch_render_stream(const void *params, void *scratch, uint32_t W, uint32_t H, bool check, uint32_t *bricks, bool bricks_valid, hipStream_t stream, bool *bricks_built = nullptr, hipEvent_t before_resolve = nullptr, int walk_share_pct = 100,
-                                bool *sparse_too = nullptr);
+                                bool *sparse_too = nullptr,
+                                int frame_class = kFrameUnknown, int cus = 0, uint32_t *launches = nullptr);
 
 hipError_t launch_packed_step(const PackedLaunch &l, hipStream_t stream);
 const char *packed_kernel_name(const CanonRules &r, uint32_t G, int variant);
diff --git a/cellularautomatons3d_amd/csrc/ca3d_render.cpp b/cellularautomatons3d_amd/csrc/ca3d_render.cpp
--- a/cellularautomatons3d_amd/csrc/ca3d_render.cpp
+++ b/cellularautomatons3d_amd/csrc/ca3d_render.cpp
@@ -75,8 +75,15 @@
 	unsigned long long *counters = nullptr;
 	uint64_t state_key[3] = {0, 0, 0};
 	bool occ_built = false, bricks_built = false;
+	int frame_class = kFrameUnknown;
+	uint32_t launches = 0;
 	RenderLaunch l;
 };
+
+static bool render_facts_usable(const uint64_t record_key[3], const uint64_t frame_key[3], bool occ_valid, bool landed)
+{
+	return record_key[0] != 0 && !memcmp(record_key, frame_key, 3 * sizeof(uint64_t)) && occ_valid && landed;
+}
 
 static bool frame_pipelined(const ca3d_engine *h, const Frame &f)
 {
@@ -191,7 +198,17 @@
 static int begin_launch(ca3d_engine *h, Frame &f, const float *uniforms)
 {
 	HIP_TRY(hipMemsetAsync(f.counters, 0, (f.trace_path ? f.counter_words : 8u) * sizeof(unsigned long long), f.rs));
+	f.launches++;
 	RenderLaunch &l = f.l;
+	if (!h->r_cus)
+	{
+		int dev = 0, cus = 0;
+		if (hipGetDevice(&dev) == hipSuccess && hipDeviceGetAttribute(&cus, hipDeviceAttributeMultiprocessorCount, dev) == hipSuccess && cus > 0) h->r_cus = cus;
+		else (void)hipGetLastError();
+	}
+	l.cus = h->r_cus;
+	l.frame_class = &f.frame_class;
+	l.launches = &f.launches;
 	l.trace = f.trace_path != nullptr;
 	l.cells = h->buf[h->cur];
 	l.G = h->G;
@@ -210,6 +227,24 @@
 	return CA3D_OK;
 }
 
+static const RenderFacts *landed_facts(ca3d_engine *h, const uint64_t key[3], bool trace)
+{
+	if (!h->render_class_launch || h->buffers_exposed || h->render_stream_check || trace || !h->r_facts) return nullptr;
+	const bool occ_valid = !memcmp(key, h->r_occ_key, 3 * sizeof(uint64_t));
+	if (!render_facts_usable(h->r_facts_key, key, occ_valid, true)) return nullptr;
+	const hipError_t q = hipEventQuery(h->r_facts_ev);
+	if (q != hipSuccess) (void)hipGetLastError();
+	return render_facts_usable(h->r_facts_key, key, occ_valid, q == hipSuccess) ? h->r_facts : nullptr;
+}
+
+static bool known_small_frame(ca3d_engine *h, const Frame &f)
+{
+	if (h->layout != CA3D_LAYOUT_PACKED32 || !h->render_skip) return false;
+	const uint64_t key[3] = {h->state_serial, h->step, (uint64_t)(uintptr_t)h->buf[h->cur]};
+	const RenderFacts *facts = landed_facts(h, key, f.trace_path != nullptr);
+	return facts && render_frame_class(h->G, *facts) == kFrameSmall;
+}
+
 static int prepare_occupancy(ca3d_engine *h, Frame &f)
 {
 	if (!(h->render_skip && h->layout == CA3D_LAYOUT_PACKED32)) return CA3D_OK;
@@ -229,6 +264,16 @@
 	f.l.occ = h->r_occ;
 	f.l.occ_valid = !memcmp(f.state_key, h->r_occ_key, sizeof f.state_key);
 	f.l.occ_built = &f.occ_built;
+	if (!h->r_facts)
+	{
+		HIP_TRY(hipHostMalloc((void **)&h->r_facts, sizeof(RenderFacts), hipHostMallocDefault));
+		memset(h->r_facts, 0, sizeof(RenderFacts));
+		HIP_TRY(hipEventCreateWithFlags(&h->r_facts_ev, hipEventDisableTiming));
+	}
+	f.l.facts_out = h->r_facts;
+	f.l.facts_ev = h->r_facts_ev;
+	if (!f.l.occ_valid) h->r_facts_key[0] = 0;
+	else f.l.facts = landed_facts(h, f.state_key, f.trace_path != nullptr);
 	return CA3D_OK;
 }
 
@@ -284,7 +329,7 @@
 	}
 	l.stream_scratch = scratch;
 	l.stream_check = h->render_stream_check != 0;
-	if (l.stream_check) HIP_TRY(hipMemsetAsync(scratch, 0, 4096, f.rs));
+	if (l.stream_check) { HIP_TRY(hipMemsetAsync(scratch, 0, 4096, f.rs)); f.launches++; }
 	return CA3D_OK;
 }
 
@@ -329,10 +374,13 @@
 	hipError_t e = launch_render(f.l, f.rs);
 	if (e != hipSuccess)
 	{
-		h->r_occ_key[0] = h->r_bricks_key[0] = 0;
+		h->r_occ_key[0] = h->r_bricks_key[0] = h->r_facts_key[0] = 0;
 		return fail(CA3D_ERR_DEVICE, "render launch failed: %s", hipGetErrorString(e));
 	}
 	if (f.occ_built) memcpy(h->r_occ_key, f.state_key, sizeof f.state_key);
+	if (f.occ_built) memcpy(h->r_facts_key, f.state_key, sizeof f.state_key);
+	h->r_last_class = f.frame_class;
+	h->r_last_launches = f.launches;
 	if (f.bricks_built) memcpy(h->r_bricks_key, f.state_key, sizeof f.state_key);
 	HIP_TRY(hipEventRecord(L ? L->stop : h->rev_stop, f.rs));
 	h->rev_valid = true;
@@ -411,9 +459,14 @@
 	f.spp = spp;
 	f.to_host = presentation_rgba8 || light_rgba16f || depth_rg16f;
 	f.trace_path = render_trace_path();
-	const bool pipelined = frame_pipelined(h, f);
+	bool pipelined = frame_pipelined(h, f);
 	int rc = bind_device(h, !pipelined);
 	if (rc) return rc;
+	if (pipelined && known_small_frame(h, f))
+	{
+		pipelined = false;
+		if ((rc = bind_device(h, true))) return rc;
+	}
 	if (f.to_host || (h->res_status_host && *h->res_status_host)) rc = settle_resident(h);
 	if (rc) return rc;
 	if ((rc = size_render_targets(h, f))) return rc;
@@ -461,6 +514,42 @@
 }
 CA3D_API_CATCH
 
+int ca3d_get_render_class(ca3d_t *h, int32_t *frame_class) CA3D_API_TRY
+{
+	if (!h || !frame_class) return fail(CA3D_ERR_INVALID_ARGUMENT, "ca3d_get_render_class: NULL argument");
+	*frame_class = h->r_last_class;
+	return CA3D_OK;
+}
+CA3D_API_CATCH
+
+int ca3d_get_render_launches(ca3d_t *h, uint32_t *launches) CA3D_API_TRY
+{
+	if (!h || !launches) return fail(CA3D_ERR_INVALID_ARGUMENT, "ca3d_get_render_launches: NULL argument");
+	*launches = h->r_last_launches;
+	return CA3D_OK;
+}
+CA3D_API_CATCH
+
+int ca3d_render_classify(uint32_t grid_size, uint64_t occupied_blocks, const uint32_t live_box[6], int32_t *frame_class) CA3D_API_TRY
+{
+	if (!live_box || !frame_class) return fail(CA3D_ERR_INVALID_ARGUMENT, "ca3d_render_classify: NULL argument");
+	if (grid_size < 32u || grid_size % 32u) return fail(CA3D_ERR_INVALID_ARGUMENT, "ca3d_render_classify: the grid size must be a multiple of 32");
+	RenderFacts facts;
+	facts.occupied = occupied_blocks;
+	for (int i = 0; i < 6; i++) facts.box[i] = live_box[i];
+	*frame_class = render_frame_class(grid_size, facts);
+	return CA3D_OK;
+}
+CA3D_API_CATCH
+
+int ca3d_render_facts_usable(const uint64_t record_key[3], const uint64_t frame_key[3], int occupancy_valid, int copy_landed, int32_t *usable) CA3D_API_TRY
+{
+	if (!record_key || !frame_key || !usable) return fail(CA3D_ERR_INVALID_ARGUMENT, "ca3d_render_facts_usable: NULL argument");
+	*usable = render_facts_usable(record_key, frame_key, occupancy_valid != 0, copy_landed != 0) ? 1 : 0;
+	return CA3D_OK;
+}
+CA3D_API_CATCH
+
 int ca3d_get_render_pipeline(ca3d_t *h, int32_t *frames_in_flight) CA3D_API_TRY
 {
 	if (!h || !frames_in_flight) return fail(CA3D_ERR_INVALID_ARGUMENT, "ca3d_get_render_pipeline: NULL argument");
diff --git a/cellularautomatons3d_amd/csrc/render.hip b/cellularautomatons3d_amd/csrc/render.hip
--- a/cellularautomatons3d_amd/csrc/render.hip
+++ b/cellularautomatons3d_amd/csrc/render.hip
@@ -981,8 +981,18 @@
 	P.ry1 = P.row0 + (((u32)y1 - P.row0 + 15u) / 16u) * 16u;
 }
 
+int render_frame_class(uint32_t G, const RenderFacts &facts)
+{
+	BoxWords b;
+	for (int i = 0; i < 6; i++) b.w[i] = facts.box[i];
+	return frame_class_of(facts.occupied, b, G, G / 32u);
+}
+
 hipError_t launch_render(const RenderLaunch &l, hipStream_t stream)
 {
+	uint32_t n_launched = 0;
+	int cls = kFrameUnknown;
+	if (l.frame_class) *l.frame_class = kFrameUnknown;
 	RenderParams P;
 	P.cells = l.cells;
 	P.G = l.G;
@@ -1022,10 +1032,21 @@
 			if (l.occ_built) *l.occ_built = true;
 			if (P.occ_coarse)
 				hipLaunchKernelGGL(ca_occupancy_coarse, dim3((nblocks / 64u + 255u) / 256u), dim3(256), 0, stream, l.occ, l.G, P.cols, nblocks / 64u, P.occ_words);
-		}
+			n_launched += P.occ_coarse ? 4u : 3u;
+			if (l.facts_out && l.facts_ev)
+			{
+				e = hipMemcpyAsync(&l.facts_out->occupied, l.occ + P.occ_words, sizeof(unsigned long long), hipMemcpyDeviceToHost, stream);
+				if (e == hipSuccess) e = hipMemcpyAsync(l.facts_out->box, box, 6u * sizeof(u32), hipMemcpyDeviceToHost, stream);
+				if (e == hipSuccess) e = hipEventRecord(l.facts_ev, stream);
+				if (e != hipSuccess) return e;
+			}
+		}
+		else if (l.facts) cls = render_frame_class(l.G, *l.facts);
 		P.live_box = box;
 		P.occ = l.occ;
 	}
+	if (l.frame_class) *l.frame_class = cls;
+	P.lr_have = P.lrx0 = P.lrx1 = P.lry0 = P.lry1 = 0;
 	P.row0 = l.row0;
 	P.row1 = l.row1 ? l.row1 : l.H;
 	P.rx0 = P.rx1 = P.ry0 = P.ry1 = P.outside_only = 0;
@@ -1043,6 +1064,7 @@
 			if (e != hipSuccess) return e;
 		}
 		else hipLaunchKernelGGL(ca_render_frame_packed, grid, dim3(256), 0, stream, F);
+		n_launched += l.bricks_built && *l.bricks_built ? 2u : 1u;
 	}
 	else if (l.sched && !P.indirect && l.counters)
 	{
@@ -1062,8 +1084,23 @@
 				P.gx0 = gr.x0; P.gx1 = gr.x1; P.gy0 = gr.y0; P.gy1 = gr.y1;
 			}
 		}
-		if (P.bg && P.occ && P.live_box) hipLaunchKernelGGL(ca_live_rect, dim3(1), dim3(64), 0, stream, P);
-		const bool beside = tiles && l.aux && l.ev_fork && l.ev_join;
+		if (P.bg && P.occ && P.live_box)
+		{
+			if (cls != kFrameUnknown)
+			{
+				BoxWords b;
+				for (int i = 0; i < 6; i++) b.w[i] = l.facts->box[i];
+				PixRect lr;
+				P.lr_have = box_words_pix_rect(b, P.G, P.cols, P.u, P.cot_half_fov, P.W, P.H, P.row0, P.row1, lr) ? 1u : 2u;
+				P.lrx0 = lr.x0; P.lrx1 = lr.x1; P.lry0 = lr.y0; P.lry1 = lr.y1;
+			}
+			else { hipLaunchKernelGGL(ca_live_rect, dim3(1), dim3(64), 0, stream, P); n_launched++; }
+		}
+		const bool dense_ok = cls == kFrameUnknown || cls == kFrameDense, scattered_ok = cls == kFrameUnknown || cls == kFrameScattered,
+		           small_ok = cls == kFrameUnknown || cls == kFrameSmall;
+		int cus = l.cus > 0 ? l.cus : 256;
+		if (l.cus <= 0) { int dev = 0; if (hipGetDevice(&dev) == hipSuccess) hipDeviceGetAttribute(&cus, hipDeviceAttributeMultiprocessorCount, dev); }
+		const bool beside = tiles && l.aux && l.ev_fork && l.ev_join && cls != kFrameSmall;
 		hipStream_t side = beside ? l.aux : stream;
 		if (beside)
 		{
@@ -1073,28 +1110,28 @@
 			if (e != hipSuccess) return e;
 		}
 
-		if (tiles)
-		{
-			int dev = 0, cus = 256;
-			if (hipGetDevice(&dev) == hipSuccess) hipDeviceGetAttribute(&cus, hipDeviceAttributeMultiprocessorCount, dev);
+		if (tiles && cls != kFrameSmall)
+		{
 			const u32 wgs = min((tiles + 3u) / 4u, (u32)cus * (u32)kSchedWaves);
 			const bool streamed = l.stream_scratch && !P.legacy && !P.trace;
 			bool stream_sparse = false;
 			if (streamed)
 			{
-				hipError_t e = launch_render_stream(&P, l.stream_scratch, l.W, l.H, l.stream_check, l.bricks, l.bricks_valid, stream, l.bricks_built, l.after, l.walk_share_pct, &stream_sparse);
+				hipError_t e = launch_render_stream(&P, l.stream_scratch, l.W, l.H, l.stream_check, l.bricks, l.bricks_valid, stream, l.bricks_built, l.after, l.walk_share_pct, &stream_sparse, cls, cus, &n_launched);
 				if (e != hipSuccess) return e;
 			}
+			const bool sched_dense = !streamed && dense_ok, sched_sparse = P.occ && !stream_sparse && scattered_ok;
 			if (one)
 			{
-				if (!streamed) hipLaunchKernelGGL((ca_render_packed_sched<false, 256, 1, kSchedWaves>), dim3(wgs), dim3(256), 0, stream, P);
-				if (P.occ && !stream_sparse) hipLaunchKernelGGL((ca_render_packed_sched<true, 256, 1, kSchedWaves>), dim3(wgs), dim3(256), 0, side, P);
+				if (sched_dense) hipLaunchKernelGGL((ca_render_packed_sched<false, 256, 1, kSchedWaves>), dim3(wgs), dim3(256), 0, stream, P);
+				if (sched_sparse) hipLaunchKernelGGL((ca_render_packed_sched<true, 256, 1, kSchedWaves>), dim3(wgs), dim3(256), 0, side, P);
 			}
 			else
 			{
-				if (!streamed) hipLaunchKernelGGL((ca_render_packed_sched<false, 64, kSchedChunk, kSchedWaves>), dim3(wgs), dim3(256), 0, stream, P);
-				if (P.occ && !stream_sparse) hipLaunchKernelGGL((ca_render_packed_sched<true, 64, kSchedChunk, kSchedWaves>), dim3(wgs), dim3(256), 0, side, P);
-			}
+				if (sched_dense) hipLaunchKernelGGL((ca_render_packed_sched<false, 64, kSchedChunk, kSchedWaves>), dim3(wgs), dim3(256), 0, stream, P);
+				if (sched_sparse) hipLaunchKernelGGL((ca_render_packed_sched<true, 64, kSchedChunk, kSchedWaves>), dim3(wgs), dim3(256), 0, side, P);
+			}
+			n_launched += (sched_dense ? 1u : 0u) + (sched_sparse ? 1u : 0u);
 		}
 		if (!beside && l.after)
 		{
@@ -1102,16 +1139,15 @@
 			if (e != hipSuccess) return e;
 		}
 		P.outside_only = tiles ? 1u : 0u;
-		if (P.bg) hipLaunchKernelGGL(ca_render_background, grid, dim3(256), 0, side, P);
-		else if (around) hipLaunchKernelGGL(ca_render_packed<false>, grid, dim3(256), 0, side, P);
-		if (P.occ && P.live_box)
-		{
-			int dev = 0, cus = 256;
-			if (hipGetDevice(&dev) == hipSuccess) hipDeviceGetAttribute(&cus, hipDeviceAttributeMultiprocessorCount, dev);
+		if (P.bg) { hipLaunchKernelGGL(ca_render_background, grid, dim3(256), 0, side, P); n_launched++; }
+		else if (around && dense_ok) { hipLaunchKernelGGL(ca_render_packed<false>, grid, dim3(256), 0, side, P); n_launched++; }
+		if (P.occ && P.live_box && small_ok)
+		{
 			P.spread = 1u;
 			hipLaunchKernelGGL(ca_render_packed_spread<true>, dim3((u32)cus * 4u), dim3(256), 0, side, P);
-		}
-		if (P.occ && around && !P.bg) hipLaunchKernelGGL(ca_render_packed<true>, grid, dim3(256), 0, side, P);
+			n_launched++;
+		}
+		if (P.occ && around && !P.bg && scattered_ok) { hipLaunchKernelGGL(ca_render_packed<true>, grid, dim3(256), 0, side, P); n_launched++; }
 		if (beside)
 		{
 			hipError_t e = hipEventRecord(l.ev_join, l.aux);
@@ -1121,9 +1157,12 @@
 	}
 	else
 	{
-		hipLaunchKernelGGL(ca_render_packed<false>, grid, dim3(256), 0, stream, P);
-		if (P.occ) hipLaunchKernelGGL(ca_render_packed<true>, grid, dim3(256), 0, stream, P);
-	}
+		const bool plain_dense = cls == kFrameUnknown || cls == kFrameDense, plain_sparse = P.occ && cls != kFrameDense;
+		if (plain_dense) hipLaunchKernelGGL(ca_render_packed<false>, grid, dim3(256), 0, stream, P);
+		if (plain_sparse) hipLaunchKernelGGL(ca_render_packed<true>, grid, dim3(256), 0, stream, P);
+		n_launched += (plain_dense ? 1u : 0u) + (plain_sparse ? 1u : 0u);
+	}
+	if (l.launches) *l.launches += n_launched;
 	return hipGetLastError();
 }
 
diff --git a/cellularautomatons3d_amd/csrc/render_device.inc b/cellularautomatons3d_amd/csrc/render_device.inc
--- a/cellularautomatons3d_amd/csrc/render_device.inc
+++ b/cellularautomatons3d_amd/csrc/render_device.inc
@@ -43,6 +43,7 @@
 	u32 bg, gx0, gx1, gy0, gy1;
 	u32 spread;
 	u32 park;
+	u32 lr_have, lrx0, lrx1, lry0, lry1;
 };
 
 constexpr float kPi = 3.14159265359f;
@@ -155,11 +156,36 @@
 	return V(fmaxf(0.0f, brdf.x * incident.x * LoN), fmaxf(0.0f, brdf.y * incident.y * LoN), fmaxf(0.0f, brdf.z * incident.z * LoN));
 }
 
+struct BoxWords
+{
+	u32 w[6];
+};
+__host__ __device__ inline bool occ_count_sparse(unsigned long long set, u32 G, u32 cols)
+{
+	return set * 4ull < (unsigned long long)cols * (G >> 3) * (G >> 3);
+}
+__host__ __device__ inline bool box_words_small(BoxWords b, u32 G)
+{
+	const u32 x1 = b.w[0], x0 = ~b.w[1], y1 = b.w[2], y0 = ~b.w[3], z1 = b.w[4], z0 = ~b.w[5];
+	if (x0 >= x1) return true;
+	return (unsigned long long)(x1 - x0) * (y1 - y0) * (z1 - z0) * 8ull < (unsigned long long)G * G * G;
+}
+__host__ __device__ inline int frame_class_of(unsigned long long set, BoxWords b, u32 G, u32 cols)
+{
+	if (!occ_count_sparse(set, G, cols)) return kFrameDense;
+	return box_words_small(b, G) ? kFrameSmall : kFrameScattered;
+}
+__device__ __forceinline__ BoxWords box_words_load(const RenderParams &P)
+{
+	BoxWords b;
+	for (int i = 0; i < 6; i++) b.w[i] = P.live_box[i];
+	return b;
+}
+
 __device__ __forceinline__ bool occ_skip_enabled(const RenderParams &P)
 {
 	if (!P.occ) return false;
-	const unsigned long long set = P.occ[P.occ_words];
-	return set * 4ull < (unsigned long long)P.cols * (P.G >> 3) * (P.G >> 3);
+	return occ_count_sparse(P.occ[P.occ_words], P.G, P.cols);
 }
 
 __device__ __forceinline__ bool misses_live_box(const RenderParams &P, v3 o, v3 d)
@@ -178,9 +204,7 @@
 __device__ __forceinline__ bool live_box_small(const RenderParams &P)
 {
 	if (!P.live_box) return false;
-	const u32 x1 = P.live_box[0], x0 = ~P.live_box[1], y1 = P.live_box[2], y0 = ~P.live_box[3], z1 = P.live_box[4], z0 = ~P.live_box[5];
-	if (x0 >= x1) return true;
-	return (unsigned long long)(x1 - x0) * (y1 - y0) * (z1 - z0) * 8ull < (unsigned long long)P.G * P.G * P.G;
+	return box_words_small(box_words_load(P), P.G);
 }
 
 __device__ __forceinline__ bool block_occupied(const RenderParams &P, int ix, int iy, int iz)
@@ -556,27 +580,36 @@
 	return true;
 }
 
-__device__ inline bool live_box_pix_rect(const RenderParams &P, PixRect &r)
+__host__ __device__ inline bool box_words_pix_rect(BoxWords b, u32 G, u32 cols, const float *u, float cot_half_fov, u32 W, u32 H, u32 row0, u32 row1, PixRect &r)
 {
 	r.x0 = r.x1 = r.y0 = r.y1 = 0u;
-	if (!P.live_box) return false;
-	const u32 x1 = P.live_box[0], x0 = ~P.live_box[1], y1 = P.live_box[2], y0 = ~P.live_box[3], z1 = P.live_box[4], z0 = ~P.live_box[5];
+	const u32 x1 = b.w[0], x0 = ~b.w[1], y1 = b.w[2], y0 = ~b.w[3], z1 = b.w[4], z0 = ~b.w[5];
 	if (x0 >= x1) return true;
 	{
-		const u32 G = P.G;
-		const u32 xa = ((0x7FFFFFFu % P.cols) << 5) + 31u, ya = 0xFFFFFFFFu % G;
+		const u32 xa = ((0x7FFFFFFu % cols) << 5) + 31u, ya = 0xFFFFFFFFu % G;
 		const u32 sx[3] = {0u, G - 1u, xa}, syz[3] = {0u, G - 1u, ya};
 		for (int k = 0; k < 3; k++)
 			if ((sx[k] >= x0 && sx[k] < x1) || (syz[k] >= y0 && syz[k] < y1) || (syz[k] >= z0 && syz[k] < z1)) return false;
 	}
-	const double cs = 1.0 / (double)P.G;
+	const double cs = 1.0 / (double)G;
 	const double lo[3] = {(double)x0 * cs - 0.5 - 2.0 * cs, (double)y0 * cs - 0.5 - 2.0 * cs, (double)z0 * cs - 0.5 - 2.0 * cs};
 	const double hi[3] = {(double)x1 * cs - 0.5 + 2.0 * cs, (double)y1 * cs - 0.5 + 2.0 * cs, (double)z1 * cs - 0.5 + 2.0 * cs};
-	return box_pix_rect(P.u, P.cot_half_fov, P.W, P.H, P.row0, P.row1, lo, hi, r);
+	return box_pix_rect(u, cot_half_fov, W, H, row0, row1, lo, hi, r);
+}
+__device__ inline bool live_box_pix_rect(const RenderParams &P, PixRect &r)
+{
+	r.x0 = r.x1 = r.y0 = r.y1 = 0u;
+	if (!P.live_box) return false;
+	return box_words_pix_rect(box_words_load(P), P.G, P.cols, P.u, P.cot_half_fov, P.W, P.H, P.row0, P.row1, r);
 }
 __device__ __forceinline__ bool in_pix_rect(const PixRect &r, u32 x, u32 y) { return x >= r.x0 && x < r.x1 && y >= r.y0 && y < r.y1; }
 __device__ __forceinline__ bool live_rect_load(const RenderParams &P, PixRect &r)
 {
+	if (P.lr_have)
+	{
+		r.x0 = P.lrx0; r.x1 = P.lrx1; r.y0 = P.lry0; r.y1 = P.lry1;
+		return P.lr_have == 1u;
+	}
 	const u32 *w = reinterpret_cast<const u32 *>(P.counters + 4);
 	r.x0 = w[1] & 0xFFFFu; r.x1 = w[1] >> 16; r.y0 = w[2] & 0xFFFFu; r.y1 = w[2] >> 16;
 	return w[0] == 1u;
diff --git a/cellularautomatons3d_amd/csrc/render_stream.hip b/cellularautomatons3d_amd/csrc/render_stream.hip
--- a/cellularautomatons3d_amd/csrc/render_stream.hip
+++ b/cellularautomatons3d_amd/csrc/render_stream.hip
@@ -985,14 +985,16 @@
 }
 
 template <int LAYOUT, bool CHECK>
-void launch_walks2(const StreamParams &S, u32 wgs2, u32 job_blocks, hipStream_t stream)
+u32 launch_walks2(const StreamParams &S, u32 wgs2, u32 job_blocks, hipStream_t stream, int frame_class)
 {
 	constexpr int PS = kBricksReadAny;
-	hipLaunchKernelGGL((ca_stream_walk2<false, LAYOUT, CHECK>), dim3(wgs2), dim3(kW2Threads), 0, stream, S);
-	if (S.skip_ok) hipLaunchKernelGGL((ca_stream_walk2<false, PS, CHECK, true>), dim3(wgs2), dim3(kW2Threads), 0, stream, S);
+	const bool dense_walks = frame_class != kFrameScattered, skip_walks = S.skip_ok && frame_class != kFrameDense;
+	if (dense_walks) hipLaunchKernelGGL((ca_stream_walk2<false, LAYOUT, CHECK>), dim3(wgs2), dim3(kW2Threads), 0, stream, S);
+	if (skip_walks) hipLaunchKernelGGL((ca_stream_walk2<false, PS, CHECK, true>), dim3(wgs2), dim3(kW2Threads), 0, stream, S);
 	hipLaunchKernelGGL(ca_stream_shadow_rays, dim3(job_blocks), dim3(256), 0, stream, S);
-	hipLaunchKernelGGL((ca_stream_walk2<true, LAYOUT, CHECK>), dim3(wgs2), dim3(kW2Threads), 0, stream, S);
-	if (S.skip_ok) hipLaunchKernelGGL((ca_stream_walk2<true, PS, CHECK, true>), dim3(wgs2), dim3(kW2Threads), 0, stream, S);
+	if (dense_walks) hipLaunchKernelGGL((ca_stream_walk2<true, LAYOUT, CHECK>), dim3(wgs2), dim3(kW2Threads), 0, stream, S);
+	if (skip_walks) hipLaunchKernelGGL((ca_stream_walk2<true, PS, CHECK, true>), dim3(wgs2), dim3(kW2Threads), 0, stream, S);
+	return 1u + (dense_walks ? 2u : 0u) + (skip_walks ? 2u : 0u);
 }
 
 }
@@ -1007,11 +1009,18 @@
 	return off;
 }
 
-hipError_t launch_render_stream(const void *params, void *scratch, uint32_t W, uint32_t H, bool check, uint32_t *bricks, bool bricks_valid, hipStream_t stream, bool *bricks_built, hipEvent_t before_resolve, int walk_share_pct, bool *sparse_too)
+hipError_t launch_render_stream(const void *params, void *scratch, uint32_t W, uint32_t H, bool check, uint32_t *bricks, bool bricks_valid, hipStream_t stream, bool *bricks_built, hipEvent_t before_resolve, int walk_share_pct, bool *sparse_too, int frame_class, int cus_known, uint32_t *launches)
 {
 	StreamParams S;
 	S.R = *static_cast<const RenderParams *>(params);
 	const RenderParams &P = S.R;
+	const bool bricked = bricks && frame_bricks_applies(P.G);
+	static const int skip_env = getenv("CA3D_STREAM_SKIP") ? atoi(getenv("CA3D_STREAM_SKIP")) : 1;
+	S.skip_ok = bricked && skip_env && P.occ ? 1u : 0u;
+	if (sparse_too) *sparse_too = S.skip_ok != 0u;
+	if (!check && (frame_class == kFrameSmall || (frame_class == kFrameScattered && !S.skip_ok))) return hipSuccess;
+	if (check) frame_class = kFrameUnknown;
+	uint32_t n_launched = 0;
 	size_t hit_off, occl_off, rays_off;
 	stream_scratch_bytes(W, H, P.spp, &hit_off, &occl_off, &rays_off);
 	char *base = static_cast<char *>(scratch);
@@ -1041,25 +1050,27 @@
 	const size_t trace_words = 8u * 2u * 4u * 256u * 8u * 2u;
 	if (trace_path && !trace_buf && hipMalloc((void **)&trace_buf, trace_words * 8u) != hipSuccess) trace_buf = nullptr;
 	S.trace = trace_path ? trace_buf : nullptr;
-	if (S.trace) hipMemsetAsync(S.trace, 0, trace_words * 8u, stream);
+	if (S.trace) { hipMemsetAsync(S.trace, 0, trace_words * 8u, stream); n_launched++; }
 	S.check = check ? 1u : 0u;
 	if (check)
 	{
 		hipMemsetAsync(S.hit, 0x5A, (size_t)S.chunks * per * 4u, stream);
 		hipMemsetAsync(S.occl, 0x5A, (size_t)S.chunks * per, stream);
+		n_launched += 2u;
 	}
 	hipError_t e = hipMemsetAsync(S.ctl, 0, 4096, stream);
 	if (e != hipSuccess) return e;
-	int dev = 0, cus = 256;
-	if (hipGetDevice(&dev) == hipSuccess) hipDeviceGetAttribute(&cus, hipDeviceAttributeMultiprocessorCount, dev);
+	n_launched++;
+	int dev = 0, cus = cus_known > 0 ? cus_known : 256;
+	if (cus_known <= 0 && hipGetDevice(&dev) == hipSuccess) hipDeviceGetAttribute(&cus, hipDeviceAttributeMultiprocessorCount, dev);
 	const u32 job_blocks = (S.chunks * per + 255u) / 256u;
-	const bool bricked = bricks && frame_bricks_applies(P.G);
 	S.volume = bricked ? bricks : P.cells;
 	if (bricked && !bricks_valid)
 	{
 		hipError_t eb = launch_brick_volume(P.cells, bricks, P.G, stream);
 		if (eb != hipSuccess) return eb;
 		if (bricks_built) *bricks_built = true;
+		n_launched++;
 	}
 	static const int pop_env = getenv("CA3D_STREAM_POP") ? atoi(getenv("CA3D_STREAM_POP")) : 0;
 	S.pop_at = pop_env >= 1 && pop_env <= 64 ? pop_env : 16;
@@ -1068,18 +1079,15 @@
 	static const int wgs_env = getenv("CA3D_STREAM_WGS_PCT") ? atoi(getenv("CA3D_STREAM_WGS_PCT")) : 0;
 	const u32 pct = (u32)(wgs_env >= 10 && wgs_env <= 100 ? wgs_env : (walk_share_pct >= 10 && walk_share_pct <= 100 ? walk_share_pct : 100));
 	const u32 wgs2 = max(8u, min(S.chunks, (u32)cus * (u32)kW2PerSimd * 4u / (u32)kW2Waves * pct / 100u));
-	static const int skip_env = getenv("CA3D_STREAM_SKIP") ? atoi(getenv("CA3D_STREAM_SKIP")) : 1;
-	S.skip_ok = bricked && skip_env && P.occ ? 1u : 0u;
-	if (sparse_too) *sparse_too = S.skip_ok != 0u;
 	static const int packed_env = getenv("CA3D_STREAM_PACKED") ? atoi(getenv("CA3D_STREAM_PACKED")) : 1;
 	const bool packed = bricked && packed_env && P.G <= 1024u && (unsigned long long)S.chunks * per < (1ull << 28);
-	void (*walks)(const StreamParams &, u32, u32, hipStream_t);
+	u32 (*walks)(const StreamParams &, u32, u32, hipStream_t, int);
 	if (packed) walks = check ? launch_walks2<kBricksPacked, true> : launch_walks2<kBricksPacked, false>;
 	else if (bricked && p2) walks = check ? launch_walks2<kBricksRead, true> : launch_walks2<kBricksRead, false>;
 	else if (bricked) walks = check ? launch_walks2<kBricksReadAny, true> : launch_walks2<kBricksReadAny, false>;
 	else if (p2) walks = check ? launch_walks2<kRowsP2, true> : launch_walks2<kRowsP2, false>;
 	else walks = check ? launch_walks2<kRowsAny, true> : launch_walks2<kRowsAny, false>;
-	walks(S, wgs2, job_blocks, stream);
+	n_launched += walks(S, wgs2, job_blocks, stream, frame_class);
 	const unsigned long long trace_waves = (unsigned long long)wgs2 * (unsigned)kW2Waves;
 	if (before_resolve)
 	{
@@ -1087,6 +1095,8 @@
 		if (ew != hipSuccess) return ew;
 	}
 	hipLaunchKernelGGL(ca_stream_resolve, dim3((S.chunks * (per / P.spp) + 255u) / 256u), dim3(256), 0, stream, S);
+	n_launched++;
+	if (launches) *launches += n_launched;
 	if (S.trace)
 	{
 		std::vector<unsigned long long> t(trace_words);
diff --git a/cellularautomatons3d_amd/engine.py b/cellularautomatons3d_amd/engine.py
--- a/cellularautomatons3d_amd/engine.py
+++ b/cellularautomatons3d_amd/engine.py
@@ -269,6 +269,16 @@
         _capi.check(self._lib.ca3d_get_render_pipeline(self._h, C.byref(n)))
         return int(n.value)
 
+    def render_class(self) -> int:
+        n = C.c_int32(0)
+        _capi.check(self._lib.ca3d_get_render_class(self._h, C.byref(n)))
+        return int(n.value)
+
+    def render_launches(self) -> int:
+        n = C.c_uint32(0)
+        _capi.check(self._lib.ca3d_get_render_launches(self._h, C.byref(n)))
+        return int(n.value)
+
     def info(self) -> Info:
         i = Info()
         _capi.check(self._lib.ca3d_get_info(self._h, C.byref(i)))
diff --git a/include/ca3d.h b/include/ca3d.h
--- a/include/ca3d.h
+++ b/include/ca3d.h
@@ -370,6 +370,11 @@
 
 int ca3d_get_render_pipeline(ca3d_t *h, int32_t *frames_in_flight);
 
+int ca3d_get_render_class(ca3d_t *h, int32_t *frame_class);
+int ca3d_get_render_launches(ca3d_t *h, uint32_t *launches);
+int ca3d_render_classify(uint32_t grid_size, uint64_t occupied_blocks, const uint32_t live_box[6], int32_t *frame_class);
+int ca3d_render_facts_usable(const uint64_t record_key[3], const uint64_t frame_key[3], int occupancy_valid, int copy_landed, int32_t *usable);
+
 int ca3d_set_option(ca3d_t *h, const char *name, int64_t value);
 
 #ifdef __cplusplus
```
